# SokhengDin/DNN-MPPI-MPC

Measured on AMD Instinct MI355X. Metric: trajectory-steps/sec (KxT/iter_time), diff-drive K=4096 T=50, higher is better.
Workload: dtype f32; 1 GPU; BASELINE config 2: differential-drive analytic dynamics, K=4096 x T=50 per GPU, reference __main__ parameters, closed loop with the driver's plant on the device; K_per_gpu=4096, K_global=4096, T=50, waypoint_mode=sequential (reference-exact), noise=Philox4x32-10 in-kernel, waypoint_idx_at_end_of_timing=99, build_id=5d93f4b6a923ee1f, exchange=none (one GPU)

## Files before the change

### dnn-mppi-mpc_amd/_capi.py

```python
from __future__ import annotations

import ctypes as C
import os

PKG = os.path.dirname(os.path.abspath(__file__))
ABI_VERSION = 6
MIN_AB_ABI_VERSION = 3
LIB_PATH = os.environ.get("MPPI_LIB") or os.path.join(PKG, "lib", "libmppi_hip.so")

MODEL_DIFFDRIVE, MODEL_RACECAR, MODEL_DIFFDRIVE_MLP = 0, 1, 2
PREC_F32, PREC_F64 = 0, 1
WAYPOINT_SEQUENTIAL, WAYPOINT_FROZEN, WAYPOINT_PER_ROLLOUT = 0, 1, 2
BETA_INV_EXPLORATION, BETA_INV_LAMBDA, BETA_LAMBDA = 0, 1, 2
FILTER_DIFFDRIVE, FILTER_RACECAR, FILTER_NONE, FILTER_TORCH = 0, 1, 2, 3
OBSTACLE_NONE, OBSTACLE_CIRCLE, OBSTACLE_OUTLINE = 0, 1, 2
OK, ERR_BAD_ARG, ERR_SHAPE, ERR_NO_DEVICE, ERR_HIP, ERR_PATH_END, ERR_UNSUPPORTED, ERR_STATE = 0, -1, -2, -3, -4, -5, -6, -7
ERR_COMM = -8
LAYOUT_FUSED, LAYOUT_DUAL, LAYOUT_PAIR, LAYOUT_TRI, LAYOUT_KIND, LAYOUT_TWICE = 0, 1, 2, 3, 3, 4


class MppiConfig(C.Structure):
    _fields_ = [
        ("struct_size", C.c_int32), ("device", C.c_int32), ("model", C.c_int32), ("precision", C.c_int32),
        ("K", C.c_int32), ("T", C.c_int32), ("K_global", C.c_int32), ("k_offset", C.c_int32),
        ("delta_t", C.c_double), ("u_max", C.c_double * 2), ("wheel_base", C.c_double),
        ("param_exploration", C.c_double), ("param_lambda", C.c_double), ("param_alpha", C.c_double),
        ("sigma", C.c_double * 4), ("stage_cost_weight", C.c_double * 4), ("terminal_cost_weight", C.c_double * 4),
        ("beta_mode", C.c_int32), ("accumulate_stage_cost", C.c_int32), ("waypoint_mode", C.c_int32),
        ("search_window", C.c_int32), ("wrap_yaw_stage", C.c_int32), ("wrap_yaw_terminal", C.c_int32),
        ("clamp_rollout", C.c_int32), ("clamp_u_after_update", C.c_int32), ("filter_mode", C.c_int32),
        ("filter_window", C.c_int32), ("obstacle_model", C.c_int32), ("raise_at_path_end", C.c_int32),
        ("safety_margin", C.c_double), ("vehicle_w", C.c_double), ("vehicle_l", C.c_double),
        ("collision_penalty", C.c_double), ("seed", C.c_uint64), ("n_agents", C.c_int32), ("noise_stream", C.c_int32),
    ]


class MppiStats(C.Structure):
    _fields_ = [("rho", C.c_double), ("eta", C.c_double), ("ess", C.c_double), ("idx_start", C.c_int32),
                ("idx_after", C.c_int32), ("path_end", C.c_int32), ("rounds", C.c_int32), ("iteration", C.c_int64),
                ("n_collided", C.c_int32), ("reserved", C.c_int32), ("iter_us", C.c_double), ("kernel_us", C.c_double)]


class MppiError(RuntimeError):
    def __init__(self, code, msg):
        super().__init__(f"libmppi_hip: {msg} (status {code})")
        self.code = code


_H = C.c_void_p
_D = C.POINTER(C.c_double)

PROTOTYPES = {
    "mppi_abi_version": (C.c_int, []),
    "mppi_last_error": (C.c_char_p, [_H]),
    "mppi_device_count": (C.c_int, []),
    "mppi_create": (C.c_int, [C.POINTER(MppiConfig), C.POINTER(_H)]),
    "mppi_destroy": (C.c_int, [_H]),
    "mppi_set_ref_path": (C.c_int, [_H, _D, C.c_int32, C.c_int32]),
    "mppi_set_obstacles": (C.c_int, [_H, _D, C.c_int32]),
    "mppi_set_agent_ref_path": (C.c_int, [_H, C.c_int32, _D, C.c_int32, C.c_int32]),
    "mppi_set_agent_obstacles": (C.c_int, [_H, C.c_int32, _D, C.c_int32]),
    "mppi_get_agent_status": (C.c_int, [_H, C.POINTER(C.c_int32), C.POINTER(C.c_int32)]),
    "mppi_set_mlp": (C.c_int, [_H, C.c_int32, C.c_int32, C.POINTER(C.c_float), C.POINTER(C.c_float),
                              C.POINTER(C.POINTER(C.c_float)), C.POINTER(C.POINTER(C.c_float)),
                              C.POINTER(C.c_float), C.POINTER(C.c_float)]),
    "mppi_set_mlp_scaled": (C.c_int, [_H, C.c_int32, C.c_int32, C.POINTER(C.c_float), C.POINTER(C.c_float),
                                     C.POINTER(C.POINTER(C.c_float)), C.POINTER(C.POINTER(C.c_float)),
                                     C.POINTER(C.c_float), C.POINTER(C.c_float), C.POINTER(C.c_double),
                                     C.POINTER(C.c_double), C.POINTER(C.c_double), C.POINTER(C.c_double)]),
    "mppi_set_agent_mlp": (C.c_int, [_H, C.c_int32, C.c_int32, C.c_int32, C.POINTER(C.c_float), C.POINTER(C.c_float),
                                    C.POINTER(C.POINTER(C.c_float)), C.POINTER(C.POINTER(C.c_float)),
                                    C.POINTER(C.c_float), C.POINTER(C.c_float)]),
    "mppi_set_agent_mlp_scaled": (C.c_int, [_H, C.c_int32, C.c_int32, C.c_int32, C.POINTER(C.c_float), C.POINTER(C.c_float),
                                           C.POINTER(C.POINTER(C.c_float)), C.POINTER(C.POINTER(C.c_float)),
                                           C.POINTER(C.c_float), C.POINTER(C.c_float), C.POINTER(C.c_double),
                                           C.POINTER(C.c_double), C.POINTER(C.c_double), C.POINTER(C.c_double)]),
    "mppi_set_u_prev": (C.c_int, [_H, _D]),
    "mppi_get_u_prev": (C.c_int, [_H, _D]),
    "mppi_set_waypoint_idx": (C.c_int, [_H, C.c_int32]),
    "mppi_get_waypoint_idx": (C.c_int, [_H, C.POINTER(C.c_int32)]),
    "mppi_step": (C.c_int, [_H, _D, C.c_void_p, _D, _D, C.POINTER(MppiStats), C.c_void_p]),
    "mppi_partial_len": (C.c_int, [_H, C.POINTER(C.c_int32)]),
    "mppi_step_begin": (C.c_int, [_H, _D, C.c_void_p, C.c_void_p, C.c_void_p]),
    "mppi_step_end": (C.c_int, [_H, C.c_void_p, C.c_int32, _D, _D, C.POINTER(MppiStats), C.c_void_p]),
    "mppi_step_end_async": (C.c_int, [_H, C.c_void_p, C.c_int32, C.c_void_p]),
    "mppi_sync_result": (C.c_int, [_H, _D, _D, C.POINTER(MppiStats), C.c_void_p]),
    "mppi_comm_handle_bytes": (C.c_int, []),
    "mppi_comm_export": (C.c_int, [_H, C.c_int32, C.c_void_p]),
    "mppi_comm_buffer": (C.c_int, [_H, C.POINTER(C.c_void_p)]),
    "mppi_comm_connect": (C.c_int, [_H, C.c_int32, C.c_int32, C.c_void_p, C.POINTER(C.c_void_p)]),
    "mppi_comm_probe": (C.c_int, [_H, C.c_void_p]),
    "mppi_comm_close": (C.c_int, [_H]),
    "mppi_get_costs": (C.c_int, [_H, _D]),
    "mppi_get_weights": (C.c_int, [_H, _D]),
    "mppi_sample_epsilon": (C.c_int, [_H, C.c_int64, C.c_void_p, C.c_void_p]),
    "mppi_set_iteration": (C.c_int, [_H, C.c_int64]),
    "mppi_set_noise_ring": (C.c_int, [_H, C.c_void_p, C.c_int32]),
    "mppi_rollout_viz": (C.c_int, [_H, C.c_void_p, C.c_void_p, C.c_void_p]),
    "mppi_set_state": (C.c_int, [_H, _D]),
    "mppi_get_state": (C.c_int, [_H, _D]),
    "mppi_run_closed_loop": (C.c_int, [_H, C.c_int32, _D, C.POINTER(MppiStats), C.c_void_p]),
    "mppi_last_kernel_ms": (C.c_int, [_H, C.POINTER(C.c_float)]),
    "mppi_enable_timing": (C.c_int, [_H, C.c_int32]),
    "mppi_set_rollout_repeats": (C.c_int, [_H, C.c_int32]),
    "mppi_get_counters": (C.c_int, [_H, C.POINTER(C.c_int64)]),
    "mppi_comm_unique_id_bytes": (C.c_int, []),
    "mppi_comm_unique_id": (C.c_int, [C.c_void_p]),
    "mppi_comm_init": (C.c_int, [_H, C.c_void_p, C.c_int32, C.c_int32]),
    "mppi_get_rollout_layout": (C.c_int, [_H, C.POINTER(C.c_int32)]),
    "mppi_get_host_timing": (C.c_int, [_H, C.POINTER(C.c_double)]),
    "mppi_get_rollout_kernel": (C.c_int, [_H, C.c_char_p, C.c_int32]),
    "mppi_time_rollout_launch": (C.c_int, [_H, C.c_int32, C.c_int32, C.c_void_p, C.POINTER(C.c_double)]),
    "mppi_step_device_x0": (C.c_int, [_H, C.c_void_p, C.c_void_p, _D, _D, C.POINTER(MppiStats), C.c_void_p]),
    "mppi_eval_state_transition": (C.c_int, [_H, _D, _D, C.c_int32, _D]),
    "mppi_eval_clamp": (C.c_int, [_H, _D, C.c_int32, _D]),
    "mppi_eval_is_collided": (C.c_int, [_H, _D, C.c_int32, _D]),
    "mppi_eval_nearest_waypoint": (C.c_int, [_H, _D, C.c_int32, C.POINTER(C.c_int32), C.c_int32, C.POINTER(C.c_int32)]),
    "mppi_eval_cost": (C.c_int, [_H, C.c_int32, _D, C.c_int32, C.POINTER(C.c_int32), C.c_int32, _D, C.POINTER(C.c_int32)]),
    "mppi_eval_moving_average": (C.c_int, [_H, _D, _D]),
    "mppi_eval_weights": (C.c_int, [_H, _D, C.c_int32, _D]),
    "mppi_cb_last_error": (C.c_char_p, [_H]),
    "mppi_cb_create": (C.c_int, [C.c_void_p, C.POINTER(_H)]),
    "mppi_cb_destroy": (C.c_int, [_H]),
    "mppi_cb_set_nominal": (C.c_int, [_H, _D]),
    "mppi_cb_get_nominal": (C.c_int, [_H, _D]),
    "mppi_cb_command": (C.c_int, [_H, _D, C.c_void_p, C.c_int32, _D, C.c_void_p]),
    "mppi_cb_get_costs": (C.c_int, [_H, _D, _D]),
    "mppi_cb_eval": (C.c_int, [_H, C.c_int32, _D, _D, C.c_int32, C.c_int32, _D]),
    "mppi_cb_nominal_trajectory": (C.c_int, [_H, _D, _D]),
}

_lib = None


def load_library(path: str | None = None):
    global _lib
    if _lib is not None and path is None:
        return _lib
    p = path or LIB_PATH
    if not os.path.exists(p):
        raise MppiError(ERR_NO_DEVICE, f"{p} not found: build it with __graft_entry__.build() "
                                       "(hipcc --offload-arch=gfx950); there is no CPU fallback")
    try:
        import torch
    except ImportError:
        pass
    lib = C.CDLL(p)
    ab_build = bool(os.environ.get("MPPI_LIB")) and path is None
    for name, (res, args) in PROTOTYPES.items():
        if ab_build and not hasattr(lib, name):
            continue
        fn = getattr(lib, name)
        fn.restype, fn.argtypes = res, args
    if lib.mppi_abi_version() != ABI_VERSION and not ab_build:
        raise MppiError(ERR_BAD_ARG, "ABI version mismatch between _capi.py and libmppi_hip.so")
    if ab_build and lib.mppi_abi_version() < MIN_AB_ABI_VERSION:
        raise MppiError(ERR_BAD_ARG, f"MPPI_LIB={p} has ABI version {lib.mppi_abi_version()}: its mppi_config / mppi_stats "
                                     f"layouts differ from this binding's (needs >= {MIN_AB_ABI_VERSION})")
    if path is None:
        _lib = lib
    return lib


def check(lib, handle, rc):
    if rc != OK:
        msg = lib.mppi_last_error(handle)
        raise MppiError(rc, msg.decode() if msg else "unknown error")
```

### dnn-mppi-mpc_amd/build.py

```python
from __future__ import annotations

import os
import subprocess

PKG = os.path.dirname(os.path.abspath(__file__))
CSRC = os.path.join(PKG, "csrc")
LIB = os.path.join(PKG, "lib", "libmppi_hip.so")


def lib_is_stale() -> bool:
    if not os.path.exists(LIB):
        return True
    t = os.path.getmtime(LIB)
    srcs = [os.path.join(CSRC, f) for f in os.listdir(CSRC) if f.endswith((".hip", ".h"))]
    srcs.append(os.path.join(os.path.dirname(PKG), "include", "mppi_hip.h"))
    return any(os.path.getmtime(s) > t for s in srcs)


def source_id() -> str:
    import hashlib
    h = hashlib.sha256()
    files = sorted(os.path.join(CSRC, f) for f in os.listdir(CSRC) if f.endswith((".hip", ".h")))
    files.append(os.path.join(os.path.dirname(PKG), "include", "mppi_hip.h"))
    for f in files:
        h.update(os.path.basename(f).encode())
        with open(f, "rb") as fh:
            h.update(fh.read())
    return h.hexdigest()[:16]


PRIMS_LIB = os.path.join(PKG, "lib", "libmppi_prims.so")
PRIMS_SRC = os.path.join(os.path.dirname(PKG), "tests", "device", "prims_harness.hip")


def prims_library() -> str:
    srcs = [PRIMS_SRC] + [os.path.join(CSRC, f) for f in os.listdir(CSRC) if f.endswith(".h")]
    if not os.path.exists(PRIMS_LIB) or any(os.path.getmtime(s) > os.path.getmtime(PRIMS_LIB) for s in srcs):
        res = subprocess.run(["make", "-C", CSRC, "prims"], stdout=subprocess.PIPE, stderr=subprocess.STDOUT, text=True)
        if res.returncode != 0:
            print(res.stdout)
            raise RuntimeError("building libmppi_prims.so failed (hipcc, gfx950)")
    return PRIMS_LIB


def build(force: bool = False, verbose: bool = False) -> str:
    if force or lib_is_stale() or not os.path.exists(PRIMS_LIB):
        cmd = ["make", "-j4", "-C", CSRC] + (["-B"] if force else [])
        res = subprocess.run(cmd, stdout=subprocess.PIPE, stderr=subprocess.STDOUT, text=True)
        if verbose or res.returncode != 0:
            print(res.stdout)
        if res.returncode != 0:
            raise RuntimeError("building libmppi_hip.so failed (hipcc, gfx950)")
    return LIB
```

### dnn-mppi-mpc_amd/csrc/mppi_capi.hip

```cpp
#include <dlfcn.h>
#include <hip/hip_runtime.h>
#include <math.h>
#include <stdio.h>
#include <stdlib.h>
#include <string.h>

#include <time.h>

#include <algorithm>
#include <string>
#include <vector>

#include "../../include/mppi_hip.h"
#include "mppi_kernels.h"
#include "mppi_owner.h"

using namespace mppi;

static thread_local std::string g_create_error;

static double now_s() {
    timespec ts;
    clock_gettime(CLOCK_MONOTONIC, &ts);
    return (double)ts.tv_sec + 1e-9 * (double)ts.tv_nsec;
}

static Switches read_switches() {
    const auto set = [](const char *name) { return getenv(name) != nullptr; };
    const auto num = [](const char *name, int unset) {
        const char *e = getenv(name);
        return e ? atoi(e) : unset;
    };
    const auto on_off = [&](const char *name) { return set(name) ? (int)(num(name, 0) != 0) : -1; };
    Switches sw;
    sw.dual = on_off("MPPI_DUAL");
    sw.pair = on_off("MPPI_PAIR");
    sw.tri = on_off("MPPI_TRI");
    sw.seq = set("MPPI_SEQ") ? (num("MPPI_SEQ", 0) == 2 ? 2 : 1) : -1;
    sw.no_stream = set("MPPI_NO_STREAM");
    sw.stream_passes = num("MPPI_STREAM_PASSES", 0);
    sw.force_unfused = set("MPPI_FORCE_UNFUSED");
    sw.no_hyp = set("MPPI_NO_HYP");
    sw.no_poll = set("MPPI_NO_POLL");
    sw.no_args = set("MPPI_NO_ARGS");
    sw.traj_per_block = num("MPPI_TRAJ_PER_BLOCK", 0);
    sw.graph = on_off("MPPI_GRAPH") == 1;
    sw.graph_verbose = set("MPPI_GRAPH_VERBOSE");
    sw.graph_slots = std::max(1, num("MPPI_GRAPH_SLOTS", 64));
    sw.mlp.f32 = set("MPPI_MLP_F32");
    sw.mlp.terms = num("MPPI_MLP_TERMS", 3) == 2 ? 2 : 3;
    const char *form = getenv("MPPI_MLP_FORM");
    sw.mlp.form = form && !strcmp(form, "4x64") ? 0 : form && !strcmp(form, "8x64") ? 1 : -1;
    if (const char *e = getenv("MPPI_EXCHANGE_TIMEOUT_MS")) sw.exchange_timeout_ms = atoll(e);
    sw.lb_timeout_ticks = std::max(0, num("MPPI_LB_TIMEOUT_TICKS", (int)LB_TIMEOUT_TICKS));
    return sw;
}

struct RcclUniqueId { char internal[128]; };

struct mppi_handle {
    mppi_config cfg;
    Switches sw;
    bool f64 = false;
    int nx = 3, n_ref = 0, n_obs = 0, n_blocks = 0, traj_per_block = 0;
    bool fused = false;
    int B = 1;
    int slots = 0;
    std::vector<Event> ev;
    size_t ev_used = 0;
    Event ev_step[2];
    bool graph_on = false;
    std::vector<char> graph_key;
    Stream graph_stream;
    Event graph_ev_in, graph_ev_out;
    Event graph_done[2];
    GraphExec graph_exec[2];
    DevBuf<void> d_partials2;
    DevBuf<void> d_heads, d_heads2;
    DevBuf<float> d_mlp;
    DevBuf<unsigned short> d_mlp16;
    size_t mlp_cap = 0, mlp16_cap = 0;
    bool hyp = false;
    DevBuf<unsigned> d_hyp_slots;
    unsigned lb_seq = 0;
    std::vector<double> ref_host;
    StepResult *res_mapped = nullptr;
    long long seq = 0;
    bool idx_valid = true;
    int layout = 0;
    const char *rollout_kernel = "";
    MlpParams mlp = {}, mlp_shared = {};
    bool shared_set = false;
    struct OwnModel {
        DevBuf<float> d_mlp;
        DevBuf<unsigned short> d_mlp16;
        size_t cap = 0, cap16 = 0;
        MlpParams q = {};
        bool set = false;
    };
    std::vector<OwnModel> own_mlp;
    DevBuf<MlpParams> d_models;
    DevBuf<void> d_ref, d_obs, d_u, d_uhist, d_S;
    struct OwnScene {
        DevBuf<void> d_ref, d_obs;
        int n_ref = 0, n_obs = 0;
        bool has_obs = false;
    };
    std::vector<OwnScene> own;
    DevBuf<AgentScene> d_scenes;
    DevBuf<int> d_pout;
    DevBuf<void> d_partials;
    DevBuf<double> d_w, d_trace;
    long long trace_cap = 0;
    DevBuf<DevState> d_st;
    DevBuf<StepResult> d_res;
    PinnedBuf<StepResult> h_res;
    size_t res_bytes = 0;
    const float *last_eps = nullptr;
    const float *noise_ring = nullptr;
    int noise_slots = 0;
    bool begun = false, timing = false, dev_loop_primed = false, slot_timed = false;
    long long iter = 0;
    int idx = 0, rollout_repeats = 1;
    float last_ms[4] = {0, 0, 0, 0};
    double last_iter_us = 0.0;
    FineBuf<char> xbuf;
    size_t xbuf_bytes = 0;
    int x_rank = 0, x_nranks = 0, x_export_nranks = 0;
    std::vector<IpcMap> x_opened;
    DevBuf<char *> d_xpeers;
    DevBuf<int> d_xerr, d_xok;
    long long xseq = 0, x_timeout = 300000000LL;
    void *rccl_comm = nullptr;
    int rccl_rank = 0, rccl_nranks = 0;
    DevBuf<double> d_rccl_part, d_rccl_gath;
    long long n_rollout_launches = 0, n_finalize_launches = 0;
    double t_enqueue_s = 0.0, t_loop_s = 0.0;
    std::string err;
};

#define FAIL(h, code, ...)                                   \
    do {                                                     \
        char _b[512];                                        \
        snprintf(_b, sizeof(_b), __VA_ARGS__);               \
        if (h) (h)->err = _b; else g_create_error = _b;      \
        return (code);                                       \
    } while (0)
#define CREATE_FAIL(code, ...) FAIL((mppi_handle *)nullptr, code, __VA_ARGS__)

#define HIPCHECK(h, call)                                                                          \
    do {                                                                                           \
        hipError_t _e = (call);                                                                    \
        if (_e != hipSuccess) FAIL(h, MPPI_ERR_HIP, "%s failed: %s", #call, hipGetErrorString(_e)); \
    } while (0)

extern "C" int mppi_abi_version(void) { return MPPI_ABI_VERSION; }

extern "C" const char *mppi_last_error(const mppi_handle *h) { return h ? h->err.c_str() : g_create_error.c_str(); }

extern "C" int mppi_device_count(void) {
    int n = 0;
    if (hipGetDeviceCount(&n) != hipSuccess) return 0;
    return n;
}

template <typename Fn> static auto with_real(const mppi_handle *h, Fn &&f) { return h->f64 ? f(double{}) : f(float{}); }

static size_t rsz(const mppi_handle *h) { return with_real(h, [](auto r) { return sizeof(r); }); }

static int kernel_model(const mppi_config &c) { return c.model == MPPI_MODEL_RACECAR ? MODEL_RACE : MODEL_DIFF; }
static double softmin_beta(const mppi_config &c) {
    return c.beta_mode == MPPI_BETA_INV_EXPLORATION ? 1.0 / c.param_exploration
           : c.beta_mode == MPPI_BETA_INV_LAMBDA    ? 1.0 / c.param_lambda
                                                    : c.param_lambda;
}
static bool at_path_end(const mppi_handle *h, int idx) { return idx >= h->n_ref - 1; }
static AgentScene scene_of(const mppi_handle *h, int a) {
    AgentScene sc = {h->d_ref, h->d_obs, h->n_ref, h->n_obs, {0, 0}};
    if (a < (int)h->own.size()) {
        const mppi_handle::OwnScene &o = h->own[a];
        if (o.d_ref) sc.ref = o.d_ref, sc.n_ref = o.n_ref;
        if (o.has_obs) sc.obs = o.d_obs, sc.n_obs = o.n_obs;
    }
    if (h->cfg.obstacle_model == MPPI_OBSTACLE_NONE) sc.n_obs = 0;
    return sc;
}
static bool any_obstacles(const mppi_handle *h) {
    for (int a = 0; a < h->B; ++a)
        if (scene_of(h, a).n_obs > 0) return true;
    return false;
}
static bool lookback_serves(const mppi_handle *h, int records) {
    const mppi_config &c = h->cfg;
    const bool lb_layout = (h->layout & LAYOUT_KIND) == LAYOUT_FUSED || h->layout == LAYOUT_DUAL;
    return h->fused && lb_layout && c.T <= 64 && c.model == MPPI_MODEL_DIFFDRIVE && c.waypoint_mode == MPPI_WAYPOINT_SEQUENTIAL &&
           !c.accumulate_stage_cost && (c.search_window == HYP_WINDOW || c.search_window == HYP_WINDOW_CUDA) && c.n_agents == 1 &&
           records <= HYP_MAX_BLOCKS && !h->sw.no_hyp;
}
static bool index_can_move(const mppi_handle *h) { return h->hyp && !(h->idx_valid && h->n_ref > 0 && at_path_end(h, h->idx)); }
template <typename R> static KParams<R> make_params(const mppi_handle *h, const float *eps);
template <typename R> static RolloutPlan front_plan(const mppi_handle *h, const KParams<R> &P);

static int upload_real(mppi_handle *h, void *dst, const double *src, size_t n) {
    return with_real(h, [&](auto r) -> int {
        using R = decltype(r);
        const std::vector<R> tmp(src, src + n);
        HIPCHECK(h, hipMemcpy(dst, tmp.data(), n * sizeof(R), hipMemcpyHostToDevice));
        return MPPI_OK;
    });
}

static int download_real(mppi_handle *h, double *dst, const void *src, size_t n) {
    return with_real(h, [&](auto r) -> int {
        using R = decltype(r);
        std::vector<R> tmp(n);
        HIPCHECK(h, hipMemcpy(tmp.data(), src, n * sizeof(R), hipMemcpyDeviceToHost));
        std::copy(tmp.begin(), tmp.end(), dst);
        return MPPI_OK;
    });
}

extern "C" int mppi_create(const mppi_config *cfg, mppi_handle **out) {
    if (!cfg || !out) CREATE_FAIL(MPPI_ERR_BAD_ARG, "mppi_create: null argument");
    if (cfg->struct_size != (int32_t)sizeof(mppi_config))
        CREATE_FAIL(MPPI_ERR_BAD_ARG, "mppi_create: struct_size %d != %zu (ABI mismatch)", cfg->struct_size, sizeof(mppi_config));
    mppi_config c = *cfg;
    const Switches sw = read_switches();
    if (c.K_global == 0) c.K_global = c.K;
    if (c.K > (1 << 20) || c.T > 2048)
        CREATE_FAIL(MPPI_ERR_SHAPE, "K=%d / T=%d beyond the supported 2^20 samples / 2048 steps", c.K, c.T);
    if (c.K < 1 || c.T < 1 || c.K_global < c.K || c.k_offset < 0 || c.k_offset + c.K > c.K_global)
        CREATE_FAIL(MPPI_ERR_SHAPE, "mppi_create: bad K=%d T=%d K_global=%d k_offset=%d", c.K, c.T, c.K_global, c.k_offset);
    if (c.model != MPPI_MODEL_DIFFDRIVE && c.model != MPPI_MODEL_RACECAR && c.model != MPPI_MODEL_DIFFDRIVE_MLP)
        CREATE_FAIL(MPPI_ERR_BAD_ARG, "mppi_create: unknown model %d", c.model);
    if (c.model == MPPI_MODEL_DIFFDRIVE_MLP && c.precision != MPPI_PREC_F32)
        CREATE_FAIL(MPPI_ERR_UNSUPPORTED, "the learned-dynamics rollout runs on the f32 MFMA path only");
    if (c.precision != MPPI_PREC_F32 && c.precision != MPPI_PREC_F64)
        CREATE_FAIL(MPPI_ERR_BAD_ARG, "mppi_create: unknown precision %d", c.precision);
    if (c.waypoint_mode != MPPI_WAYPOINT_SEQUENTIAL && c.waypoint_mode != MPPI_WAYPOINT_FROZEN && c.waypoint_mode != MPPI_WAYPOINT_PER_ROLLOUT)
        CREATE_FAIL(MPPI_ERR_BAD_ARG, "mppi_create: unknown waypoint_mode %d", c.waypoint_mode);
    if (c.waypoint_mode == MPPI_WAYPOINT_PER_ROLLOUT && c.model == MPPI_MODEL_RACECAR)
        CREATE_FAIL(MPPI_ERR_UNSUPPORTED,
// ... 554 lines not shown
    P.window = c.search_window;
    P.model = kernel_model(c);
    P.accumulate = c.accumulate_stage_cost;
    P.sequential = c.waypoint_mode == MPPI_WAYPOINT_SEQUENTIAL;
    P.per_rollout = c.waypoint_mode == MPPI_WAYPOINT_PER_ROLLOUT;
    P.lb_timeout = h->sw.lb_timeout_ticks;
    P.obstacle_model = any_obstacles(h) ? c.obstacle_model : OBS_NONE;
    P.clamp_rollout = c.clamp_rollout;
    P.wrap_stage = c.wrap_yaw_stage;
    P.wrap_term = c.wrap_yaw_terminal;
    const float *noise = eps ? eps : h->noise_ring;
    P.eps_slots = eps ? 0 : (h->noise_ring ? h->noise_slots : 0);
    P.use_philox = noise == nullptr;
    P.traj_per_block = h->traj_per_block;
    P.seed_lo = (unsigned)(c.seed & 0xffffffffu);
    P.seed_hi = (unsigned)(c.seed >> 32);
    P.dt = (R)c.delta_t;
    P.umax0 = (R)c.u_max[0];
    P.umax1 = (R)c.u_max[1];
    P.wheel_base = (R)c.wheel_base;
    P.beta = (R)softmin_beta(c);
    P.gamma = (R)(c.param_lambda * (1.0 - c.param_alpha));
    P.penalty = (R)c.collision_penalty;
    P.two_pi = (R)(2.0 * M_PI);
    const double det = c.sigma[0] * c.sigma[3] - c.sigma[1] * c.sigma[2];
    const double si[4] = {c.sigma[3] / det, -c.sigma[1] / det, -c.sigma[2] / det, c.sigma[0] / det};
    for (int i = 0; i < 4; ++i) {
        P.sinv[i] = (R)si[i];
        P.ws[i] = (R)c.stage_cost_weight[i];
        P.wt[i] = (R)c.terminal_cost_weight[i];
    }
    const double vw = c.vehicle_w * c.safety_margin, vl = c.vehicle_l * c.safety_margin;
    const double sx[9] = {-0.5 * vl, -0.5 * vl, 0.0, 0.5 * vl, 0.5 * vl, 0.5 * vl, 0.0, -0.5 * vl, -0.5 * vl};
    const double sy[9] = {0.0, 0.5 * vw, 0.5 * vw, 0.5 * vw, 0.0, -0.5 * vw, -0.5 * vw, -0.5 * vw, 0.0};
    for (int i = 0; i < 9; ++i) {
        P.shape_x[i] = (R)sx[i];
        P.shape_y[i] = (R)sy[i];
    }
    const double l00 = sqrt(c.sigma[0]), l10 = c.sigma[2] / l00, l11 = sqrt(c.sigma[3] - l10 * l10);
    P.chol[0] = (float)l00;
    P.chol[1] = (float)l10;
    P.chol[2] = (float)l11;
    P.ref = (const R *)sc0.ref;
    P.obs = (const R *)sc0.obs;
    P.scenes = h->d_scenes;
    P.u = (const R *)h->d_u.get();
    P.eps = noise;
    P.S = (R *)h->d_S.get();
    P.pout = h->d_pout;
    P.st = h->d_st;
    P.noise_stream = c.noise_stream;
    P.slots = h->slots;
    P.n_agents = h->B;
    P.layout = h->layout;
    P.heads = (R *)h->d_heads.get();
    P.hyp = index_can_move(h);
    P.lb_seq = 0;
    P.hyp_slots = h->d_hyp_slots;
    return P;
}

static double record_beta(const mppi_handle *h) {
    const double beta = softmin_beta(h->cfg);
    return h->f64 ? beta : (double)(float)beta;
}

static FinalizeParams make_finalize(const mppi_handle *h, int plant, const void *abi_recs = nullptr, int n_recs = 0) {
    const mppi_config &c = h->cfg;
    FinalizeParams F;
    memset(&F, 0, sizeof(F));
    F.T = c.T;
    F.K = c.K;
    F.n_part = n_recs;
    F.filter_mode = c.filter_mode;
    F.filter_window = c.filter_window;
    F.clamp_u = c.clamp_u_after_update;
    F.raise_at_path_end = c.raise_at_path_end;
    F.model = kernel_model(c);
    F.sequential = c.waypoint_mode == MPPI_WAYPOINT_SEQUENTIAL;
    F.plant = plant;
    const AgentScene sc0 = scene_of(h, 0);
    F.n_ref = sc0.n_ref;
    F.window = c.search_window;
    F.is_f64 = h->f64;
    F.count_hits = any_obstacles(h);
    F.beta = record_beta(h);
    F.dt = c.delta_t;
    F.wheel_base = c.wheel_base;
    F.umax0 = c.u_max[0];
    F.umax1 = c.u_max[1];
    F.partials = abi_recs;
    F.heads = h->d_heads;
    F.u = h->d_u;
    F.u_out = h->d_u;
    F.u_before = h->d_uhist;
    F.ref = sc0.ref;
    F.scenes = h->d_scenes;
    F.pout = h->d_pout;
    F.st = h->d_st;
    F.st_out = h->d_st;
    F.res = h->d_res;
    F.slots = h->slots;
    F.n_agents = h->B;
    F.res_stride = h->res_bytes;
    F.u0_trace = nullptr;
    F.hyp_slots = h->d_hyp_slots;
    F.lb_seq = 0;
    F.pad_lb = 0;
    return F;
}

constexpr int EV_PER_SLOT = 8;
constexpr size_t EV_MAX = 8u * 200000u;

static hipEvent_t next_event(mppi_handle *h) {
    if (h->ev_used == h->ev.size()) hipEventCreate(h->ev.emplace_back().put());
    return h->ev[h->ev_used++];
}

static bool timing_on(const mppi_handle *h) { return h->timing && h->ev_used + EV_PER_SLOT <= EV_MAX; }

static void wire_exchange(const mppi_handle *h, FinalizeParams &F) {
    if (h->x_nranks <= 1) return;
    F.x_nranks = h->x_nranks;
    F.x_rank = h->x_rank;
    F.x_timeout = h->x_timeout;
    F.x_peers = h->d_xpeers;
    F.x_err = h->d_xerr;
}

template <typename R> static RolloutPlan front_plan(const mppi_handle *h, const KParams<R> &P) {
    if constexpr (sizeof(R) == 4)
        if (h->cfg.model == MPPI_MODEL_DIFFDRIVE_MLP) return plan_mlp(P, h->mlp, h->sw);
    return plan_rollout<R>(P, h->fused, h->sw);
}

struct SlotPlan {
    RolloutPlan front;
    bool reduce = false;
    int n_merges = 0;
    MergeStep merge[2];
    double beta = 0.0;
    KernelLaunch fin;
};
template <typename R>
static SlotPlan plan_slot(const mppi_handle *h, const KParams<R> &P, FinalizeParams *F, double *rank_record = nullptr) {
    SlotPlan sp;
    sp.front = front_plan<R>(h, P);
    sp.reduce = h->cfg.model != MPPI_MODEL_DIFFDRIVE_MLP && !h->fused;
    sp.beta = record_beta(h);
    const void *recs = h->d_partials, *heads = h->d_heads;
    const MergeTree tree = merge_tree(sp.front.records, rank_record == nullptr);
    if (tree.group) {
        sp.merge[sp.n_merges++] = plan_merge<R>(recs, heads, sp.front.records, tree.group, h->cfg.T, h->d_partials2, h->d_heads2);
        recs = h->d_partials2;
        heads = h->d_heads2;
    }
    if (rank_record) {
        sp.merge[sp.n_merges++] = plan_merge<R>(recs, heads, tree.n_out, tree.n_out, h->cfg.T, rank_record, nullptr);
        return sp;
    }
    F->partials = recs;
    F->heads = heads;
    F->n_part = tree.n_out;
    F->hyp = sp.front.lookback;
    F->hyp_blocks = sp.front.records;
    wire_exchange(h, *F);
    sp.fin = plan_finalize<R>(*F, false, sp.front.lookback);
    return sp;
}

template <typename R> static void launch_records(mppi_handle *h, const SlotPlan &sp, const KParams<R> &P, hipStream_t s, bool tm) {
    if (tm) hipEventRecord(next_event(h), s);
    h->n_rollout_launches += h->rollout_repeats;
    for (int rep = 0; rep < h->rollout_repeats; ++rep) {
        if constexpr (sizeof(R) == 4)
            if (h->cfg.model == MPPI_MODEL_DIFFDRIVE_MLP) {
                launch_mlp(sp.front, P, h->mlp, h->d_models, h->d_partials, nullptr, s);
                continue;
            }
        launch_rollout<R>(sp.front, P, h->d_partials, s);
    }
    h->rollout_kernel = sp.front.k.name;
    if (tm) hipEventRecord(next_event(h), s);
    if (tm) hipEventRecord(next_event(h), s);
    if (sp.reduce) launch_reduce<R>(P, h->d_partials, sp.front.records, s);
    for (int i = 0; i < sp.n_merges; ++i) launch_merge<R>(sp.merge[i], h->cfg.T, sp.beta, s);
    if (tm) hipEventRecord(next_event(h), s);
}

static void launch_back(mppi_handle *h, const KernelLaunch &fin, const FinalizeParams &F, hipStream_t s, bool tm) {
    if (tm) hipEventRecord(next_event(h), s);
    ++h->n_finalize_launches;
    launch_finalize(fin, F, s);
    if (tm) hipEventRecord(next_event(h), s);
    if (tm) hipEventRecord(next_event(h), s);
    if (tm) hipEventRecord(next_event(h), s);
}

template <typename R>
static void launch_slot(mppi_handle *h, const SlotPlan &sp, const KParams<R> &P, FinalizeParams F, hipStream_t s) {
    const bool tm = timing_on(h);
    if (F.x_nranks > 1) F.x_seq = ++h->xseq;
    if (sp.front.lookback) {
        if ((++h->lb_seq & 0xffffffu) == 0u) ++h->lb_seq;
        KParams<R> Pl = P;
        Pl.lb_seq = F.lb_seq = h->lb_seq;
        launch_records<R>(h, sp, Pl, s, tm);
    } else {
        launch_records<R>(h, sp, P, s, tm);
    }
    launch_back(h, sp.fin, F, s, tm);
}

static void collect_timing(mppi_handle *h) {
    double acc[4] = {0, 0, 0, 0};
    const size_t slots = h->ev_used / EV_PER_SLOT;
    for (size_t i = 0; i < slots; ++i)
        for (int j = 0; j < 4; ++j) {
            float ms = 0;
            hipEventElapsedTime(&ms, h->ev[EV_PER_SLOT * i + 2 * j], h->ev[EV_PER_SLOT * i + 2 * j + 1]);
            acc[j] += ms;
        }
    const double cal = slots ? acc[3] / slots : 0.0;
    for (int j = 0; j < 3; ++j) {
        const double v = slots ? acc[j] / slots - cal : 0.0;
        h->last_ms[j] = (float)(v > 0 ? v : 0);
    }
    h->last_ms[3] = (float)cal;
}

static int check_ready(mppi_handle *h, const char *who) {
    if (!h) return MPPI_ERR_BAD_ARG;
    for (int a = 0; a < h->B; ++a) {
        const AgentScene sc = scene_of(h, a);
        if (!sc.ref || sc.n_ref < 1) {
            if (h->B > 1) FAIL(h, MPPI_ERR_STATE, "%s: ref_path of agent %d has not been set", who, a);
            FAIL(h, MPPI_ERR_STATE, "%s: ref_path has not been set", who);
        }
        if (sc.n_obs > 0 && !sc.obs) FAIL(h, MPPI_ERR_STATE, "%s: obstacles not uploaded", who);
    }
    if (h->cfg.model == MPPI_MODEL_DIFFDRIVE_MLP)
        for (int a = 0; a < h->B; ++a)
            if (!has_model(h, a)) {
                if (h->B > 1) FAIL(h, MPPI_ERR_STATE, "%s: agent %d has no model (mppi_set_mlp / mppi_set_agent_mlp)", who, a);
                FAIL(h, MPPI_ERR_STATE, "%s: mppi_set_mlp has not been called", who);
            }
    return MPPI_OK;
}

#define SINGLE_AGENT_ONLY(h, who)                                                                                     \
    do {                                                                                                              \
        if ((h)->B > 1) FAIL(h, MPPI_ERR_UNSUPPORTED, "%s serves single-agent handles (n_agents = %d)", who, (h)->B); \
    } while (0)

static void fill_stats(mppi_handle *h, mppi_stats *stats) {
    if (!stats) return;
    if (h->timing && h->ev_used >= EV_PER_SLOT) {
        if (hipEventSynchronize(h->ev[h->ev_used - 1]) == hipSuccess) collect_timing(h);
        else (void)hipGetLastError();
    }
    const StepResult *r = h->h_res;
    stats->rho = r->rho;
    stats->eta = r->eta;
    stats->ess = r->ess;
    stats->idx_start = r->idx_start;
    stats->idx_after = r->idx_after;
    stats->path_end = r->path_end;
    stats->rounds = r->rounds;
    stats->iteration = r->iter;
    stats->n_collided = r->n_collided;
    stats->reserved = 0;
    stats->iter_us = h->last_iter_us;
    stats->kernel_us = h->timing ? 1e3 * ((double)h->last_ms[0] + h->last_ms[1] + h->last_ms[2]) : 0.0;
}

static int host_x0_call(const mppi_handle *h, const double *x0) {
    const int p = h->idx, n = h->n_ref, w = h->cfg.search_window;
    int best_j = 0;
    double best = INFINITY;
    for (int j = 0; j < w && p + j < n; ++j) {
        const double dx = x0[0] - h->ref_host[4 * (size_t)(p + j)], dy = x0[1] - h->ref_host[4 * (size_t)(p + j) + 1];
        const double d = dx * dx + dy * dy;
        if (d < best) { best = d; best_j = j; }
    }
    return p + best_j;
}

static int fetch_result(mppi_handle *h, size_t bytes, hipStream_t s, bool check_launches = true) {
    HIPCHECK(h, hipMemcpyAsync(h->h_res, h->d_res, bytes, hipMemcpyDeviceToHost, s));
    HIPCHECK(h, hipStreamSynchronize(s));
    if (check_launches) HIPCHECK(h, hipGetLastError());
    return MPPI_OK;
}

static int wait_result(mppi_handle *h, long long seq, hipStream_t s) {
    if (seq) {
        volatile long long *flag = &h->h_res->seq;
        const double t0 = now_s();
        for (long long spins = 0; *flag != seq; ++spins) {
            __builtin_ia32_pause();
            if ((spins & 1023) == 1023 && now_s() - t0 > 0.020) {
                HIPCHECK(h, hipStreamSynchronize(s));
                HIPCHECK(h, hipGetLastError());
                if (*flag != seq) FAIL(h, MPPI_ERR_HIP, "the finalize kernel never published its result");
                break;
            }
        }
        __atomic_thread_fence(__ATOMIC_ACQUIRE);
        return MPPI_OK;
    }
    return fetch_result(h, h->res_bytes, s);
}

static void note_noise(mppi_handle *h, const float *eps, bool observed_state) {
    h->last_eps = eps;
    if (observed_state) h->dev_loop_primed = false;
}

enum : unsigned {
    KEEP_IDX_VALID = 1u,
    KEEP_GOING = 2u,
};
static int adopt_result(mppi_handle *h, unsigned keep, double *u_out, double *u0_out, mppi_stats *stats) {
    const StepResult *res = h->h_res;
    h->idx = res->idx_after;
    if (!(keep & KEEP_IDX_VALID)) h->idx_valid = true;
    fill_stats(h, stats);
    if (!(keep & KEEP_GOING)) {
        if (res->status == STATUS_EXCHANGE_FAILED)
            FAIL(h, MPPI_ERR_COMM, "peer-to-peer exchange: a rank did not arrive within the timeout");
        if (res->status == STATUS_PATH_END) FAIL(h, MPPI_ERR_PATH_END, "[ERROR] Reached the end of the reference path.");
    }
    h->iter = res->iter;
    if (u_out) memcpy(u_out, reinterpret_cast<const double *>(h->h_res + 1), sizeof(double) * 2 * h->cfg.T);
    if (u0_out) { u0_out[0] = res->u0[0]; u0_out[1] = res->u0[1]; }
    return MPPI_OK;
}

template <typename R>
static int step_rccl(mppi_handle *h, const double *x0, const double *x0_dev, const float *eps, double *u_out, double *u0_out,
                     mppi_stats *stats, hipStream_t s);
template <typename R>
static int closed_loop_rccl(mppi_handle *h, int n_iters, double *u0_trace, mppi_stats *stats, hipStream_t s);

template <typename R>
static int step_impl(mppi_handle *h, const double *x0, const double *x0_dev, const float *eps, double *u_out, double *u0_out,
                     mppi_stats *stats, hipStream_t s) {
    if (h->rccl_comm && h->x_nranks <= 1) return step_rccl<R>(h, x0, x0_dev, eps, u_out, u0_out, stats, s);
    const double t_call = now_s();
    KParams<R> P = make_params<R>(h, eps);
    FinalizeParams F = make_finalize(h, 0);
    const bool by_args = x0 && h->idx_valid && !h->sw.no_args;
    if (!x0) {
        if (!h->idx_valid) FAIL(h, MPPI_ERR_STATE, "mppi_step_device_x0 after an asynchronous split step: call mppi_sync_result first");
        launch_set_state_dev<R>(P, x0_dev, h->nx, s);
    } else if (by_args) {
        P.use_args = F.use_args = 1;
        P.c_arg = F.c_arg = host_x0_call(h, x0);
        P.hyp = h->hyp && !at_path_end(h, P.c_arg);
        for (int i = 0; i < 4; ++i) P.x0_arg[i] = F.x0_arg[i] = x0[i];
    } else {
        launch_set_state<R>(P, x0, s);
    }
    if (!h->sw.no_poll) F.res = h->res_mapped;
    const SlotPlan sp = plan_slot<R>(h, P, &F);
    for (int round = 0;; ++round) {
        F.seq = !h->sw.no_poll ? ++h->seq : 0;
        launch_slot<R>(h, sp, P, F, s);
        HIPCHECK(h, hipGetLastError());
        int rc = wait_result(h, F.seq, s);
        if (rc) return rc;
        if (h->h_res->status != STATUS_NEED_ROUND) break;
        if (round > h->cfg.K + 1) FAIL(h, MPPI_ERR_STATE, "waypoint speculation did not converge");
        P.use_args = 0;
    }
    note_noise(h, eps, true);
    h->last_iter_us = 1e6 * (now_s() - t_call);
    return adopt_result(h, 0, u_out, u0_out, stats);
}

extern "C" int mppi_step(mppi_handle *h, const double *x0, const float *eps, double *u_out, double *u0_out,
                         mppi_stats *stats, void *stream) {
    int rc = check_ready(h, "mppi_step");
    if (rc) return rc;
    SINGLE_AGENT_ONLY(h, "mppi_step");
    if (!x0) FAIL(h, MPPI_ERR_BAD_ARG, "mppi_step: x0 is null");
    HIPCHECK(h, hipSetDevice(h->cfg.device));
    double x[4] = {0, 0, 0, 0};
    for (int i = 0; i < h->nx; ++i) x[i] = x0[i];
    return with_real(h, [&](auto r) { return step_impl<decltype(r)>(h, x, nullptr, eps, u_out, u0_out, stats, (hipStream_t)stream); });
}

extern "C" int mppi_step_device_x0(mppi_handle *h, const double *x0_device, const float *eps, double *u_out, double *u0_out,
                                   mppi_stats *stats, void *stream) {
    int rc = check_ready(h, "mppi_step_device_x0");
    if (rc) return rc;
    SINGLE_AGENT_ONLY(h, "mppi_step_device_x0");
    if (!x0_device) FAIL(h, MPPI_ERR_BAD_ARG, "mppi_step_device_x0: x0 is null");
    HIPCHECK(h, hipSetDevice(h->cfg.device));
    return with_real(h, [&](auto r) { return step_impl<decltype(r)>(h, nullptr, x0_device, eps, u_out, u0_out, stats, (hipStream_t)stream); });
}

extern "C" int mppi_partial_len(const mppi_handle *h, int32_t *n) {
    if (!h || !n) return MPPI_ERR_BAD_ARG;
    *n = partial_len(h->cfg.T);
    return MPPI_OK;
}

template <typename R>
static int begin_impl(mppi_handle *h, const double *x0, const float *eps, double *partial, hipStream_t s) {
    KParams<R> P = make_params<R>(h, eps);
    if (x0 || !h->dev_loop_primed) launch_set_state<R>(P, x0, s);
    h->dev_loop_primed = x0 == nullptr;
    h->slot_timed = timing_on(h);
    launch_records<R>(h, plan_slot<R>(h, P, nullptr, partial), P, s, h->slot_timed);
    HIPCHECK(h, hipGetLastError());
    note_noise(h, eps, false);
    h->begun = true;
    return MPPI_OK;
}

extern "C" int mppi_step_begin(mppi_handle *h, const double *x0, const float *eps, double *partial, void *stream) {
    int rc = check_ready(h, "mppi_step_begin");
    if (rc) return rc;
    SINGLE_AGENT_ONLY(h, "mppi_step_begin");
    if (!partial) FAIL(h, MPPI_ERR_BAD_ARG, "mppi_step_begin: null argument");
    if (h->cfg.waypoint_mode == MPPI_WAYPOINT_SEQUENTIAL)
        FAIL(h, MPPI_ERR_UNSUPPORTED, "the split step needs MPPI_WAYPOINT_FROZEN (no cross-sample waypoint state)");
    HIPCHECK(h, hipSetDevice(h->cfg.device));
    double x[4] = {0, 0, 0, 0};
    if (x0)
        for (int i = 0; i < h->nx; ++i) x[i] = x0[i];
    return with_real(h, [&](auto r) { return begin_impl<decltype(r)>(h, x0 ? x : nullptr, eps, partial, (hipStream_t)stream); });
}

extern "C" int mppi_step_end(mppi_handle *h, const double *partials, int32_t nranks, double *u_out, double *u0_out,
                             mppi_stats *stats, void *stream) {
    int rc = check_ready(h, "mppi_step_end");
    if (rc) return rc;
    SINGLE_AGENT_ONLY(h, "mppi_step_end");
    if (!partials || nranks < 1 || nranks > MERGE_MAX_RECORDS)
        FAIL(h, MPPI_ERR_BAD_ARG, "mppi_step_end: bad partials/nranks (1..%d)", MERGE_MAX_RECORDS);
    if (!h->begun) FAIL(h, MPPI_ERR_STATE, "mppi_step_end without mppi_step_begin");
    HIPCHECK(h, hipSetDevice(h->cfg.device));
    hipStream_t s = (hipStream_t)stream;
    const FinalizeParams F = make_finalize(h, 0, partials, nranks);
    with_real(h, [&](auto r) { launch_back(h, plan_finalize<decltype(r)>(F, true, false), F, s, h->slot_timed); });
    if ((rc = fetch_result(h, h->res_bytes, s))) return rc;
    h->begun = false;
    h->dev_loop_primed = false;
    return adopt_result(h, KEEP_IDX_VALID, u_out, u0_out, stats);
}

extern "C" int mppi_step_end_async(mppi_handle *h, const double *partials, int32_t nranks, void *stream) {
    int rc = check_ready(h, "mppi_step_end_async");
    if (rc) return rc;
    SINGLE_AGENT_ONLY(h, "mppi_step_end_async");
    if (!partials || nranks < 1 || nranks > MERGE_MAX_RECORDS)
        FAIL(h, MPPI_ERR_BAD_ARG, "mppi_step_end_async: bad partials/nranks (1..%d)", MERGE_MAX_RECORDS);
    if (!h->begun) FAIL(h, MPPI_ERR_STATE, "mppi_step_end_async without mppi_step_begin");
    HIPCHECK(h, hipSetDevice(h->cfg.device));
    const FinalizeParams F = make_finalize(h, 1, partials, nranks);
    with_real(h, [&](auto r) { launch_back(h, plan_finalize<decltype(r)>(F, true, false), F, (hipStream_t)stream, h->slot_timed); });
    HIPCHECK(h, hipGetLastError());
    h->begun = false;
    h->idx_valid = false;
    return MPPI_OK;
}

extern "C" int mppi_sync_result(mppi_handle *h, double *u_out, double *u0_out, mppi_stats *stats, void *stream) {
    if (!h) return MPPI_ERR_BAD_ARG;
    HIPCHECK(h, hipSetDevice(h->cfg.device));
    if (int rc = fetch_result(h, h->res_bytes, (hipStream_t)stream, false)) return rc;
    return adopt_result(h, 0, u_out, u0_out, stats);
}

extern "C" int mppi_get_costs(mppi_handle *h, double *S) {
    if (!h || !S) return MPPI_ERR_BAD_ARG;
    HIPCHECK(h, hipSetDevice(h->cfg.device));
    HIPCHECK(h, hipDeviceSynchronize());
    return download_real(h, S, h->d_S, (size_t)h->B * h->cfg.K);
}

extern "C" int mppi_get_weights(mppi_handle *h, double *w) {
    if (!h || !w) return MPPI_ERR_BAD_ARG;
    SINGLE_AGENT_ONLY(h, "mppi_get_weights");
    HIPCHECK(h, hipSetDevice(h->cfg.device));
    HIPCHECK(h, hipDeviceSynchronize());
    if (!h->d_w) HIPCHECK(h, h->d_w.alloc(sizeof(double) * h->cfg.K));
    with_real(h, [&](auto r) {
        using R = decltype(r);
        launch_weights<R>(make_params<R>(h, nullptr), h->h_res->rho, h->h_res->eta, h->d_w, nullptr);
    });
    HIPCHECK(h, hipDeviceSynchronize());
    HIPCHECK(h, hipMemcpy(w, h->d_w, sizeof(double) * h->cfg.K, hipMemcpyDeviceToHost));
    return MPPI_OK;
}

extern "C" int mppi_sample_epsilon(mppi_handle *h, int64_t iteration, float *eps_out, void *stream) {
    if (!h || !eps_out || iteration < 0) return MPPI_ERR_BAD_ARG;
    HIPCHECK(h, hipSetDevice(h->cfg.device));
    KParams<float> P = make_params<float>(h, nullptr);
    for (int a = 0; a < h->B; ++a)
        launch_sample(P.seed_lo, P.seed_hi, (unsigned)iteration, h->cfg.K, h->cfg.T, h->cfg.k_offset, P.chol,
                      eps_out + (size_t)a * h->cfg.K * h->cfg.T * 2, (hipStream_t)stream, (unsigned)(h->cfg.noise_stream + a));
    HIPCHECK(h, hipGetLastError());
    return MPPI_OK;
}

extern "C" int mppi_set_noise_ring(mppi_handle *h, const float *eps_ring, int32_t n_slots) {
    if (!h) return MPPI_ERR_BAD_ARG;
    if (!eps_ring || n_slots == 0) {
        h->noise_ring = nullptr;
        h->noise_slots = 0;
        return MPPI_OK;
    }
    if (n_slots < 1 || (n_slots & (n_slots - 1)) != 0)
        FAIL(h, MPPI_ERR_BAD_ARG, "mppi_set_noise_ring: n_slots must be a power of two (got %d)", n_slots);
    hipPointerAttribute_t at;
    memset(&at, 0, sizeof(at));
    if (hipPointerGetAttributes(&at, eps_ring) != hipSuccess || at.type == hipMemoryTypeHost || at.type == hipMemoryTypeUnregistered ||
        at.device != h->cfg.device) {
        (void)hipGetLastError();
        FAIL(h, MPPI_ERR_BAD_ARG, "mppi_set_noise_ring: the ring must be device memory on the handle's GPU (device %d)", h->cfg.device);
    }
    h->noise_ring = eps_ring;
    h->noise_slots = n_slots;
    return MPPI_OK;
}

extern "C" int mppi_rollout_viz(mppi_handle *h, float *optimal_traj, float *sampled_traj, void *stream) {
    int rc = check_ready(h, "mppi_rollout_viz");
    if (rc) return rc;
    SINGLE_AGENT_ONLY(h, "mppi_rollout_viz");
    if (h->iter < 1) FAIL(h, MPPI_ERR_STATE, "mppi_rollout_viz before the first mppi_step");
    HIPCHECK(h, hipSetDevice(h->cfg.device));
    with_real(h, [&](auto r) {
        using R = decltype(r);
        const KParams<R> P = make_params<R>(h, h->last_eps);
        const R *hist = (const R *)h->d_uhist.get(), *hist_after = hist + 2 * h->cfg.T;
        if constexpr (sizeof(R) == 4)
            if (h->cfg.model == MPPI_MODEL_DIFFDRIVE_MLP)
                return launch_viz_mlp(P, h->mlp, h->sw, hist, hist_after, h->iter - 1, optimal_traj, sampled_traj, (hipStream_t)stream);
        launch_viz<R>(P, hist, hist_after, h->iter - 1, optimal_traj, sampled_traj, (hipStream_t)stream);
    });
    HIPCHECK(h, hipGetLastError());
    return MPPI_OK;
}


namespace {
struct RcclApi {
    void *lib = nullptr;
    int (*GetUniqueId)(void *) = nullptr;
    int (*CommInitRank)(void **, int, RcclUniqueId, int) = nullptr;
    int (*AllGather)(const void *, void *, size_t, int, void *, hipStream_t) = nullptr;
    int (*CommDestroy)(void *) = nullptr;
    const char *(*GetErrorString)(int) = nullptr;
    std::string why;
};
RcclApi rccl_load() {
    RcclApi a;
    for (const char *name : {"librccl.so.1", "librccl.so"}) {
        a.lib = dlopen(name, RTLD_NOW | RTLD_GLOBAL);
        if (a.lib) break;
    }
    if (!a.lib) {
        a.why = std::string("librccl.so.1 could not be loaded: ") + dlerror();
        return a;
    }
    a.GetUniqueId = reinterpret_cast<decltype(a.GetUniqueId)>(dlsym(a.lib, "ncclGetUniqueId"));
    a.CommInitRank = reinterpret_cast<decltype(a.CommInitRank)>(dlsym(a.lib, "ncclCommInitRank"));
    a.AllGather = reinterpret_cast<decltype(a.AllGather)>(dlsym(a.lib, "ncclAllGather"));
    a.CommDestroy = reinterpret_cast<decltype(a.CommDestroy)>(dlsym(a.lib, "ncclCommDestroy"));
    a.GetErrorString = reinterpret_cast<decltype(a.GetErrorString)>(dlsym(a.lib, "ncclGetErrorString"));
    if (!a.GetUniqueId || !a.CommInitRank || !a.AllGather || !a.CommDestroy || !a.GetErrorString) {
        a.why = "librccl.so.1 lacks an expected symbol";
        a.lib = nullptr;
    }
    return a;
}
RcclApi &rccl_api() {
    static RcclApi a = rccl_load();
    return a;
}
}

static void rccl_release(mppi_handle *h) {
    if (h->rccl_comm) rccl_api().CommDestroy(h->rccl_comm);
    (void)h->d_rccl_part.reset();
    (void)h->d_rccl_gath.reset();
    h->rccl_comm = nullptr;
    h->rccl_nranks = 0;
}

#define RCCLCHECK(h, call)                                                                                   \
    do {                                                                                                     \
        const int _r = (call);                                                                               \
        if (_r != 0) FAIL(h, MPPI_ERR_COMM, "%s failed: %s", #call, rccl_api().GetErrorString(_r));          \
    } while (0)

extern "C" int mppi_comm_unique_id_bytes(void) { return (int)sizeof(RcclUniqueId); }

extern "C" int mppi_comm_unique_id(void *id_out) {
    if (!id_out) return MPPI_ERR_BAD_ARG;
    RcclApi &a = rccl_api();
    if (!a.lib) {
        g_create_error = a.why;
        return MPPI_ERR_COMM;
    }
    if (a.GetUniqueId(id_out) != 0) {
        g_create_error = "ncclGetUniqueId failed";
        return MPPI_ERR_COMM;
    }
    return MPPI_OK;
}

extern "C" int mppi_comm_init(mppi_handle *h, const void *unique_id, int32_t rank, int32_t nranks) {
    if (!h || !unique_id) return MPPI_ERR_BAD_ARG;
    SINGLE_AGENT_ONLY(h, "mppi_comm_init");
    if (nranks < 1 || nranks > MERGE_MAX_RECORDS || rank < 0 || rank >= nranks)
        FAIL(h, MPPI_ERR_BAD_ARG, "mppi_comm_init: rank %d of %d (1..%d ranks)", rank, nranks, MERGE_MAX_RECORDS);
    if (h->cfg.waypoint_mode == MPPI_WAYPOINT_SEQUENTIAL)
        FAIL(h, MPPI_ERR_UNSUPPORTED, "the exchange needs MPPI_WAYPOINT_FROZEN (no cross-sample waypoint state)");
    RcclApi &a = rccl_api();
    if (!a.lib) FAIL(h, MPPI_ERR_COMM, "mppi_comm_init: %s", a.why.c_str());
    HIPCHECK(h, hipSetDevice(h->cfg.device));
    rccl_release(h);
    RcclUniqueId id;
    memcpy(&id, unique_id, sizeof(id));
    RCCLCHECK(h, a.CommInitRank(&h->rccl_comm, nranks, id, rank));
    const size_t len = (size_t)partial_len(h->cfg.T);
    HIPCHECK(h, h->d_rccl_part.alloc(sizeof(double) * len));
    HIPCHECK(h, h->d_rccl_gath.alloc(sizeof(double) * len * nranks));
    h->rccl_rank = rank;
    h->rccl_nranks = nranks;
    return MPPI_OK;
}

static int trace_rows(mppi_handle *h, int n_iters, double **rows) {
    if (h->trace_cap < n_iters) {
        h->trace_cap = 0;
        HIPCHECK(h, h->d_trace.reset());
        HIPCHECK(h, h->d_trace.alloc(sizeof(double) * 2 * n_iters));
        h->trace_cap = n_iters;
    }
    *rows = h->d_trace.get() - 2 * h->iter;
    return MPPI_OK;
}

template <typename R>
static int rccl_iteration(mppi_handle *h, const KParams<R> &P, int plant, double *u0_trace_dev, hipStream_t s) {
    const bool tm = timing_on(h);
    launch_records<R>(h, plan_slot<R>(h, P, nullptr, h->d_rccl_part), P, s, tm);
    RCCLCHECK(h, rccl_api().AllGather(h->d_rccl_part, h->d_rccl_gath, (size_t)partial_len(h->cfg.T), 8 ,
                                      h->rccl_comm, s));
    FinalizeParams F = make_finalize(h, plant, h->d_rccl_gath, h->rccl_nranks);
    F.u0_trace = u0_trace_dev;
    launch_back(h, plan_finalize<R>(F, true, false), F, s, tm);
    return MPPI_OK;
}

static int rccl_fetch(mppi_handle *h, double *u_out, double *u0_out, mppi_stats *stats, hipStream_t s) {
    HIPCHECK(h, hipGetLastError());
    if (int rc = fetch_result(h, h->res_bytes, s)) return rc;
    return adopt_result(h, 0, u_out, u0_out, stats);
}

template <typename R>
static int step_rccl(mppi_handle *h, const double *x0, const double *x0_dev, const float *eps, double *u_out, double *u0_out,
                     mppi_stats *stats, hipStream_t s) {
    const KParams<R> P = make_params<R>(h, eps);
    if (x0) launch_set_state<R>(P, x0, s);
    else launch_set_state_dev<R>(P, x0_dev, h->nx, s);
    if (int rc = rccl_iteration<R>(h, P, 0, nullptr, s)) return rc;
    note_noise(h, eps, true);
    return rccl_fetch(h, u_out, u0_out, stats, s);
}

template <typename R>
static int closed_loop_rccl(mppi_handle *h, int n_iters, double *u0_trace, mppi_stats *stats, hipStream_t s) {
    const KParams<R> P = make_params<R>(h, nullptr);
    double *trace = nullptr;
    if (u0_trace)
        if (int rc = trace_rows(h, n_iters, &trace)) return rc;
    if (!h->dev_loop_primed) launch_set_state<R>(P, nullptr, s);
    h->dev_loop_primed = false;
    for (int i = 0; i < n_iters; ++i)
        if (int rc = rccl_iteration<R>(h, P, 1, trace, s)) return rc;
    note_noise(h, nullptr, false);
    if (int rc = rccl_fetch(h, nullptr, nullptr, stats, s)) return rc;
    if (u0_trace) HIPCHECK(h, hipMemcpy(u0_trace, h->d_trace, sizeof(double) * 2 * n_iters, hipMemcpyDeviceToHost));
    h->dev_loop_primed = true;
    return MPPI_OK;
}

extern "C" int mppi_comm_handle_bytes(void) { return (int)sizeof(hipIpcMemHandle_t); }

extern "C" int mppi_comm_close(mppi_handle *h) {
    if (!h) return MPPI_ERR_BAD_ARG;
    hipSetDevice(h->cfg.device);
    hipDeviceSynchronize();
    h->x_opened.clear();
    (void)h->d_xpeers.reset();
    (void)h->d_xerr.reset();
    (void)h->d_xok.reset();
    (void)h->xbuf.reset();
    h->x_nranks = h->x_export_nranks = 0;
    rccl_release(h);
    return MPPI_OK;
}

extern "C" int mppi_comm_export(mppi_handle *h, int32_t nranks, void *handle_out) {
    if (!h || !handle_out) return MPPI_ERR_BAD_ARG;
    SINGLE_AGENT_ONLY(h, "mppi_comm_export");
    if (nranks < 2 || nranks > XCHG_MAX_RANKS)
        FAIL(h, MPPI_ERR_BAD_ARG, "mppi_comm_export: nranks must be 2..%d (got %d)", XCHG_MAX_RANKS, nranks);
    if (h->cfg.waypoint_mode == MPPI_WAYPOINT_SEQUENTIAL)
        FAIL(h, MPPI_ERR_UNSUPPORTED, "the exchange needs MPPI_WAYPOINT_FROZEN (no cross-sample waypoint state)");
    if (merge_lds_elems(h->cfg.T, h->cfg.filter_window, rsz(h)) * rsz(h) + sizeof(double) * XCHG_LDS_RANKS * xchg_rec_len(h->cfg.T) > 64 * 1024)
        FAIL(h, MPPI_ERR_UNSUPPORTED, "the peer-to-peer exchange stages the rank records in LDS: horizon T=%d is too long for it "
                                      "(use the split step with a collective)", h->cfg.T);
    if (h->xbuf) mppi_comm_close(h);
    HIPCHECK(h, hipSetDevice(h->cfg.device));
    h->xbuf_bytes = 2 * xchg_slot_bytes(h->cfg.T, nranks);
    HIPCHECK(h, h->xbuf.alloc(h->xbuf_bytes));
    HIPCHECK(h, hipMemset(h->xbuf, 0, h->xbuf_bytes));
    HIPCHECK(h, hipDeviceSynchronize());
    hipIpcMemHandle_t ipc;
    HIPCHECK(h, hipIpcGetMemHandle(&ipc, h->xbuf));
    memcpy(handle_out, &ipc, sizeof(ipc));
    h->x_export_nranks = nranks;
    return MPPI_OK;
}

extern "C" int mppi_comm_buffer(mppi_handle *h, void **device_ptr) {
    if (!h || !device_ptr) return MPPI_ERR_BAD_ARG;
    if (!h->xbuf) FAIL(h, MPPI_ERR_STATE, "mppi_comm_buffer before mppi_comm_export");
    *device_ptr = h->xbuf;
    return MPPI_OK;
}

extern "C" int mppi_comm_connect(mppi_handle *h, int32_t rank, int32_t nranks, const void *handles,
                                 void *const *local_ptrs) {
    if (!h || (!handles && !local_ptrs)) return MPPI_ERR_BAD_ARG;
    if (!h->xbuf || nranks != h->x_export_nranks)
        FAIL(h, MPPI_ERR_STATE, "mppi_comm_connect: call mppi_comm_export with the same nranks first");
    if (rank < 0 || rank >= nranks) FAIL(h, MPPI_ERR_BAD_ARG, "mppi_comm_connect: rank %d of %d", rank, nranks);
    HIPCHECK(h, hipSetDevice(h->cfg.device));
    std::vector<char *> peers(nranks, nullptr);
    std::vector<IpcMap> opened;
    for (int r = 0; r < nranks; ++r) {
        if (r == rank) {
            peers[r] = h->xbuf;
        } else if (local_ptrs && local_ptrs[r]) {
            hipPointerAttribute_t at;
            memset(&at, 0, sizeof(at));
            if (hipPointerGetAttributes(&at, local_ptrs[r]) != hipSuccess || at.type == hipMemoryTypeHost ||
                at.type == hipMemoryTypeUnregistered) {
                (void)hipGetLastError();
                FAIL(h, MPPI_ERR_UNSUPPORTED, "mppi_comm_connect: local_ptrs[%d] is not device memory (pass the peer's mppi_comm_buffer)", r);
            }
            if (at.device != h->cfg.device) {
                int can = 0;
                if (hipDeviceCanAccessPeer(&can, h->cfg.device, at.device) != hipSuccess || !can)
                    FAIL(h, MPPI_ERR_UNSUPPORTED, "mppi_comm_connect: device %d cannot access rank %d's buffer on device %d "
                                                  "(no peer access: use the collective carrier)", h->cfg.device, r, at.device);
                const hipError_t pe = hipDeviceEnablePeerAccess(at.device, 0);
                if (pe != hipSuccess && pe != hipErrorPeerAccessAlreadyEnabled)
                    FAIL(h, MPPI_ERR_UNSUPPORTED, "mppi_comm_connect: hipDeviceEnablePeerAccess(%d) failed: %s", at.device,
                         hipGetErrorString(pe));
                (void)hipGetLastError();
            }
            peers[r] = (char *)local_ptrs[r];
        } else {
            if (!handles) FAIL(h, MPPI_ERR_BAD_ARG, "mppi_comm_connect: no handle for rank %d", r);
            hipIpcMemHandle_t ipc;
            memcpy(&ipc, (const char *)handles + sizeof(ipc) * (size_t)r, sizeof(ipc));
            HIPCHECK(h, hipIpcOpenMemHandle(opened.emplace_back().put(), ipc, hipIpcMemLazyEnablePeerAccess));
            peers[r] = (char *)opened.back().get();
        }
    }
    DevBuf<char *> d_xpeers;
    DevBuf<int> d_xerr, d_xok;
    HIPCHECK(h, d_xpeers.alloc(sizeof(char *) * nranks));
    HIPCHECK(h, hipMemcpy(d_xpeers, peers.data(), sizeof(char *) * nranks, hipMemcpyHostToDevice));
    HIPCHECK(h, d_xerr.alloc(sizeof(int)));
    HIPCHECK(h, d_xok.alloc(sizeof(int)));
    HIPCHECK(h, hipMemset(d_xerr, 0, sizeof(int)));
    h->d_xpeers = std::move(d_xpeers);
    h->d_xerr = std::move(d_xerr);
    h->d_xok = std::move(d_xok);
    for (IpcMap &m : opened) h->x_opened.push_back(std::move(m));
    if (const long long ms = read_switches().exchange_timeout_ms; ms > 0) h->x_timeout = ms * 100000LL;
    h->x_rank = rank;
    h->x_nranks = nranks;
    h->xseq = 0;
    return MPPI_OK;
}

extern "C" int mppi_comm_probe(mppi_handle *h, void *stream) {
    if (!h) return MPPI_ERR_BAD_ARG;
    if (h->x_nranks <= 1) FAIL(h, MPPI_ERR_STATE, "mppi_comm_probe before mppi_comm_connect");
    HIPCHECK(h, hipSetDevice(h->cfg.device));
    FinalizeParams F = make_finalize(h, 0);
    wire_exchange(h, F);
    F.x_seq = ++h->xseq;
    launch_exchange_probe(F, h->d_xok, (hipStream_t)stream);
    int ok = 0;
    HIPCHECK(h, hipMemcpyAsync(&ok, h->d_xok, sizeof(int), hipMemcpyDeviceToHost, (hipStream_t)stream));
    HIPCHECK(h, hipStreamSynchronize((hipStream_t)stream));
    if (!ok) {
// ... 206 lines not shown
    return MPPI_OK;
}

extern "C" int mppi_time_rollout_launch(mppi_handle *h, int32_t n_slots, int32_t extra, void *stream, double *us_out2) {
    int rc = check_ready(h, "mppi_time_rollout_launch");
    if (rc) return rc;
    if (!us_out2 || n_slots < 1 || n_slots > 4096 || extra < 1 || extra > 16)
        FAIL(h, MPPI_ERR_BAD_ARG, "mppi_time_rollout_launch: n_slots 1..4096, extra 1..16");
    if (h->x_nranks > 1 || h->rccl_comm)
        FAIL(h, MPPI_ERR_UNSUPPORTED, "mppi_time_rollout_launch: not with an exchange between ranks (its sequence numbers cannot be replayed)");
    HIPCHECK(h, hipSetDevice(h->cfg.device));
    return with_real(h, [&](auto r) { return time_rollout_impl<decltype(r)>(h, n_slots, extra, (hipStream_t)stream, us_out2); });
}

static void eval_transition_mlp(mppi_handle *h, const KParams<float> &P, const void *x, const void *v, int n, void *out) {
    launch_eval_mlp(P, h->mlp, h->sw, (const float *)x, (const float *)v, n, (float *)out, nullptr);
}
static void eval_transition_mlp(mppi_handle *, const KParams<double> &, const void *, const void *, int, void *) {}

template <typename R>
static int eval_impl(mppi_handle *h, int what, const double *x, const double *v, int n, int32_t *prev_idx, int update,
                     double *out, int32_t *idx_out) {
    const KParams<R> P = make_params<R>(h, nullptr);
    const int nx = h->nx;
    const bool need_x = what != EVAL_CLAMP, need_v = what == EVAL_TRANSITION || what == EVAL_CLAMP;
    const bool need_idx = what == EVAL_COST_STAGE || what == EVAL_COST_TERMINAL || what < 0;
    const int n_out = what == EVAL_TRANSITION ? nx : what == EVAL_CLAMP ? 2 : 1;
    DevBuf<R> dx, dv, dout;
    DevBuf<int> di, dp;
    if (need_x) {
        HIPCHECK(h, dx.alloc(sizeof(R) * (size_t)n * nx));
        if (int rc = upload_real(h, dx, x, (size_t)n * nx)) return rc;
    }
    if (need_v) {
        HIPCHECK(h, dv.alloc(sizeof(R) * (size_t)n * 2));
        if (int rc = upload_real(h, dv, v, (size_t)n * 2)) return rc;
    }
    if (need_idx) {
        if (!prev_idx) FAIL(h, MPPI_ERR_BAD_ARG, "mppi_eval: prev_idx is null");
        if (*prev_idx < 0 || *prev_idx >= P.n_ref) FAIL(h, MPPI_ERR_BAD_ARG, "mppi_eval: waypoint index %d out of range", *prev_idx);
        HIPCHECK(h, di.alloc(sizeof(int) * (size_t)n));
        HIPCHECK(h, dp.alloc(sizeof(int)));
        launch_eval_index<R>(P, dx, nx, n, *prev_idx, update ? 1 : 0, di, dp, nullptr);
    }
    if (what >= 0) {
        HIPCHECK(h, dout.alloc(sizeof(R) * (size_t)n * n_out));
        if (what == EVAL_TRANSITION && h->cfg.model == MPPI_MODEL_DIFFDRIVE_MLP)
            eval_transition_mlp(h, P, dx, dv, n, dout);
        else
            launch_eval<R>(P, what, dx, dv, di, n, dout, nullptr);
    }
    HIPCHECK(h, hipGetLastError());
    HIPCHECK(h, hipDeviceSynchronize());
    if (what >= 0)
        if (int rc = download_real(h, out, dout, (size_t)n * n_out)) return rc;
    if (need_idx) {
        if (idx_out) HIPCHECK(h, hipMemcpy(idx_out, di, sizeof(int) * (size_t)n, hipMemcpyDeviceToHost));
        int pn = *prev_idx;
        HIPCHECK(h, hipMemcpy(&pn, dp, sizeof(int), hipMemcpyDeviceToHost));
        if (update) *prev_idx = pn;
    }
    return MPPI_OK;
}

static int eval_entry(mppi_handle *h, const char *who, int what, const double *x, const double *v, int n, int32_t *prev_idx,
                      int update, double *out, int32_t *idx_out) {
    int rc = check_ready(h, who);
    if (rc) return rc;
    if (n < 1 || (what >= 0 && !out)) FAIL(h, MPPI_ERR_BAD_ARG, "%s: bad argument", who);
    if ((what != EVAL_CLAMP && !x) || ((what == EVAL_TRANSITION || what == EVAL_CLAMP) && !v))
        FAIL(h, MPPI_ERR_BAD_ARG, "%s: null input", who);
    HIPCHECK(h, hipSetDevice(h->cfg.device));
    return with_real(h, [&](auto r) { return eval_impl<decltype(r)>(h, what, x, v, n, prev_idx, update, out, idx_out); });
}

extern "C" int mppi_eval_state_transition(mppi_handle *h, const double *x, const double *v, int32_t n, double *x_next) {
    return eval_entry(h, "mppi_eval_state_transition", EVAL_TRANSITION, x, v, n, nullptr, 0, x_next, nullptr);
}
extern "C" int mppi_eval_clamp(mppi_handle *h, const double *v, int32_t n, double *out) {
    return eval_entry(h, "mppi_eval_clamp", EVAL_CLAMP, nullptr, v, n, nullptr, 0, out, nullptr);
}
extern "C" int mppi_eval_is_collided(mppi_handle *h, const double *x, int32_t n, double *out) {
    return eval_entry(h, "mppi_eval_is_collided", EVAL_COLLIDED, x, nullptr, n, nullptr, 0, out, nullptr);
}
extern "C" int mppi_eval_nearest_waypoint(mppi_handle *h, const double *x, int32_t n, int32_t *prev_idx, int32_t update_prev_idx,
                                          int32_t *idx_out) {
    if (h && !idx_out) FAIL(h, MPPI_ERR_BAD_ARG, "mppi_eval_nearest_waypoint: idx_out is null");
    return eval_entry(h, "mppi_eval_nearest_waypoint", -1, x, nullptr, n, prev_idx, update_prev_idx, nullptr, idx_out);
}
extern "C" int mppi_eval_cost(mppi_handle *h, int32_t terminal, const double *x, int32_t n, int32_t *prev_idx,
                              int32_t update_prev_idx, double *cost, int32_t *idx_out) {
    return eval_entry(h, "mppi_eval_cost", terminal ? EVAL_COST_TERMINAL : EVAL_COST_STAGE, x, nullptr, n, prev_idx,
                      update_prev_idx, cost, idx_out);
}

extern "C" int mppi_eval_moving_average(mppi_handle *h, const double *xx, double *out) {
    if (!h || !xx || !out) return MPPI_ERR_BAD_ARG;
    HIPCHECK(h, hipSetDevice(h->cfg.device));
    const int T = h->cfg.T;
    DevBuf<void> in, o;
    HIPCHECK(h, in.alloc(rsz(h) * 2 * T));
    HIPCHECK(h, o.alloc(rsz(h) * 2 * T));
    if (int rc = upload_real(h, in, xx, (size_t)2 * T)) return rc;
    with_real(h, [&](auto r) {
        using R = decltype(r);
        launch_eval_filter<R>((const R *)in.get(), (R *)o.get(), T, h->cfg.filter_window, h->cfg.filter_mode, nullptr);
    });
    HIPCHECK(h, hipGetLastError());
    HIPCHECK(h, hipDeviceSynchronize());
    return download_real(h, out, o, (size_t)2 * T);
}

extern "C" int mppi_eval_weights(mppi_handle *h, const double *S, int32_t n, double *w) {
    if (!h || !S || !w || n < 1) return MPPI_ERR_BAD_ARG;
    HIPCHECK(h, hipSetDevice(h->cfg.device));
    DevBuf<double> in, o;
    HIPCHECK(h, in.alloc(sizeof(double) * (size_t)n));
    HIPCHECK(h, o.alloc(sizeof(double) * (size_t)n));
    HIPCHECK(h, hipMemcpy(in, S, sizeof(double) * (size_t)n, hipMemcpyHostToDevice));
    launch_eval_weights(in, n, softmin_beta(h->cfg), o, nullptr);
    HIPCHECK(h, hipGetLastError());
    HIPCHECK(h, hipDeviceSynchronize());
    HIPCHECK(h, hipMemcpy(w, o, sizeof(double) * (size_t)n, hipMemcpyDeviceToHost));
    return MPPI_OK;
}

extern "C" int mppi_get_counters(mppi_handle *h, int64_t *out3) {
    if (!h || !out3) return MPPI_ERR_BAD_ARG;
    out3[0] = h->iter;
    out3[1] = h->n_rollout_launches;
    out3[2] = h->n_finalize_launches;
    return MPPI_OK;
}

extern "C" int mppi_get_host_timing(const mppi_handle *h, double *out2) {
    if (!h || !out2) return MPPI_ERR_BAD_ARG;
    out2[0] = h->t_enqueue_s;
    out2[1] = h->t_loop_s;
    return MPPI_OK;
}

extern "C" int mppi_get_rollout_layout(const mppi_handle *h, int32_t *layout) {
    if (!h || !layout) return MPPI_ERR_BAD_ARG;
    *layout = (h->fused && h->cfg.model != MPPI_MODEL_DIFFDRIVE_MLP) ? h->layout : -1;
    return MPPI_OK;
}

extern "C" int mppi_get_rollout_kernel(const mppi_handle *h, char *buf, int32_t n) {
    if (!h || !buf || n < 1) return MPPI_ERR_BAD_ARG;
    snprintf(buf, (size_t)n, "%s", h->rollout_kernel);
    return MPPI_OK;
}

extern "C" int mppi_enable_timing(mppi_handle *h, int32_t on) {
    if (!h) return MPPI_ERR_BAD_ARG;
    if (on && !h->timing) h->ev_used = 0;
    h->timing = on != 0;
    return MPPI_OK;
}

extern "C" int mppi_set_rollout_repeats(mppi_handle *h, int32_t n) {
    if (!h || n < 1 || n > 64) return MPPI_ERR_BAD_ARG;
    h->rollout_repeats = n;
    return MPPI_OK;
}

extern "C" int mppi_last_kernel_ms(mppi_handle *h, float *out4) {
    if (!h || !out4) return MPPI_ERR_BAD_ARG;
    HIPCHECK(h, hipSetDevice(h->cfg.device));
    HIPCHECK(h, hipDeviceSynchronize());
    collect_timing(h);
    memcpy(out4, h->last_ms, sizeof(h->last_ms));
    return MPPI_OK;
}
```

### dnn-mppi-mpc_amd/csrc/mppi_kernels.h

```cpp
#pragma once
#include <hip/hip_runtime.h>
#include <stdarg.h>
#include <stddef.h>
#include <stdint.h>
#include <stdio.h>

namespace mppi {

constexpr int MODEL_DIFF = 0, MODEL_RACE = 1;
constexpr int OBS_NONE = 0, OBS_CIRCLE = 1, OBS_OUTLINE = 2;
constexpr int FILTER_DIFF = 0, FILTER_RACE = 1, FILTER_NONE = 2, FILTER_TORCH = 3;
constexpr int NO_TRIGGER = 0x7fffffff;
constexpr int STATUS_DONE = 0, STATUS_NEED_ROUND = 1, STATUS_PATH_END = 2, STATUS_EXCHANGE_FAILED = 3;

constexpr int XCHG_MAX_RANKS = 64;
constexpr int XCHG_LDS_RANKS = 16;
__host__ __device__ inline int xchg_rec_len(int T) { return (3 + 2 * T + 1) & ~1; }
__host__ __device__ inline size_t xchg_slot_bytes(int T, int nranks) {
    return sizeof(long long) * XCHG_MAX_RANKS + sizeof(double) * (size_t)nranks * xchg_rec_len(T);
}

constexpr int HYP_WINDOW = 20, HYP_WINDOW_CUDA = 10;
constexpr int LB_CAND = 32, LB_BAD = 0x80;
constexpr unsigned LB_TAG_MASK = 0xffffff00u;
constexpr unsigned long long LB_TIMEOUT_TICKS = 20000ull;
constexpr int HYP_MAX_BLOCKS = 512;
constexpr int LB_COPIES = 8, LB_COPY_STRIDE = 2048;
__host__ __device__ inline unsigned lb_tag(unsigned seq) { return (seq & 0xffffffu) << 8; }

struct DevState {
    double x0[4];
    int p;
    int c;
    int k_start;
    int first_k;
    int round;
    int path_end;
    int idx_start;
    int pad;
    long long iter;
};

struct StepResult {
    int status, k_next, c_next, idx_start;
    int idx_after, path_end, rounds;
    int costs_hyp;
    int n_collided, pad_res;
    long long iter;
    double rho, eta, ess;
    double u0[2];
    double x_next[4];
    long long seq;
};

__host__ __device__ inline int partial_len(int T) { return 3 + 2 * T; }
__host__ __device__ inline int record_len(int T, int elem_bytes) {
    const int vw = 16 / elem_bytes;
    return 4 + ((2 * T + vw - 1) / vw) * vw;
}

constexpr int MERGE_THREADS = 256;
constexpr int MERGE_MAX_RECORDS = 256;
constexpr int MERGE_MAX_WINDOWS = 2;
__host__ __device__ inline size_t merge_lds_elems(int T, int W, size_t elem, int nt = MERGE_THREADS) {
    const size_t r4 = 3, nw = (2 * (size_t)(T + W + 1) + r4) & ~r4, nu = (2 * (size_t)T + r4) & ~r4;
    return nw + nu + (size_t)MERGE_MAX_WINDOWS * nt + 64 + (size_t)(nt / 32) * 32 * (16 / elem);
}
struct MergeTree { int group, n_out, windows; };
inline MergeTree merge_tree(int n, bool finalize_reads) {
    MergeTree t = {0, n, 1};
    if (n > (finalize_reads ? MERGE_MAX_WINDOWS : 1) * MERGE_MAX_RECORDS) {
        t.group = n > 64 * MERGE_MAX_RECORDS ? MERGE_MAX_RECORDS : 64;
        t.n_out = (n + t.group - 1) / t.group;
    }
    t.windows = (t.n_out + MERGE_MAX_RECORDS - 1) / MERGE_MAX_RECORDS;
    return t;
}

struct alignas(32) AgentScene {
    const void *ref, *obs;
    int n_ref, n_obs;
    int pad[2];
};
static_assert(sizeof(AgentScene) == 32, "AgentScene layout");

template <typename R> struct KParams {
    int K, T, k_offset, noise_stream;
    int n_exploit, n_ref, n_obs, window;
    int model, accumulate, sequential, obstacle_model;
    int clamp_rollout, wrap_stage, wrap_term, use_philox;
    int traj_per_block, slots;
    unsigned seed_lo, seed_hi;
    R dt, umax0, umax1, wheel_base;
    R beta, gamma, penalty, two_pi;
    R sinv[4], ws[4], wt[4];
    R shape_x[9], shape_y[9];
    float chol[3];
    const R *ref;
    const R *obs;
    const R *u;
    const float *eps;
    int eps_slots;
    int pad_eps;
    R *S;
    int *pout;
    DevState *st;
    R *heads;
    int use_args, c_arg;
    double x0_arg[4];
    int n_agents, layout;
    int per_rollout;
    int lb_timeout;
    int hyp;
    unsigned lb_seq;
    unsigned *hyp_slots;
    const AgentScene *scenes;
    long long pad_scenes[3];
};
static_assert(sizeof(KParams<float>) == 424 && sizeof(KParams<double>) == 576, "KParams layout");
static_assert(offsetof(KParams<float>, hyp) == 376 && offsetof(KParams<double>, hyp) == 528, "KParams layout");
static_assert(offsetof(KParams<float>, scenes) == 392 && offsetof(KParams<double>, scenes) == 544, "KParams layout");

struct FinalizeParams {
    int T, K, n_part, pad2;
    int filter_mode, filter_window, clamp_u, raise_at_path_end;
    int model, sequential, plant, n_ref;
    int window, is_f64, count_hits, pad1;
    double beta, dt, wheel_base, umax0, umax1;
    const void *partials;
    const void *heads;
    void *u;
    void *u_out;
    DevState *st_out;
    void *u_before;
    const void *ref;
    const int *pout;
    DevState *st;
    StepResult *res;
    double *u0_trace;
    long long seq;
    int use_args, c_arg;
    double x0_arg[4];
    int x_nranks, x_rank;
    long long x_seq;
    long long x_timeout;
    char *const *x_peers;
    int *x_err;
    int slots, n_agents;
    size_t res_stride;
    int hyp, hyp_blocks;
    const unsigned *hyp_slots;
    unsigned lb_seq, pad_lb;
    const AgentScene *scenes;
    long long pad_scenes[3];
};

constexpr int MLP_MAX_HIDDEN = 4;
struct MlpParams {
    const float *w_in, *b_in;
    const float *w_h[MLP_MAX_HIDDEN], *b_h[MLP_MAX_HIDDEN];
    const float *w_out;
    float b_out[3];
    int use_h3;
    const unsigned short *h3_w_in;
    const unsigned short *h3_w_h[MLP_MAX_HIDDEN];
    float in_gain, in_bias;
    int n_hidden;
    int hidden;
};

inline bool mlp_shape_is_h3(int hidden, int n_hidden) { return hidden == 512 && (n_hidden == 2 || n_hidden == 3); }
inline bool mlp_shape_supported(int hidden, int n_hidden) {
    return (hidden == 64 || hidden == 128 || hidden == 256 || hidden == 512) && n_hidden >= 1 && n_hidden <= MLP_MAX_HIDDEN;
}

struct VizParams {
    int K, T, model, clamp_rollout;
    int k_offset, n_exploit, use_philox, pad;
    unsigned seed_lo, seed_hi;
    long long iter;
};

template <typename R> void launch_set_state(const KParams<R> &P, const double *x0_or_null, hipStream_t s);
template <typename R> void launch_reduce(const KParams<R> &P, void *partials, int n_blocks, hipStream_t s);
bool fused_supported(int T);

struct Switches {
    int dual = -1, pair = -1, tri = -1;
    int seq = -1;
    bool no_stream = false;
    int stream_passes = 0;
    bool force_unfused = false, no_hyp = false, no_poll = false, no_args = false;
    int traj_per_block = 0;
    bool graph = false, graph_verbose = false;
    int graph_slots = 64;
    struct Mlp { bool f32 = false; int terms = 3, form = -1; } mlp;
    long long exchange_timeout_ms = 0;
    int lb_timeout_ticks = (int)LB_TIMEOUT_TICKS;
};

struct KernelLaunch {
    const void *fn = nullptr;
    const char *name = "";
    dim3 grid, block;
    size_t lds = 0;
    bool *lds_raised = nullptr;
};
struct RolloutPlan {
    KernelLaunch k;
    int records = 0;
    int passes = 0;
    bool lookback = false;
};
struct MergeStep {
    KernelLaunch k;
    const void *recs = nullptr, *heads = nullptr;
    int n = 0, group = 0;
    void *out = nullptr, *out_heads = nullptr;
};
constexpr int PLAN_MAX_DEVICES = 64;
struct KernelEntry {
    char name[96];
    bool lds_raised[PLAN_MAX_DEVICES] = {};
    __attribute__((format(printf, 2, 3))) explicit KernelEntry(const char *fmt, ...) {
        va_list ap;
        va_start(ap, fmt);
        vsnprintf(name, sizeof(name), fmt, ap);
        va_end(ap);
    }
    static const char *of(bool b) { return b ? "true" : "false"; }
};
inline KernelLaunch plan_entry(const void *fn, KernelEntry &e, int threads, size_t lds = 0) {
    KernelLaunch p;
    p.fn = fn;
    p.name = e.name;
    p.block = dim3(threads);
    p.lds = lds;
    p.lds_raised = lds ? e.lds_raised : nullptr;
    return p;
}
inline void launch_plan(const KernelLaunch &p, void **args, hipStream_t s) {
    if (p.lds_raised) {
        int dev = 0;
        (void)hipGetDevice(&dev);
        const bool known = dev >= 0 && dev < PLAN_MAX_DEVICES;
        if (!known || !p.lds_raised[dev]) {
            (void)hipFuncSetAttribute(p.fn, hipFuncAttributeMaxDynamicSharedMemorySize, (int)p.lds);
            if (known) p.lds_raised[dev] = true;
        }
    }
    (void)hipLaunchKernel(p.fn, p.grid, p.block, args, p.lds, s);
}

enum { LAYOUT_FUSED = 0, LAYOUT_DUAL = 1, LAYOUT_PAIR = 2, LAYOUT_TRI = 3, LAYOUT_KIND = 3, LAYOUT_TWICE = 4 };
int rollout_layout(const Switches &sw, int K, int T, int n_agents, int model, bool f64, bool per_rollout = false, bool tri_ok = false);
int fused_blocks(int K, int T, int layout);
int fused_max_records(int K, int T, int layout);
template <typename R> RolloutPlan plan_rollout(const KParams<R> &P, bool fused, const Switches &sw);
template <typename R> void launch_rollout(const RolloutPlan &plan, const KParams<R> &P, void *partials, hipStream_t s);
template <typename R> MergeStep plan_merge(const void *recs, const void *heads, int n, int group, int T, void *out, void *out_heads);
template <typename R> void launch_merge(const MergeStep &m, int T, double beta, hipStream_t s);
template <typename R> KernelLaunch plan_finalize(const FinalizeParams &F, bool abi_recs, bool lookback);
void launch_finalize(const KernelLaunch &k, const FinalizeParams &F, hipStream_t s);
void launch_exchange_probe(const FinalizeParams &F, int *ok_out, hipStream_t s);
enum { EVAL_TRANSITION = 0, EVAL_COST_STAGE = 1, EVAL_COST_TERMINAL = 2, EVAL_COLLIDED = 3, EVAL_CLAMP = 4 };
template <typename R>
void launch_eval_index(const KParams<R> &P, const R *xy, int stride, int n, int p0, int sequential, int *idx_out, int *p_out,
                       hipStream_t s);
template <typename R>
void launch_eval(const KParams<R> &P, int what, const R *x, const R *v, const int *idx, int n, R *out, hipStream_t s);
template <typename R> void launch_eval_filter(const R *xx, R *out, int T, int W, int mode, hipStream_t s);
void launch_eval_weights(const double *S, int n, double beta, double *w, hipStream_t s);
template <typename R> void launch_set_state_dev(const KParams<R> &P, const double *x_dev, int nx, hipStream_t s);
template <typename R> void launch_weights(const KParams<R> &P, double rho, double eta, double *w_out, hipStream_t s);
void launch_sample(unsigned seed_lo, unsigned seed_hi, unsigned iter, int K, int T, int k_offset, const float *chol,
                   float *eps_out, hipStream_t s, unsigned stream_word = 0);
template <typename R>
void launch_viz(const KParams<R> &P, const R *u_before, const R *u_after_pre_shift, long long iter, float *opt,
                float *smp, hipStream_t s);
int reduce_blocks(int K, int traj_per_block);
struct MlpViz;
RolloutPlan plan_mlp(const KParams<float> &P, const MlpParams &Q, const Switches &sw, const MlpViz *viz = nullptr);
void launch_mlp(const RolloutPlan &plan, const KParams<float> &P, const MlpParams &Q, const MlpParams *models, void *partials,
                const MlpViz *viz, hipStream_t s);
void launch_viz_mlp(const KParams<float> &P, const MlpParams &Q, const Switches &sw, const float *u_before, const float *u_upd,
                    long long iter, float *opt, float *smp, hipStream_t s);
void launch_eval_mlp(const KParams<float> &P, const MlpParams &Q, const Switches &sw, const float *x, const float *v, int n,
                     float *out, hipStream_t s);
int mlp_blocks(int K, int tile);
void pack_linear(const float *w, int n_in, float *packed, int n_out = 512);
void pack_linear_h3(const float *w, int n_in, unsigned short *packed, int n_out = 512);
constexpr int MODEL_DIFF_MLP = 2;

}
```

### dnn-mppi-mpc_amd/csrc/mppi_kernels.hip

```cpp
#include <hip/hip_runtime.h>
#include <limits.h>
#include <math.h>

#include "mppi_device.h"

#ifdef MPPI_STAMPS
namespace mppi {
__device__ unsigned long long g_stamps[128];
}
#define STAMP(n)                                                                 \
    do {                                                                         \
        if (blockIdx.x == gridDim.x - 1 && threadIdx.x == 0) g_stamps[64 + (n)] = wall_clock64(); \
        if (blockIdx.x == 0 && threadIdx.x == 0) {                               \
            g_stamps[n] = wall_clock64();                                        \
            if ((n) < 8) g_stamps[40 + (n)] = clock64();  \
            if ((n) == 16 || (n) == 21) g_stamps[32 + (n)] = clock64();           \
        }                                                                        \
    } while (0)
#else
#define STAMP(n) \
    do {         \
    } while (0)
#endif

#include "mppi_merge.h"

namespace mppi {

template <typename R>
__device__ __forceinline__ void x0_call(DevState *st, const R *ref, int n_ref, int window, int sequential, int lane,
                                        double x, double y, int p) {
    const int c = nearest_x0(ref, p, window_len<R>(window, n_ref, p), x, y, lane);
    if (lane == 0) {
        st->c = c;
        st->idx_start = c;
        st->path_end = c >= n_ref - 1;
        if (!sequential) st->p = c;
        st->k_start = 0;
        st->first_k = NO_TRIGGER;
        st->round = 0;
    }
}

template <typename R>
__global__ __launch_bounds__(64) void k_set_state(const R *ref, int n_ref, int window, int sequential, DevState *st,
                                                  double x0, double x1, double x2, double x3, int have_x,
                                                  const AgentScene *scenes) {
    const int lane = threadIdx.x;
    st += blockIdx.x;
    if (scenes) {
        ref = reinterpret_cast<const R *>(scenes[blockIdx.x].ref);
        n_ref = scenes[blockIdx.x].n_ref;
    }
    if (have_x) {
        if (lane == 0) { st->x0[0] = x0; st->x0[1] = x1; st->x0[2] = x2; st->x0[3] = x3; }
    } else {
        x0 = st->x0[0];
        x1 = st->x0[1];
    }
    x0_call<R>(st, ref, n_ref, window, sequential, lane, x0, x1, st->p);
}

template <typename R, int MODEL, bool OBS = true, bool PLAIN = false> struct Rollout {
    __device__ __forceinline__ bool use_philox() const { return PLAIN || P.use_philox; }
    __device__ __forceinline__ bool clamp_rollout() const { return PLAIN || P.clamp_rollout; }
    __device__ __forceinline__ bool wrap_stage() const { return !PLAIN && P.wrap_stage; }
    __device__ __forceinline__ bool wrap_term() const { return !PLAIN && P.wrap_term; }
    const KParams<R> &P;
    const int k, lane, c;
    const unsigned iter;
    const bool exploit;
    R cx, cy, cyaw, cvel;
    int p;
    bool slow;
    bool hit_seen = false;
    bool doomed = false;
    int *sh_first = nullptr;
    R s_acc, s_last;
    const int n_chunk, lane_last;
    const RefPair<R> *win;
    const ObsLanes<R> obs;
    const int agent;

    __device__ __forceinline__ Rollout(const KParams<R> &P_, const DevState &sv, int k_, int lane_,
                                       const RefPair<R> *win_, const ObsLanes<R> &obs_, int agent_ = 0)
        : P(P_), k(k_), lane(lane_), c(sv.c), iter((unsigned)sv.iter),
          exploit((k_ + P_.k_offset) < P_.n_exploit), cx((R)sv.x0[0]), cy((R)sv.x0[1]), cyaw((R)sv.x0[2]),
          cvel(MODEL == MODEL_RACE ? (R)sv.x0[3] : R(0)), p(sv.c), slow(false), s_acc(0), s_last(0),
          n_chunk((P_.T + 63) >> 6), lane_last((P_.T - 1) & 63), win(win_), obs(obs_), agent(agent_) {}

    __device__ __forceinline__ void load_eps(int ch, float &e0, float &e1) const {
        const int t = ch * 64 + lane;
        e0 = 0.f;
        e1 = 0.f;
        if (t < P.T) noise_at(P, use_philox(), iter, agent, k, t, e0, e1);
    }

    struct Step { R x, y, yaw, vel, u0, u1, v0, v1; bool act; };
    __device__ __forceinline__ Step dynamics(int ch, float &e0, float &e1) {
        const int t = ch * 64 + lane;
        const bool act = t < P.T;
        STAMP(8);
        load_eps(ch, e0, e1);
        STAMP(9);
        R u0 = 0, u1 = 0;
        if (act) {
            const R *u = P.u + (size_t)agent * 2 * P.T;
            u0 = u[2 * t];
            u1 = u[2 * t + 1];
        }
        R v0 = exploit ? u0 + (R)e0 : (R)e0, v1 = exploit ? u1 + (R)e1 : (R)e1;
        if (clamp_rollout()) {
            v0 = mf::clamp(v0, P.umax0);
            v1 = mf::clamp(v1, P.umax1);
        }
        if (!act) { v0 = 0; v1 = 0; }

        R x, y, yaw, vel = 0;
        if (MODEL == MODEL_DIFF) {
            const R dyaw = v1 * P.dt;
            yaw = cyaw + wv::scan_incl<wv::OpAdd>(dyaw);
            const R yaw_b = wv::shift_up1(yaw, cyaw);
            R sn, cs;
            mf::sincos_(yaw_b, sn, cs);
            x = cx + wv::scan_incl<wv::OpAdd>(v0 * cs * P.dt);
            y = cy + wv::scan_incl<wv::OpAdd>(v0 * sn * P.dt);
        } else {
            const R dvel = act ? v1 * P.dt : R(0);
            vel = cvel + wv::scan_incl<wv::OpAdd>(dvel);
            const R vel_b = wv::shift_up1(vel, cvel);
            const R dyaw = act ? vel_b / P.wheel_base * mf::tan_(v0) * P.dt : R(0);
            yaw = cyaw + wv::scan_incl<wv::OpAdd>(dyaw);
            const R yaw_b = wv::shift_up1(yaw, cyaw);
            R sn, cs;
            mf::sincos_(yaw_b, sn, cs);
            x = cx + wv::scan_incl<wv::OpAdd>(act ? vel_b * cs * P.dt : R(0));
            y = cy + wv::scan_incl<wv::OpAdd>(act ? vel_b * sn * P.dt : R(0));
        }
        cx = wv::read_lane(x, 63);
        cy = wv::read_lane(y, 63);
        cyaw = wv::read_lane(yaw, 63);
        if (MODEL == MODEL_RACE) cvel = wv::read_lane(vel, 63);
        STAMP(10);
        return Step{x, y, yaw, vel, u0, u1, v0, v1, act};
    }

    __device__ __forceinline__ void chunk(int ch, float &e0, float &e1) {
        const R *__restrict__ ref = P.ref;
        const Step sp = dynamics(ch, e0, e1);
        const R x = sp.x, y = sp.y, yaw = sp.yaw, vel = sp.vel, u0 = sp.u0, u1 = sp.u1, v0 = sp.v0, v1 = sp.v1;
        const bool act = sp.act;
        int my_idx;
        if (P.per_rollout) {
            slow = window_len<R>(P.window, P.n_ref, p) > 1;
            doomed = false;
// ... 1001 lines not shown
        }
        if (P.clamp_rollout) {
            v00 = mf::clamp(v00, P.umax0); v01 = mf::clamp(v01, P.umax1);
            v10 = mf::clamp(v10, P.umax0); v11 = mf::clamp(v11, P.umax1);
        }
        if (!a0) { v00 = 0; v01 = 0; }
        if (!a1) { v10 = 0; v11 = 0; }
        const R d0 = v01 * P.dt, d1 = v11 * P.dt;
        const R yb0 = yaw_0 + wv::shift_up1_half(wv::scan_incl_half<wv::OpAdd>(d0 + d1), R(0));
        const R yw0 = yb0 + d0, yw1 = yw0 + d1;
        R s0, c0, s1, c1;
        mf::sincos_(yb0, s0, c0);
        mf::sincos_(yw0, s1, c1);
        const R dx0 = v00 * c0 * P.dt, dx1 = v10 * c1 * P.dt, dy0 = v00 * s0 * P.dt, dy1 = v10 * s1 * P.dt;
        const R px0 = x_0 + wv::shift_up1_half(wv::scan_incl_half<wv::OpAdd>(dx0 + dx1), R(0)) + dx0, px1 = px0 + dx1;
        const R py0 = y_0 + wv::shift_up1_half(wv::scan_incl_half<wv::OpAdd>(dy0 + dy1), R(0)) + dy0, py1 = py0 + dy1;
        const R lx_l = sub_last ? px1 : px0, ly_l = sub_last ? py1 : py0, lyaw_l = sub_last ? yw1 : yw0;
        const R lx = h ? wv::read_lane(lx_l, 32 + lane_last) : wv::read_lane(lx_l, lane_last);
        const R ly = h ? wv::read_lane(ly_l, 32 + lane_last) : wv::read_lane(ly_l, lane_last);
        const R lyaw = h ? wv::read_lane(lyaw_l, 32 + lane_last) : wv::read_lane(lyaw_l, lane_last);
        R wx, wy, wyaw;
        {
            const R ddx = lx - cand_x, ddy = ly - cand_y;
            const R d = l32 < wlen ? ddx * ddx + ddy * ddy : R(INFINITY);
            const R ms = wv::scan_incl_half<wv::OpMin>(d);
            const R m = h ? wv::read_lane(ms, 63) : wv::read_lane(ms, 31);
            const int js = wv::scan_incl_half<wv::OpMinInt>(d == m ? l32 : 0x7fffffff);
            const int ja = wv::read_lane(js, 31), jb = wv::read_lane(js, 63);
            wx = h ? wv::read_lane(cand_x, jb) : wv::read_lane(cand_x, ja);
            wy = h ? wv::read_lane(cand_y, jb) : wv::read_lane(cand_y, ja);
            wyaw = h ? wv::read_lane(cand_yaw, jb) : wv::read_lane(cand_yaw, ja);
        }
        auto track = [&](const R (&w)[4], bool wrap) {
            const R yw = wrap ? mf::pymod(lyaw + P.two_pi, P.two_pi) : lyaw;
            const R ex = lx - wx, ey = ly - wy, eyaw = yw - wyaw;
            return w[0] * (ex * ex) + w[1] * (ey * ey) + w[2] * (eyaw * eyaw);
        };
        const bool hit = OBS ? collided<false>(P, lx, ly, lyaw, obs) : false;
        R st_c = track(P.ws, P.wrap_stage);
        if (hit) st_c += P.penalty;
        const R va = sub_last ? v10 : v00, vb = sub_last ? v11 : v01;
        const R ctrl_l = ca * va + cb * vb;
        const R ctrl = h ? wv::read_lane(ctrl_l, 32 + lane_last) : wv::read_lane(ctrl_l, lane_last);
        R term = track(P.wt, P.wrap_term);
        if (hit) term += P.penalty;
        const R S_k = (st_c + P.gamma * ctrl) + term;
        if (l32 == 0 && valid) S_[k] = S_k;
        if (OBS && valid && hit) hit_h += R(1);
        if (valid) {
            const R rho_new = fmin(rho_h, S_k);
            const R scale = rho_h < R(INFINITY) ? mf::exp_(-P.beta * (rho_h - rho_new)) : R(0);
            const R e_w = mf::exp_(-P.beta * (S_k - rho_new));
            const float4 e = *reinterpret_cast<const float4 *>(&sh_raw[sidx][4 * l32]);
            w0 = w0 * scale + e_w * (R)e.x; w1 = w1 * scale + e_w * (R)e.y;
            w2 = w2 * scale + e_w * (R)e.z; w3 = w3 * scale + e_w * (R)e.w;
            eta_h = eta_h * scale + e_w;
            eta2_h = eta2_h * scale * scale + e_w * e_w;
            rho_h = rho_new;
        }
    }
    if (l32 == 0) sh_rho[sidx] = rho_h;
    __syncthreads();
    const R rho = wv::read_lane(wv::scan_incl_half<wv::OpMin>(sh_rho[l32]), 31);
    const R sc = rho_h < R(INFINITY) ? mf::exp_(-P.beta * (rho_h - rho)) : R(0);
    if (l32 == 0) { sh_eta[sidx][0] = sc * eta_h; sh_eta[sidx][1] = sc * sc * eta2_h; sh_eta[sidx][2] = hit_h; }
    *reinterpret_cast<VecT4<R> *>(&sh_acc[sidx][4 * l32]) = VecT4<R>{sc * w0, sc * w1, sc * w2, sc * w3};
    __syncthreads();
    const size_t slot = (size_t)agent * P.slots + blockIdx.x;
    R *out = partials + slot * record_len(T, (int)sizeof(R));
    if (tid < 2 * T) {
        R acc = 0;
#pragma unroll
        for (int q = 0; q < ROWS; ++q) acc += sh_acc[q][tid];
        out[4 + tid] = acc;
    }
    if (tid == 64 * (DUAL_WAVES - 1)) record_head(P, out, slot, rho, sh_eta);
}

template <typename R>
__global__ __launch_bounds__(256) void k_reduce(const KParams<R> P, R *__restrict__ partials) {
    extern __shared__ __attribute__((aligned(16))) char smem[];
    const DevState *st = P.st;
    if (round_unresolved(st, P.K)) return;
    const int tid = threadIdx.x, lane = tid & 63, wid = tid >> 6, nw = blockDim.x >> 6;
    const int k0 = blockIdx.x * P.traj_per_block, k1 = min(P.K, k0 + P.traj_per_block), nk = k1 - k0;
    R *sh_e = reinterpret_cast<R *>(smem);
    R *sh_red = sh_e + P.traj_per_block;
    R *sh_acc = sh_red + 16;
    const unsigned iter = (unsigned)st->iter;

    R m = R(INFINITY);
    for (int i = tid; i < nk; i += blockDim.x) m = fmin(m, P.S[k0 + i]);
    m = wv::reduce<wv::OpMin>(m);
    if (lane == 0) sh_red[wid] = m;
    __syncthreads();
    R rho = sh_red[0];
    for (int w = 1; w < nw; ++w) rho = fmin(rho, sh_red[w]);
    __syncthreads();

    R eta = 0, eta2 = 0, n_hit = 0;
    for (int i = tid; i < nk; i += blockDim.x) {
        const R e = mf::exp_(-P.beta * (P.S[k0 + i] - rho));
        sh_e[i] = e;
        eta += e;
        eta2 += e * e;
        if (P.obstacle_model != OBS_NONE && P.S[k0 + i] >= P.penalty) n_hit += R(1);
    }
    eta = wv::reduce<wv::OpAdd>(eta);
    eta2 = wv::reduce<wv::OpAdd>(eta2);
    n_hit = wv::reduce<wv::OpAdd>(n_hit);
    if (lane == 0) { sh_red[4 + wid] = eta; sh_red[8 + wid] = eta2; sh_red[12 + wid] = n_hit; }
    __syncthreads();
    R *out = partials + (size_t)blockIdx.x * record_len(P.T, (int)sizeof(R));
    if (tid == 0) {
        R a = 0, b = 0, nh = 0;
        for (int w = 0; w < nw; ++w) { a += sh_red[4 + w]; b += sh_red[8 + w]; nh += sh_red[12 + w]; }
        out[0] = rho;
        out[1] = a;
        out[2] = b;
        *reinterpret_cast<VecT4<R> *>(P.heads + 4 * (size_t)blockIdx.x) = VecT4<R>{rho, a, b, nh};
    }

    const int n_chunk = (P.T + 63) >> 6;
    for (int ch = 0; ch < n_chunk; ++ch) {
        const int t = ch * 64 + lane;
        R a0 = 0, a1 = 0;
        if (t < P.T) {
            for (int i = wid; i < nk; i += nw) {
                float e0, e1;
                noise_at(P, (bool)P.use_philox, iter, 0, k0 + i, t, e0, e1);
                const R w = sh_e[i];
                a0 += w * (R)e0;
                a1 += w * (R)e1;
            }
        }
        sh_acc[wid * 128 + 2 * lane] = a0;
        sh_acc[wid * 128 + 2 * lane + 1] = a1;
        __syncthreads();
        if (tid < 128 && ch * 64 + (tid >> 1) < P.T) {
            R s = 0;
            for (int w = 0; w < nw; ++w) s += sh_acc[w * 128 + tid];
            out[4 + ch * 128 + tid] = s;
        }
        __syncthreads();
    }
}

template <typename R>
__global__ void k_weights(const R *__restrict__ S, int K, double beta, double rho, double eta, double *w) {
    const int k = blockIdx.x * blockDim.x + threadIdx.x;
    if (k < K) w[k] = exp(-beta * ((double)S[k] - rho)) / eta;
}

template <typename A, bool ABI_OUT>
__global__ __launch_bounds__(MERGE_THREADS) void k_merge(const A *__restrict__ recs, const A *__restrict__ heads, int n,
                                                         int group, int T, A beta, void *__restrict__ out,
                                                         A *__restrict__ out_heads) {
    extern __shared__ __attribute__((aligned(16))) char smem[];
    const MergeLds<A> L(smem, T, 0);
    A *sh_w = L.w;
    const int b0 = blockIdx.x * group, nb = min(group, n - b0);
    const A *mine = recs + (size_t)b0 * record_len(T, (int)sizeof(A));
    MergeRegs<A, MERGE_THREADS, 1> mr;
    merge_load_heads<A, MERGE_THREADS, 1>(heads + 4 * (size_t)b0, mr);
    merge_load_tile<A, MERGE_THREADS, 1>(mine, T, 0, mr);
    A rho, eta, eta2, n_hit = 0;
    merge_combine<A, MERGE_THREADS, 1>(mine, nb, T, beta, mr, L.s, L.part, rho, eta, eta2, [&](int i, A v) { sh_w[i] = v; }, &n_hit);
    if (ABI_OUT) {
        double *o = reinterpret_cast<double *>(out) + (size_t)blockIdx.x * partial_len(T);
        for (int i = threadIdx.x; i < 2 * T; i += MERGE_THREADS) o[3 + i] = (double)(sh_w[i] * eta);
        if (threadIdx.x == 0) { o[0] = (double)rho; o[1] = (double)eta; o[2] = (double)eta2; }
    } else {
        A *o = reinterpret_cast<A *>(out) + (size_t)blockIdx.x * record_len(T, (int)sizeof(A));
        for (int i = threadIdx.x; i < 2 * T; i += MERGE_THREADS) o[4 + i] = sh_w[i] * eta;
        if (threadIdx.x == 0) {
            o[0] = rho; o[1] = eta; o[2] = eta2;
            *reinterpret_cast<VecT4<A> *>(out_heads + 4 * (size_t)blockIdx.x) = VecT4<A>{rho, eta, eta2, n_hit};
        }
    }
}

__device__ __forceinline__ char *peer_base(unsigned long long peer_ptr, int p) {
    const unsigned lo = (unsigned)__builtin_amdgcn_readlane((int)(unsigned)peer_ptr, p);
    const unsigned hi = (unsigned)__builtin_amdgcn_readlane((int)(unsigned)(peer_ptr >> 32), p);
    return reinterpret_cast<char *>(((unsigned long long)hi << 32) | lo);
}
__device__ __forceinline__ unsigned long long load_peer_ptrs(const FinalizeParams &F) {
    const int lane = threadIdx.x & 63;
    return lane < F.x_nranks ? reinterpret_cast<unsigned long long>(F.x_peers[lane]) : 0ull;
}

__device__ __forceinline__ bool exchange_flags(const FinalizeParams &F, unsigned long long peer_ptr, size_t slot_off) {
    const int tid = threadIdx.x;
    char *own = peer_base(peer_ptr, F.x_rank);
    __syncthreads();
    if (tid < F.x_nranks) {
        long long *theirs = reinterpret_cast<long long *>(reinterpret_cast<char *>(peer_ptr) + slot_off) + F.x_rank;
        __hip_atomic_store(theirs, F.x_seq, __ATOMIC_RELEASE, __HIP_MEMORY_SCOPE_SYSTEM);
        const long long *mine = reinterpret_cast<const long long *>(own + slot_off) + tid;
        const unsigned long long t0 = wall_clock64();
        while (__hip_atomic_load(mine, __ATOMIC_RELAXED, __HIP_MEMORY_SCOPE_SYSTEM) != F.x_seq) {
            if (wall_clock64() - t0 > (unsigned long long)F.x_timeout) {
                __hip_atomic_store(F.x_err, 1, __ATOMIC_RELAXED, __HIP_MEMORY_SCOPE_AGENT);
                break;
            }
            __builtin_amdgcn_s_sleep(2);
        }
        __builtin_amdgcn_fence(__ATOMIC_ACQUIRE, "");
    }
    __syncthreads();
    return __hip_atomic_load(F.x_err, __ATOMIC_RELAXED, __HIP_MEMORY_SCOPE_AGENT) == 0;
}

__global__ __launch_bounds__(64) void k_exchange_probe(const FinalizeParams F, int *ok_out) {
    const int tid = threadIdx.x, n_chk = 8;
    const size_t slot_off = (size_t)(F.x_seq & 1) * xchg_slot_bytes(F.T, F.x_nranks);
    const size_t recs_off = slot_off + sizeof(long long) * XCHG_MAX_RANKS;
    auto pattern = [&](int rank, int i) { return (double)(F.x_seq * 4096 + rank * 64 + i); };
    const unsigned long long peer_ptr = load_peer_ptrs(F);
    for (int p = 0; p < F.x_nranks; ++p) {
        double *rec = reinterpret_cast<double *>(peer_base(peer_ptr, p) + recs_off) + (size_t)F.x_rank * xchg_rec_len(F.T);
        if (tid < n_chk) rec[tid] = pattern(F.x_rank, tid);
    }
    bool ok = exchange_flags(F, peer_ptr, slot_off);
    const double *recs = reinterpret_cast<const double *>(peer_base(peer_ptr, F.x_rank) + recs_off);
    bool match = true;
    for (int r = 0; r < F.x_nranks; ++r)
        if (tid < n_chk) match &= recs[(size_t)r * xchg_rec_len(F.T) + tid] == pattern(r, tid);
    ok = ok && __ballot(!match) == 0ull;
    if (tid == 0) *ok_out = ok ? 1 : 0;
}

template <typename A, int MODE, int NT, int NWIN, bool PLAIN = false, bool HYPK = false>
__device__ __forceinline__ void finalize_body(const void *partials_pre, const void *heads_pre, const DevState *st_pre,
                                              const void *u_pre, int T_pre, const FinalizeParams &F, char *smem,
                                              int agent) {
    constexpr bool ABI_RECS = MODE == 1, XCHG = MODE == 2;
    const bool f_use_args = !PLAIN && F.use_args, f_sequential = PLAIN || F.sequential, f_plant = PLAIN || F.plant;
    const bool f_raise = !PLAIN && F.raise_at_path_end, f_clamp_u = !PLAIN && F.clamp_u, f_trace = !PLAIN && F.u0_trace != nullptr;
    const int f_model = PLAIN ? (int)MODEL_DIFF : F.model, f_filter = PLAIN ? (int)FILTER_DIFF : F.filter_mode;
    static_assert(MODE == 0 || NT == MERGE_THREADS, "the ABI / exchange variants are 256-thread kernels");
    const int tid = threadIdx.x, lane = tid & 63, wid = tid >> 6;
    const int T = F.T, W = F.filter_window;
    const MergeLds<A, NT> L(smem, T, W);
    A *sh_w = L.w;
    A *sh_u = L.u;
    DevState *st_out = F.st_out + agent;
    StepResult *res = reinterpret_cast<StepResult *>(reinterpret_cast<char *>(F.res) + (size_t)agent * F.res_stride);
    double *res_u = reinterpret_cast<double *>(res + 1);
    const A *u_in = reinterpret_cast<const A *>(u_pre);
    A *u_out = reinterpret_cast<A *>(F.u_out) + (size_t)agent * 2 * T;
    A *u_hist = reinterpret_cast<A *>(F.u_before) + (size_t)agent * 4 * T;
    const int *pout = F.pout + (size_t)agent * F.K;
    const void *partials = partials_pre;
    const A *ref = reinterpret_cast<const A *>(F.ref);

    STAMP(16);
    static_assert(sizeof(DevState) == 72, "DevState layout");
    const int st_word = reinterpret_cast<const int *>(st_pre)[lane < 18 ? lane : 0];
    const A u_old = tid < 2 * T_pre ? u_in[tid] : A(0);
    unsigned long long peer_ptr = 0;
    if (XCHG) peer_ptr = load_peer_ptrs(F);
    MergeRegs<A, NT, NWIN> mr;
    constexpr int HW = HYP_MAX_BLOCKS / 256;
    uint4 hwords[HW];
#pragma unroll
    for (int i = 0; i < HW; ++i) {
        hwords[i] = uint4{0, 0, 0, 0};
        if (HYPK && 4 * (lane + 64 * i) < F.hyp_blocks) hwords[i] = reinterpret_cast<const uint4 *>(F.hyp_slots)[lane + 64 * i];
    }
    if (!ABI_RECS) {
        merge_load_heads<A, NT, NWIN>(reinterpret_cast<const A *>(heads_pre), mr);
        merge_load_tile<A, NT, NWIN>(reinterpret_cast<const A *>(partials_pre), T_pre, 0, mr);
    }
    STAMP(24);
    DevState sv;
    {
        auto word = [&](int i) { return __builtin_amdgcn_readlane(st_word, i); };
        auto dbl = [&](int i) {
            return __builtin_bit_cast(double, ((long long)word(i + 1) << 32) | (unsigned int)word(i));
        };
        sv.x0[0] = dbl(0); sv.x0[1] = dbl(2); sv.x0[2] = dbl(4); sv.x0[3] = dbl(6);
        sv.p = word(8); sv.c = word(9); sv.k_start = word(10); sv.first_k = word(11);
        sv.round = word(12); sv.path_end = word(13); sv.idx_start = word(14); sv.pad = 0;
        sv.iter = ((long long)word(17) << 32) | (unsigned int)word(16);
    }
    const int fk = sv.first_k, round = sv.round;
    const bool args = f_use_args && round == 0;
    const int c_state = args ? F.c_arg : sv.c;
    const int p_state = (args && !f_sequential) ? F.c_arg : sv.p;
    const int idx_start = args ? F.c_arg : sv.idx_start, path_end = args ? (F.c_arg >= F.n_ref - 1) : sv.path_end;
    const long long iter = sv.iter;
    const double x0v[4] = {args ? F.x0_arg[0] : sv.x0[0], args ? F.x0_arg[1] : sv.x0[1],
                           args ? F.x0_arg[2] : sv.x0[2], args ? F.x0_arg[3] : sv.x0[3]};
    DevState nx = sv;
    nx.x0[0] = x0v[0]; nx.x0[1] = x0v[1]; nx.x0[2] = x0v[2]; nx.x0[3] = x0v[3];
    nx.c = c_state; nx.p = p_state; nx.idx_start = idx_start; nx.path_end = path_end;
    nx.first_k = NO_TRIGGER;
    auto publish = [&]() {
        __syncthreads();
        if (tid == 0 && F.seq) {
            __threadfence_system();
            *reinterpret_cast<volatile long long *>(&res->seq) = F.seq;
        }
    };
    auto leave = [&]() {
        if (tid == 0) *st_out = nx;
        if (u_out != u_in)
            for (int i = tid; i < 2 * T; i += NT) u_out[i] = i == tid ? u_old : u_in[i];
        publish();
    };

    if (XCHG && *reinterpret_cast<volatile int *>(F.x_err)) {
        if (tid == 0) { res->status = STATUS_EXCHANGE_FAILED; res->iter = iter; }
        return leave();
    }
    int c_final = c_state;
    bool hyp_done = false;
    if (HYPK) {
        static_assert(!HYPK || (MODE == 0 && NWIN <= 2 && NT == MERGE_THREADS), "the resolution is part of the plain 256-thread finalize");
        const bool hyp_round = round == 0 && min(F.window, F.n_ref - c_state) > 1;
        if (hyp_round) {
            const unsigned tag = lb_tag(F.lb_seq);
            int mx = 0;
            bool bd = false;
#pragma unroll
            for (int i = 0; i < HW; ++i) {
                const unsigned hw[4] = {hwords[i].x, hwords[i].y, hwords[i].z, hwords[i].w};
#pragma unroll
                for (int j = 0; j < 4; ++j) {
                    if (4 * (lane + 64 * i) + j < F.hyp_blocks) {
                        bd |= (hw[j] & LB_TAG_MASK) != tag || (hw[j] & LB_BAD) != 0u;
                        mx = max(mx, (int)(hw[j] & (LB_BAD - 1)));
                    }
                }
            }
            const int lb_max = wv::reduce<wv::OpMaxInt>(mx);
            const bool lb_bad = __ballot(bd) != 0ull;
            if (lb_bad) {
                nx.k_start = 0;
                nx.c = c_state;
                nx.round = round + 1;
                if (tid == 0) {
                    res->status = STATUS_NEED_ROUND;
                    res->k_next = 0;
                    res->c_next = c_state;
                    res->rounds = round + 1;
                    res->iter = iter;
                }
                return leave();
            }
            c_final = c_state + lb_max;
            hyp_done = true;
        }
    }
    if (!hyp_done && f_sequential && fk != NO_TRIGGER) {
        const int c_new = pout[fk];
        if (fk + 1 < F.K) {
            nx.k_start = fk + 1;
            nx.c = c_new;
            nx.round = round + 1;
            if (tid == 0) {
                res->status = STATUS_NEED_ROUND;
                res->k_next = fk + 1;
                res->c_next = c_new;
                res->rounds = round + 1;
                res->iter = iter;
            }
            return leave();
        }
        c_final = c_new;
    }
    const int p_now = f_sequential ? c_final : p_state;

    A cand_x = 0, cand_y = 0;
    const int wlen_next = min(F.window, F.n_ref - p_now);
    if (wid == 0 && f_plant && lane < wlen_next) {
        cand_x = ref[4 * (p_now + lane)];
        cand_y = ref[4 * (p_now + lane) + 1];
    }
    A sn_yaw = 0, cs_yaw = 1;
    if (f_plant) mf::sincos_((A)x0v[2], sn_yaw, cs_yaw);
    STAMP(17);

    const bool pad_copy = f_filter == FILTER_RACE || f_filter == FILTER_TORCH;
    auto store_w = [&](int i, A v) { filter_store<A>(sh_w, i, v, T, W, pad_copy); };
    A rho, eta, eta2;
    A n_hit = A(-1);
    const bool count_hits = F.count_hits != 0;
    if (ABI_RECS) {
        merge_abi<A>(reinterpret_cast<const double *>(F.partials), F.n_part, T, (A)F.beta, L.s, L.red, rho, eta, eta2,
                     store_w);
    } else if (!XCHG) {
        if (count_hits) n_hit = A(0);
        merge_combine<A, NT, NWIN>(reinterpret_cast<const A *>(partials), F.n_part, T, (A)F.beta, mr, L.s, L.part, rho,
                                   eta, eta2, store_w, &n_hit);
        if (!count_hits) n_hit = A(0);
    } else {
        merge_combine<A, NT, NWIN>(reinterpret_cast<const A *>(partials), F.n_part, T, (A)F.beta, mr, L.s, L.part, rho,
                                   eta, eta2, [&](int i, A v) { sh_u[i] = v; });
        const size_t slot_off = (size_t)(F.x_seq & 1) * xchg_slot_bytes(T, F.x_nranks);
        const size_t rec_off = slot_off + sizeof(long long) * XCHG_MAX_RANKS + sizeof(double) * (size_t)F.x_rank * xchg_rec_len(T);
        for (int p = 0; p < F.x_nranks; ++p) {
            double *rec = reinterpret_cast<double *>(peer_base(peer_ptr, p) + rec_off);
            for (int i = tid; i < 2 * T; i += NT) rec[3 + i] = (double)(sh_u[i] * eta);
            if (tid == 0) { rec[0] = (double)rho; rec[1] = (double)eta; rec[2] = (double)eta2; }
        }
        __builtin_amdgcn_fence(__ATOMIC_RELEASE, "");
        if (!exchange_flags(F, peer_ptr, slot_off)) {
            if (tid == 0) {
                res->status = STATUS_EXCHANGE_FAILED;
                res->rounds = round + 1; res->iter = iter;
            }
            return leave();
        }
        const double *recs = reinterpret_cast<const double *>(peer_base(peer_ptr, F.x_rank) + slot_off + sizeof(long long) * XCHG_MAX_RANKS);
        if (F.x_nranks <= XCHG_LDS_RANKS) {
            double *sh_x = reinterpret_cast<double *>(smem + sizeof(A) * merge_lds_elems(T, W, sizeof(A), NT));
            const int tot = F.x_nranks * xchg_rec_len(T);
            for (int i = tid; i < tot; i += NT) sh_x[i] = recs[i];
            __syncthreads();
            recs = sh_x;
        }
        merge_abi<A>(recs, F.x_nranks, T, (A)F.beta, L.s, L.red, rho, eta, eta2, store_w, xchg_rec_len(T));
    }
    STAMP(18);

    if (f_raise && path_end) {
        nx.k_start = 0;
        nx.round = 0;
        if (tid == 0) {
            res->status = STATUS_PATH_END;
            res->idx_start = idx_start; res->idx_after = p_state; res->path_end = 1;
            res->rounds = round + 1; res->iter = iter;
        }
        return leave();
    }

    for (int i = tid; i < 2 * T; i += NT) {
        const int t = i >> 1, d = i & 1;
        const A f = filter_at<A>(sh_w, t, d, T, W, f_filter);
        const A uo = i == tid ? u_old : u_in[i];
        A un = uo + f;
        if (f_clamp_u) un = mf::clamp(un, d == 0 ? (A)F.umax0 : (A)F.umax1);
        sh_u[i] = un;
    }
    __syncthreads();
    STAMP(19);
    for (int i = tid; i < 2 * T; i += NT) {
        const int t = i >> 1, d = i & 1;
        const A uo = i == tid ? u_old : u_in[i];
        const A shifted = sh_u[2 * (t < T - 1 ? t + 1 : T - 1) + d];
        u_hist[i] = uo;
        u_hist[2 * T + i] = sh_u[i];
        res_u[i] = (double)shifted;
        u_out[i] = shifted;
    }

    STAMP(20);
    if (wid == 0) {
        const A u0a = sh_u[2 * (T > 1 ? 1 : 0)], u0b = sh_u[2 * (T > 1 ? 1 : 0) + 1];
        double xn[4] = {x0v[0], x0v[1], x0v[2], x0v[3]};
        if (f_plant) {
            if (f_model == MODEL_DIFF) {
                xn[0] += (double)(u0a * cs_yaw) * F.dt;
                xn[1] += (double)(u0a * sn_yaw) * F.dt;
                xn[2] += (double)u0b * F.dt;
            } else {
                const A steer = mf::clamp(u0a, (A)F.umax0), accel = mf::clamp(u0b, (A)F.umax1);
                const double v = xn[3];
                xn[0] += v * (double)cs_yaw * F.dt;
                xn[1] += v * (double)sn_yaw * F.dt;
                xn[2] += v / F.wheel_base * (double)mf::tan_(steer) * F.dt;
                xn[3] += (double)accel * F.dt;
            }
        }
        nx.iter = iter + 1;
        nx.k_start = 0;
        nx.round = 0;
        nx.p = p_now;
        if (lane == 0) {
            res->status = STATUS_DONE;
            res->k_next = 0; res->c_next = c_final;
            res->idx_start = idx_start;
            res->idx_after = p_now;
            res->path_end = path_end;
            res->rounds = round + 1;
            res->costs_hyp = hyp_done ? 1 : 0;
            res->n_collided = (int)n_hit;
            res->rho = (double)rho; res->eta = (double)eta; res->ess = (double)(eta * eta / eta2);
            res->u0[0] = (double)u0a; res->u0[1] = (double)u0b;
            for (int q = 0; q < 4; ++q) res->x_next[q] = xn[q];
            if (f_trace && agent == 0) { F.u0_trace[2 * iter] = (double)u0a; F.u0_trace[2 * iter + 1] = (double)u0b; }
            res->iter = iter + 1;
        }
        if (f_plant) {
            double best = INFINITY;
            int bj = INT_MAX;
            if (lane < wlen_next) {
                const double dx = xn[0] - (double)cand_x, dy = xn[1] - (double)cand_y;
                best = dx * dx + dy * dy;
                bj = lane;
            }
            for (int j = lane + 64; j < wlen_next; j += 64) {
                const double dx = xn[0] - (double)ref[4 * (p_now + j)], dy = xn[1] - (double)ref[4 * (p_now + j) + 1];
                const double dd = dx * dx + dy * dy;
                if (dd < best) { best = dd; bj = j; }
            }
            wv::argmin_first(best, bj);
            const int c = p_now + bj;
            nx.x0[0] = xn[0]; nx.x0[1] = xn[1]; nx.x0[2] = xn[2]; nx.x0[3] = xn[3];
            nx.c = c;
            nx.idx_start = c;
            nx.path_end = c >= F.n_ref - 1;
            if (!f_sequential) nx.p = c;
        }
        if (lane == 0) *st_out = nx;
    }
    publish();
    STAMP(21);
}

template <typename A, int MODE, int NWIN, bool MULTI, bool PLAIN = false, bool HYPK = false>
__global__ __launch_bounds__(MERGE_THREADS) void k_finalize(const void *partials_pre, const void *heads_pre,
                                                            const DevState *st_pre, const void *u_pre, int T_pre,
                                                            const FinalizeParams F) {
    extern __shared__ __attribute__((aligned(16))) char smem[];
    if (MULTI) {
        const int a = blockIdx.y;
        const AgentScene sc = F.scenes[a];
        FinalizeParams Fa = F;
        Fa.ref = sc.ref;
        Fa.n_ref = sc.n_ref;
        Fa.count_hits = F.count_hits && sc.n_obs > 0;
        const size_t rec = (size_t)a * F.slots * record_len(T_pre, (int)sizeof(A));
        finalize_body<A, MODE, MERGE_THREADS, NWIN>(reinterpret_cast<const A *>(partials_pre) + rec,
                                                    reinterpret_cast<const A *>(heads_pre) + (size_t)a * F.slots * 4,
                                                    st_pre + a, reinterpret_cast<const A *>(u_pre) + (size_t)a * 2 * T_pre,
                                                    T_pre, Fa, smem, a);
    } else {
        finalize_body<A, MODE, MERGE_THREADS, NWIN, PLAIN, HYPK>(partials_pre, heads_pre, st_pre, u_pre, T_pre, F, smem, 0);
    }
}

__global__ void k_sample(unsigned seed_lo, unsigned seed_hi, unsigned iter, int K, int T, int k_offset, float l00,
                         float l10, float l11, float *__restrict__ eps, unsigned stream_word) {
    const size_t i = (size_t)blockIdx.x * blockDim.x + threadIdx.x;
    if (i >= (size_t)K * T) return;
    const int k = (int)(i / T), t = (int)(i % T);
    const float chol[3] = {l00, l10, l11};
    float e0, e1;
    px::sample(seed_lo, seed_hi, iter, (unsigned)(k + k_offset), t, chol, e0, e1, stream_word);
    reinterpret_cast<float2 *>(eps)[i] = make_float2(e0, e1);
}

template <typename R, int MODEL>
__global__ __launch_bounds__(256) void k_viz(const KParams<R> P, const R *__restrict__ u_before,
                                             const R *__restrict__ u_upd, unsigned iter, float *__restrict__ opt,
                                             float *__restrict__ smp) {
    const int lane = threadIdx.x & 63;
    const int row = blockIdx.x * (blockDim.x >> 6) + (threadIdx.x >> 6) - 1;
    if (row >= P.K) return;
    if (row < 0 && !opt) return;
    if (row >= 0 && !smp) return;
    const DevState *st = P.st;
    constexpr int NX = MODEL == MODEL_RACE ? 4 : 3;
    R cx = (R)st->x0[0], cy = (R)st->x0[1], cyaw = (R)st->x0[2], cvel = MODEL == MODEL_RACE ? (R)st->x0[3] : R(0);
    const bool exploit = (row + P.k_offset) < P.n_exploit;
    float *dst = row < 0 ? opt : smp + (size_t)row * P.T * NX;
    const int n_chunk = (P.T + 63) >> 6;
    for (int ch = 0; ch < n_chunk; ++ch) {
        const int t = ch * 64 + lane;
        const bool act = t < P.T;
        const int tc = (t + P.T - 1) % P.T;
        R v0 = 0, v1 = 0;
        if (act) {
            if (row < 0) {
                v0 = mf::clamp(u_upd[2 * tc], P.umax0);
                v1 = mf::clamp(u_upd[2 * tc + 1], P.umax1);
            } else {
                float e0, e1;
                noise_at(P, (bool)P.use_philox, iter, 0, row, tc, e0, e1);
                perturb_clamp(P, exploit, true, u_before[2 * tc], u_before[2 * tc + 1], e0, e1, v0, v1);
            }
        }
        R x, y, yaw, vel = 0;
        if (MODEL == MODEL_DIFF) {
            yaw = cyaw + wv::scan_incl<wv::OpAdd>(v1 * P.dt);
            const R yaw_b = wv::shift_up1(yaw, cyaw);
            R sn, cs;
            mf::sincos_(yaw_b, sn, cs);
            x = cx + wv::scan_incl<wv::OpAdd>(v0 * cs * P.dt);
            y = cy + wv::scan_incl<wv::OpAdd>(v0 * sn * P.dt);
        } else {
            vel = cvel + wv::scan_incl<wv::OpAdd>(act ? v1 * P.dt : R(0));
            const R vel_b = wv::shift_up1(vel, cvel);
            yaw = cyaw + wv::scan_incl<wv::OpAdd>(act ? vel_b / P.wheel_base * mf::tan_(v0) * P.dt : R(0));
            const R yaw_b = wv::shift_up1(yaw, cyaw);
            R sn, cs;
            mf::sincos_(yaw_b, sn, cs);
            x = cx + wv::scan_incl<wv::OpAdd>(act ? vel_b * cs * P.dt : R(0));
            y = cy + wv::scan_incl<wv::OpAdd>(act ? vel_b * sn * P.dt : R(0));
        }
        cx = wv::read_lane(x, 63); cy = wv::read_lane(y, 63); cyaw = wv::read_lane(yaw, 63);
        if (MODEL == MODEL_RACE) cvel = wv::read_lane(vel, 63);
        if (act) {
            dst[(size_t)t * NX] = (float)x;
            dst[(size_t)t * NX + 1] = (float)y;
            dst[(size_t)t * NX + 2] = (float)yaw;
            if (MODEL == MODEL_RACE) dst[(size_t)t * NX + 3] = (float)vel;
        }
    }
}

template <typename R>
__global__ __launch_bounds__(64) void k_eval_index(const R *__restrict__ ref, int n_ref, int window, const R *__restrict__ xy,
                                                   int stride, int n, int p0, int sequential, int *__restrict__ idx_out,
                                                   int *__restrict__ p_out) {
    const int lane = threadIdx.x;
    if (sequential) {
        int p = p0;
        for (int i = 0; i < n; ++i) {
            p = nearest_uniform(ref, p, window_len<R>(window, n_ref, p), xy[(size_t)i * stride], xy[(size_t)i * stride + 1], lane);
            if (lane == 0) idx_out[i] = p;
        }
        if (lane == 0) *p_out = p;
    } else {
        const int i = blockIdx.x * 64 + lane;
        if (i < n) idx_out[i] = nearest_in_window(ref, p0, window_len<R>(window, n_ref, p0), xy[(size_t)i * stride], xy[(size_t)i * stride + 1]);
        if (i == 0) *p_out = p0;
    }
}

template <typename R, int MODEL>
__global__ __launch_bounds__(256) void k_eval(const KParams<R> P, int what, const R *__restrict__ x, const R *__restrict__ v,
                                              const int *__restrict__ idx, int n, R *__restrict__ out) {
    constexpr int NX = MODEL == MODEL_RACE ? 4 : 3;
    const int lane = threadIdx.x & 63, i = blockIdx.x * blockDim.x + threadIdx.x;
    const ObsLanes<R> obs = load_obstacles(P, lane);
    const bool act = i < n;
    R s[4] = {R(0), R(0), R(0), R(0)}, v0 = 0, v1 = 0;
    if (act && x)
        for (int q = 0; q < NX; ++q) s[q] = x[(size_t)i * NX + q];
    if (act && v) { v0 = v[2 * (size_t)i]; v1 = v[2 * (size_t)i + 1]; }
    if (what == EVAL_TRANSITION) {
        R sn, cs;
        mf::sincos_(s[2], sn, cs);
        if (MODEL == MODEL_DIFF) {
            s[0] += v0 * cs * P.dt;
            s[1] += v0 * sn * P.dt;
            s[2] += v1 * P.dt;
        } else {
            const R vel = s[3];
            s[0] += vel * cs * P.dt;
            s[1] += vel * sn * P.dt;
            s[2] += vel / P.wheel_base * mf::tan_(v0) * P.dt;
            s[3] += v1 * P.dt;
        }
        if (act)
            for (int q = 0; q < NX; ++q) out[(size_t)i * NX + q] = s[q];
    } else if (what == EVAL_CLAMP) {
        if (act) {
            out[2 * (size_t)i] = mf::clamp(v0, P.umax0);
            out[2 * (size_t)i + 1] = mf::clamp(v1, P.umax1);
        }
    } else {
        const bool hit = collided<MODEL == MODEL_RACE>(P, s[0], s[1], s[2], obs);
        if (what == EVAL_COLLIDED) {
            if (act) out[i] = hit ? R(1) : R(0);
        } else {
            const bool term = what == EVAL_COST_TERMINAL;
            const R c = state_cost_row<R, MODEL>(P, term ? P.wt : P.ws, term ? P.wrap_term : P.wrap_stage,
                                                 P.ref + 4 * (act ? idx[i] : 0), s[0], s[1], s[2], s[3], hit);
            if (act) out[i] = c;
        }
    }
}

template <typename A>
__global__ __launch_bounds__(256) void k_eval_filter(const A *__restrict__ xx, A *__restrict__ out, int T, int W, int f_filter) {
    extern __shared__ __attribute__((aligned(16))) char smem[];
    A *sh_w = reinterpret_cast<A *>(smem);
    const bool pad_copy = f_filter == FILTER_RACE || f_filter == FILTER_TORCH;
    for (int i = threadIdx.x; i < 2 * T; i += blockDim.x) filter_store<A>(sh_w, i, xx[i], T, W, pad_copy);
    __syncthreads();
    for (int i = threadIdx.x; i < 2 * T; i += blockDim.x) out[i] = filter_at<A>(sh_w, i >> 1, i & 1, T, W, f_filter);
}

__global__ __launch_bounds__(256) void k_eval_weights(const double *__restrict__ S, int n, double beta, double *__restrict__ w) {
    __shared__ double sh[8];
    const int tid = threadIdx.x, lane = tid & 63, wid = tid >> 6;
    double m = INFINITY;
    for (int i = tid; i < n; i += 256) m = fmin(m, S[i]);
    m = wv::reduce<wv::OpMin>(m);
// ... 35 lines not shown
}
template <bool PLAIN, bool SHARE> static KernelLaunch tri_entry() {
    static KernelEntry e("k_rollout_tri<%s, %s>", KernelEntry::of(PLAIN), KernelEntry::of(SHARE));
    return plan_entry(reinterpret_cast<const void *>(k_rollout_tri<PLAIN, SHARE>), e, 64 * DUAL_WAVES);
}
template <typename R, bool MULTI, bool OBS, bool PHILOX> static KernelLaunch stream_entry() {
    static KernelEntry e("k_rollout_stream<%s, %s, %s, %s>", type_name<R>(), KernelEntry::of(MULTI), KernelEntry::of(OBS),
                                 KernelEntry::of(PHILOX));
    return plan_entry(reinterpret_cast<const void *>(k_rollout_stream<R, MULTI, OBS, PHILOX>), e, 64 * DUAL_WAVES);
}

int reduce_blocks(int K, int traj_per_block) { return (K + traj_per_block - 1) / traj_per_block; }

template <typename R> void launch_set_state(const KParams<R> &P, const double *x, hipStream_t s) {
    const int agents = x ? 1 : (P.n_agents > 1 ? P.n_agents : 1);
    const double z[4] = {0, 0, 0, 0};
    const double *v = x ? x : z;
    hipLaunchKernelGGL(k_set_state<R>, dim3(agents), dim3(64), 0, s, P.ref, P.n_ref, P.window, P.sequential, P.st, v[0],
                       v[1], v[2], v[3], x ? 1 : 0, agents > 1 ? P.scenes : (const AgentScene *)nullptr);
}

bool fused_supported(int T) { return T <= 128; }
static bool dual_layout(const Switches &sw, int K, int T, int n_agents) {
    if (T > 64) return false;
    if (sw.dual >= 0) return sw.dual != 0;
    return (long long)K * n_agents >= 8192;
}
static bool pair_layout(const Switches &sw, int T) {
    if (T <= 64 || T > 128) return false;
    if (sw.pair >= 0) return sw.pair != 0;
    return true;
}
static bool tri_layout(const Switches &sw, int T, bool tri_ok) {
    if (!tri_ok || T <= 64 || T > 32 * TRI_STEPS) return false;
    if (sw.tri >= 0) return sw.tri != 0;
    return true;
}
int rollout_layout(const Switches &sw, int K, int T, int n_agents, int model, bool f64, bool per_rollout, bool tri_ok) {
    if (!per_rollout && model == MODEL_RACE && !f64 && n_agents <= 1 && tri_layout(sw, T, tri_ok)) return LAYOUT_TRI;
    const int kind = per_rollout ? LAYOUT_FUSED : dual_layout(sw, K, T, n_agents) ? LAYOUT_DUAL : pair_layout(sw, T) ? LAYOUT_PAIR : LAYOUT_FUSED;
    if (kind == LAYOUT_FUSED) return kind;
    const int blocks = fused_blocks(K, T, kind);
    const bool shares_cu = kind == LAYOUT_DUAL && model == MODEL_DIFF && !f64;
    bool twice = blocks > (shares_cu ? 512 : 256) && blocks <= 1024;
    if (sw.seq >= 0) twice = sw.seq == 2;
    return kind | (twice ? LAYOUT_TWICE : 0);
}
int fused_blocks(int K, int T, int layout) {
    const int kind = layout & LAYOUT_KIND;
    const int per_block = ((kind == LAYOUT_DUAL || kind == LAYOUT_TRI) ? DUAL_SAMPLES : FUSED_WAVES) * (layout & LAYOUT_TWICE ? 2 : 1);
    return (K + per_block - 1) / per_block;
}

static int stream_batches(int K) { return (K + DUAL_SAMPLES - 1) / DUAL_SAMPLES; }
template <typename R> static int stream_passes(const KParams<R> &P, const Switches &sw) {
    if (P.model != MODEL_DIFF || P.sequential || P.accumulate || P.T > 64 || P.window > 32 ||
        (P.layout & LAYOUT_KIND) != LAYOUT_DUAL)
        return 0;
    if (sw.no_stream) return 0;
    const long long batches = (long long)stream_batches(P.K) * (P.n_agents > 1 ? P.n_agents : 1);
    if (sw.stream_passes > 0) return sw.stream_passes;
    int np = (int)(batches / 1024);
    return np < 1 ? 1 : np > 16 ? 16 : np;
}
int fused_max_records(int K, int T, int layout) {
    const int blocks = fused_blocks(K, T, layout), batches = (layout & LAYOUT_KIND) == LAYOUT_DUAL ? stream_batches(K) : 0;
    return blocks > batches ? blocks : batches;
}

template <typename R, int MODEL, bool MULTI, int SPW> static KernelLaunch dual_plan(bool twice, bool plain, bool lb) {
    if constexpr (!MULTI && MODEL == MODEL_DIFF && SPW == 2)
        if (lb) return plain ? dual_entry<R, MODEL_DIFF, 2, false, 1, true, true>() : dual_entry<R, MODEL_DIFF, 2, false, 1, false, true>();
    if constexpr (!MULTI)
        if (plain) return twice ? dual_entry<R, MODEL, SPW, false, 2, true>() : dual_entry<R, MODEL, SPW, false, 1, true>();
    if constexpr (MULTI && SPW == 2)
        if (plain && !twice) return dual_entry<R, MODEL, 2, true, 1, true>();
    return twice ? dual_entry<R, MODEL, SPW, MULTI, 2, false>() : dual_entry<R, MODEL, SPW, MULTI, 1, false>();
}
template <typename R, int MODEL, int NCH, bool MULTI, bool HYPK> static KernelLaunch fused_plan(int spec) {
    return spec == 2   ? fused_entry<R, MODEL, NCH, MULTI, 2, HYPK>()
           : spec == 1 ? fused_entry<R, MODEL, NCH, MULTI, 1, HYPK>()
                       : fused_entry<R, MODEL, NCH, MULTI, 0, HYPK>();
}
template <typename R, int MODEL, bool MULTI> static RolloutPlan plan_fused(const KParams<R> &P, const Switches &sw) {
    RolloutPlan p;
    if (const int np = stream_passes(P, sw)) {
        const bool obs = P.obstacle_model != OBS_NONE;
        p.k = P.use_philox ? (obs ? stream_entry<R, MULTI, true, true>() : stream_entry<R, MULTI, false, true>())
                           : (obs ? stream_entry<R, MULTI, true, false>() : stream_entry<R, MULTI, false, false>());
        p.passes = np;
        p.records = (stream_batches(P.K) + np - 1) / np;
        p.k.grid = dim3(p.records, MULTI ? P.n_agents : 1);
        return p;
    }
    const int blocks = fused_blocks(P.K, P.T, P.layout);
    const bool twice = (P.layout & LAYOUT_TWICE) != 0;
    const bool race = MODEL == MODEL_RACE;
    const bool plain_ok = P.use_philox && P.clamp_rollout && (bool)P.wrap_stage == race && (bool)P.wrap_term == race;
    switch (P.layout & LAYOUT_KIND) {
    case LAYOUT_DUAL:
        p.lookback = !MULTI && MODEL == MODEL_DIFF && P.hyp && !twice;
        p.k = dual_plan<R, MODEL, MULTI, 2>(twice, plain_ok, p.lookback);
        break;
    case LAYOUT_PAIR: p.k = dual_plan<R, MODEL, MULTI, 1>(twice, plain_ok, false); break;
    case LAYOUT_TRI:
        if constexpr (sizeof(R) == 4 && MODEL == MODEL_RACE && !MULTI) {
            const bool share = blocks > 256;
            p.k = plain_ok ? (share ? tri_entry<true, true>() : tri_entry<true, false>())
                           : (share ? tri_entry<false, true>() : tri_entry<false, false>());
        }
        break;
    default:
        {
            const bool plain = P.obstacle_model == OBS_NONE && P.use_philox && P.clamp_rollout && !P.wrap_stage && !P.wrap_term &&
                               !P.per_rollout;
            const int spec = plain ? 2 : P.obstacle_model == OBS_NONE ? 1 : 0;
            p.lookback = !MULTI && MODEL == MODEL_DIFF && P.hyp && P.T <= 64;
            p.k = p.lookback  ? fused_plan<R, MODEL_DIFF, 1, false, true>(spec)
                  : P.T <= 64 ? fused_plan<R, MODEL, 1, MULTI, false>(spec)
                              : fused_plan<R, MODEL, 2, MULTI, false>(spec);
        }
    }
    p.records = blocks;
    p.k.grid = dim3(blocks, MULTI ? P.n_agents : 1);
    return p;
}

template <typename R> RolloutPlan plan_rollout(const KParams<R> &P, bool fused, const Switches &sw) {
    const bool diff = P.model == MODEL_DIFF;
    if (fused) {
        if (P.n_agents > 1) return diff ? plan_fused<R, MODEL_DIFF, true>(P, sw) : plan_fused<R, MODEL_RACE, true>(P, sw);
        return diff ? plan_fused<R, MODEL_DIFF, false>(P, sw) : plan_fused<R, MODEL_RACE, false>(P, sw);
    }
    RolloutPlan p;
    p.k = diff ? rollout_entry<R, MODEL_DIFF>() : rollout_entry<R, MODEL_RACE>();
    p.k.grid = dim3((P.K + 3) / 4);
    p.records = reduce_blocks(P.K, P.traj_per_block);
    return p;
}
template <typename R> void launch_rollout(const RolloutPlan &plan, const KParams<R> &P, void *partials, hipStream_t s) {
    const DevState *st = P.st;
    int n_pass = plan.passes;
    void *args[] = {&st, const_cast<KParams<R> *>(&P), &partials, &n_pass};
    launch_plan(plan.k, args, s);
}

template <typename R> void launch_reduce(const KParams<R> &P, void *partials, int n_blocks, hipStream_t s) {
    const size_t shmem = sizeof(R) * ((size_t)P.traj_per_block + 16 + 4 * 128);
    hipLaunchKernelGGL(k_reduce<R>, dim3(n_blocks), dim3(256), shmem, s, P, (R *)partials);
}

static size_t merge_lds(int T, int W, size_t elem) { return elem * merge_lds_elems(T, W, elem); }

template <typename R, bool ABI_OUT> static KernelLaunch merge_entry() {
    static KernelEntry e("k_merge<%s, %s>", type_name<R>(), KernelEntry::of(ABI_OUT));
    return plan_entry(reinterpret_cast<const void *>(k_merge<R, ABI_OUT>), e, MERGE_THREADS);
}
template <typename R> MergeStep plan_merge(const void *recs, const void *heads, int n, int group, int T, void *out, void *out_heads) {
    MergeStep m;
    m.k = out_heads ? merge_entry<R, false>() : merge_entry<R, true>();
    m.k.grid = dim3((n + group - 1) / group);
    m.k.lds = merge_lds(T, 0, sizeof(R));
    m.recs = recs, m.heads = heads, m.n = n, m.group = group, m.out = out, m.out_heads = out_heads;
    return m;
}
template <typename R> void launch_merge(const MergeStep &m, int T, double beta, hipStream_t s) {
    R b = (R)beta;
    void *args[] = {const_cast<const void **>(&m.recs), const_cast<const void **>(&m.heads), const_cast<int *>(&m.n),
                    const_cast<int *>(&m.group), &T, &b, const_cast<void **>(&m.out), const_cast<void **>(&m.out_heads)};
    launch_plan(m.k, args, s);
}

template <typename R, int MODE, int NWIN, bool MULTI, bool PLAIN = false, bool HYPK = false> static KernelLaunch finalize_entry() {
    static KernelEntry e("k_finalize<%s, %d, %d, %s, %s, %s>", type_name<R>(), MODE, NWIN, KernelEntry::of(MULTI), KernelEntry::of(PLAIN),
                         KernelEntry::of(HYPK));
    return plan_entry(reinterpret_cast<const void *>(k_finalize<R, MODE, NWIN, MULTI, PLAIN, HYPK>), e, MERGE_THREADS);
}
template <typename R> KernelLaunch plan_finalize(const FinalizeParams &F, bool abi_recs, bool lookback) {
    const bool two = merge_tree(F.n_part, true).windows > 1;
    const bool multi = !abi_recs && F.x_nranks <= 1 && F.n_agents > 1;
    const bool plain = F.sequential && F.plant && !F.use_args && !F.raise_at_path_end && !F.clamp_u && F.model == MODEL_DIFF &&
                       !F.u0_trace && F.filter_mode == FILTER_DIFF;
    KernelLaunch k = abi_recs         ? finalize_entry<R, 1, 1, false>()
                     : F.x_nranks > 1 ? (two ? finalize_entry<R, 2, 2, false>() : finalize_entry<R, 2, 1, false>())
                     : multi          ? (two ? finalize_entry<R, 0, 2, true>() : finalize_entry<R, 0, 1, true>())
                     : two            ? (lookback ? finalize_entry<R, 0, 2, false, false, true>() : finalize_entry<R, 0, 2, false>())
                     : lookback       ? (plain ? finalize_entry<R, 0, 1, false, true, true>() : finalize_entry<R, 0, 1, false, false, true>())
                                      : (plain ? finalize_entry<R, 0, 1, false, true, false>() : finalize_entry<R, 0, 1, false>());
    k.grid = dim3(1, multi ? F.n_agents : 1);
    k.lds = merge_lds(F.T, F.filter_window, sizeof(R)) + (F.x_nranks > 1 ? sizeof(double) * XCHG_LDS_RANKS * xchg_rec_len(F.T) : 0) +
            (lookback ? (size_t)HYP_MAX_BLOCKS + 16 : 0);
    return k;
}
void launch_finalize(const KernelLaunch &k, const FinalizeParams &F, hipStream_t s) {
    const DevState *st = F.st;
    void *args[] = {const_cast<const void **>(&F.partials), const_cast<const void **>(&F.heads), &st, const_cast<void **>(&F.u),
                    const_cast<int *>(&F.T), const_cast<FinalizeParams *>(&F)};
    launch_plan(k, args, s);
}

void launch_exchange_probe(const FinalizeParams &F, int *ok_out, hipStream_t s) {
    hipLaunchKernelGGL(k_exchange_probe, dim3(1), dim3(64), 0, s, F, ok_out);
}

template <typename R>
void launch_eval_index(const KParams<R> &P, const R *xy, int stride, int n, int p0, int sequential, int *idx_out, int *p_out,
                       hipStream_t s) {
    hipLaunchKernelGGL(k_eval_index<R>, dim3(sequential ? 1 : (n + 63) / 64), dim3(64), 0, s, P.ref, P.n_ref, P.window, xy,
                       stride, n, p0, sequential, idx_out, p_out);
}
template <typename R>
void launch_eval(const KParams<R> &P, int what, const R *x, const R *v, const int *idx, int n, R *out, hipStream_t s) {
    const dim3 grid((n + 255) / 256), block(256);
    if (P.model == MODEL_DIFF) hipLaunchKernelGGL((k_eval<R, MODEL_DIFF>), grid, block, 0, s, P, what, x, v, idx, n, out);
    else hipLaunchKernelGGL((k_eval<R, MODEL_RACE>), grid, block, 0, s, P, what, x, v, idx, n, out);
}
template <typename R> void launch_eval_filter(const R *xx, R *out, int T, int W, int mode, hipStream_t s) {
    hipLaunchKernelGGL(k_eval_filter<R>, dim3(1), dim3(256), sizeof(R) * 2 * (size_t)(T + W + 2), s, xx, out, T, W, mode);
}
void launch_eval_weights(const double *S, int n, double beta, double *w, hipStream_t s) {
    hipLaunchKernelGGL(k_eval_weights, dim3(1), dim3(256), 0, s, S, n, beta, w);
}
template <typename R> void launch_set_state_dev(const KParams<R> &P, const double *x_dev, int nx, hipStream_t s) {
    hipLaunchKernelGGL(k_set_state_dev<R>, dim3(1), dim3(64), 0, s, P.ref, P.n_ref, P.window, P.sequential, P.st, x_dev, nx);
}

template <typename R> void launch_weights(const KParams<R> &P, double rho, double eta, double *w, hipStream_t s) {
    hipLaunchKernelGGL(k_weights<R>, dim3((P.K + 255) / 256), dim3(256), 0, s, P.S, P.K, (double)P.beta, rho, eta, w);
}

void launch_sample(unsigned seed_lo, unsigned seed_hi, unsigned iter, int K, int T, int k_offset, const float *chol,
                   float *eps_out, hipStream_t s, unsigned stream_word) {
    const size_t n = (size_t)K * T;
    hipLaunchKernelGGL(k_sample, dim3((unsigned)((n + 255) / 256)), dim3(256), 0, s, seed_lo, seed_hi, iter, K, T,
                       k_offset, chol[0], chol[1], chol[2], eps_out, stream_word);
}

template <typename R>
void launch_viz(const KParams<R> &P, const R *u_before, const R *u_upd, long long iter, float *opt, float *smp,
                hipStream_t s) {
    const int rows = P.K + 1, blocks = (rows + 3) / 4;
    if (P.model == MODEL_DIFF)
        hipLaunchKernelGGL((k_viz<R, MODEL_DIFF>), dim3(blocks), dim3(256), 0, s, P, u_before, u_upd, (unsigned)iter,
                           opt, smp);
    else
        hipLaunchKernelGGL((k_viz<R, MODEL_RACE>), dim3(blocks), dim3(256), 0, s, P, u_before, u_upd, (unsigned)iter,
                           opt, smp);
}

#ifdef MPPI_STAMPS
extern "C" int mppi_debug_stamps(unsigned long long *out, int n) {
    return (int)hipMemcpyFromSymbol(out, HIP_SYMBOL(g_stamps), sizeof(unsigned long long) * (n < 128 ? n : 128));
}
#endif

#define INSTANTIATE(R)                                                                                    \
    template void launch_set_state<R>(const KParams<R> &, const double *, hipStream_t);                   \
    template RolloutPlan plan_rollout<R>(const KParams<R> &, bool, const Switches &);                     \
    template void launch_rollout<R>(const RolloutPlan &, const KParams<R> &, void *, hipStream_t);        \
    template void launch_reduce<R>(const KParams<R> &, void *, int, hipStream_t);                         \
    template MergeStep plan_merge<R>(const void *, const void *, int, int, int, void *, void *);             \
    template void launch_merge<R>(const MergeStep &, int, double, hipStream_t);                           \
    template KernelLaunch plan_finalize<R>(const FinalizeParams &, bool, bool);                           \
    template void launch_weights<R>(const KParams<R> &, double, double, double *, hipStream_t);           \
    template void launch_eval_index<R>(const KParams<R> &, const R *, int, int, int, int, int *, int *, hipStream_t); \
    template void launch_eval<R>(const KParams<R> &, int, const R *, const R *, const int *, int, R *, hipStream_t);   \
    template void launch_eval_filter<R>(const R *, R *, int, int, int, hipStream_t);                                 \
    template void launch_set_state_dev<R>(const KParams<R> &, const double *, int, hipStream_t);                     \
    template void launch_viz<R>(const KParams<R> &, const R *, const R *, long long, float *, float *, hipStream_t);
INSTANTIATE(float)
INSTANTIATE(double)

}
```

### dnn-mppi-mpc_amd/csrc/mppi_merge.h

```cpp
#pragma once
#include <hip/hip_runtime.h>
#include <math.h>

#include "mppi_device.h"

#ifndef STAMP
#define STAMP(n) \
    do {         \
    } while (0)
#endif

namespace mppi {

template <int NT> struct MergeShape {
    static constexpr int GROUPS = NT / 32, MAXJ = MERGE_MAX_RECORDS / GROUPS, WAVES = NT / 64;
};

template <typename A> struct alignas(16) VecT { A v[16 / sizeof(A)]; };

template <typename A, int NT = MERGE_THREADS> struct MergeLds {
    A *w, *u, *s, *red, *part;
    __device__ __forceinline__ MergeLds(char *smem, int T, int W) {
        w = reinterpret_cast<A *>(smem);
        u = w + ((2 * (T + W + 1) + 3) & ~3);
        s = u + ((2 * T + 3) & ~3);
        red = s + MERGE_MAX_WINDOWS * NT;
        part = red + 64;
    }
};

__device__ __forceinline__ float fast_exp(float x) { return __expf(x); }
__device__ __forceinline__ double fast_exp(double x) { return exp(x); }
__device__ __forceinline__ float fast_div(float a, float b) { return a * __builtin_amdgcn_rcpf(b); }
__device__ __forceinline__ double fast_div(double a, double b) { return a / b; }

template <typename A> __device__ __forceinline__ void filter_store(A *sh_w, int i, A v, int T, int W, bool pad_copy) {
    const int t = i >> 1, d = i & 1, H = W / 2;
    const A pv = pad_copy ? v : A(0);
    sh_w[2 * (t + H) + d] = v;
    if (t < H) sh_w[2 * t + d] = pv;
    if (t >= T - (W - H)) sh_w[2 * (t + W) + d] = pv;
}
template <typename A> __device__ __forceinline__ A filter_at(const A *sh_w, int t, int d, int T, int W, int f_filter) {
    const int H = W / 2;
    const A inv_w = fast_div(A(1), (A)W);
    if (f_filter == FILTER_NONE) return sh_w[2 * (t + H) + d];
    if (f_filter == FILTER_TORCH) {
        A sacc = 0;
        for (int q = 0; q < W; ++q) {
            const int m = t - H + q;
            if (m >= 0) sacc += sh_w[2 * m + d] * inv_w;
        }
        return sacc;
    }
    const A *tap = sh_w + 2 * t + d;
    A sacc = 0;
    if (W == 10) {
#pragma unroll
        for (int q = 0; q < 10; ++q) sacc += tap[2 * (9 - q)] * inv_w;
    } else {
        for (int q = 0; q < W; ++q) sacc += tap[2 * (W - 1 - q)] * inv_w;
    }
    if (f_filter == FILTER_DIFF) {
        const int n_conv = (W + 1) / 2;
        if (t == 0) sacc *= fast_div((A)W, (A)n_conv);
        else if (t < n_conv) sacc *= fast_div((A)W, (A)(t + n_conv));
        if (t == T - 1)
            for (int q = 1; q < n_conv; ++q) sacc *= fast_div((A)W, (A)(q + n_conv - (W % 2)));
    }
    return sacc;
}

template <typename A> struct BlockRed {
    static __device__ __forceinline__ A min1(A v, A *sh, int tid) {
        v = wv::reduce<wv::OpMin>(v);
        __syncthreads();
        if ((tid & 63) == 0) sh[tid >> 6] = v;
        __syncthreads();
        A r = sh[0];
#pragma unroll
        for (int w = 1; w < MERGE_THREADS / 64; ++w) r = fmin(r, sh[w]);
        return r;
    }
    static __device__ __forceinline__ void add2(A &a, A &b, A *sh, int tid) {
        a = wv::reduce<wv::OpAdd>(a);
        b = wv::reduce<wv::OpAdd>(b);
        __syncthreads();
        if ((tid & 63) == 0) { sh[tid >> 6] = a; sh[32 + (tid >> 6)] = b; }
        __syncthreads();
        a = 0;
        b = 0;
#pragma unroll
        for (int w = 0; w < MERGE_THREADS / 64; ++w) { a += sh[w]; b += sh[32 + w]; }
    }
};

template <typename A, int NT = MERGE_THREADS, int NWIN = 1> struct MergeRegs {
    VecT<A> w[NWIN][MergeShape<NT>::MAXJ];
    A hr[4 * NWIN], he[4 * NWIN], he2[4 * NWIN];
    A hc[4 * NWIN];
};

template <typename A, int NT, int NWIN>
__device__ __forceinline__ void merge_load_heads(const A *__restrict__ heads, MergeRegs<A, NT, NWIN> &m) {
    const int lane = threadIdx.x & 63;
#pragma unroll
    for (int i = 0; i < 4 * NWIN; ++i) {
        const int b = lane + 64 * i;
        const size_t r = (size_t)b;
        const VecT4<A> hd = *reinterpret_cast<const VecT4<A> *>(heads + 4 * r);
        m.hr[i] = hd.x;
        m.he[i] = hd.y;
        m.he2[i] = hd.z;
        m.hc[i] = hd.w;
    }
}

template <typename A, int NT, int NWIN>
__device__ __forceinline__ void merge_load_tile(const A *__restrict__ recs, int T, int vt, MergeRegs<A, NT, NWIN> &m) {
    constexpr int VW = 16 / sizeof(A), MAXJ = MergeShape<NT>::MAXJ;
    const int tid = threadIdx.x, vc = tid & 31, grp = tid >> 5;
    const unsigned rbytes = (unsigned)record_len(T, (int)sizeof(A)) * (unsigned)sizeof(A);
    const int nvc = (2 * T + VW - 1) / VW;
    const char *base = reinterpret_cast<const char *>(recs);
    const unsigned col = (unsigned)(4 + min(vt * 32 + vc, nvc - 1) * VW) * (unsigned)sizeof(A);
    const unsigned off0 = (unsigned)(grp * MAXJ) * rbytes + col;
#pragma unroll
    for (int win = 0; win < NWIN; ++win)
#pragma unroll
        for (int j = 0; j < MAXJ; ++j)
            m.w[win][j] = *reinterpret_cast<const VecT<A> *>(base + (off0 + (unsigned)(win * MERGE_MAX_RECORDS + j) * rbytes));
}

template <typename A, int NT, int NWIN, typename Store>
__device__ __forceinline__ void merge_combine(const A *__restrict__ recs, int n, int T, A beta,
                                              MergeRegs<A, NT, NWIN> &m, A *sh_s, A *sh_part, A &rho, A &eta, A &eta2,
                                              Store store, A *n_hit = nullptr) {
    constexpr int VW = 16 / sizeof(A), MAXJ = MergeShape<NT>::MAXJ, GROUPS = MergeShape<NT>::GROUPS;
    using V = VecT<A>;
    const int tid = threadIdx.x, lane = tid & 63, wid = tid >> 6;
    const int vc = tid & 31, grp = tid >> 5;
    const int nvc = (2 * T + VW - 1) / VW;
    A lr = A(INFINITY);
#pragma unroll
    for (int i = 0; i < 4 * NWIN; ++i) {
        if (lane + 64 * i >= n) m.hr[i] = A(INFINITY);
        lr = fmin(lr, m.hr[i]);
    }
    rho = wv::reduce<wv::OpMin>(lr);
    STAMP(25);
    A sc[4 * NWIN];
    eta = 0;
    eta2 = 0;
#pragma unroll
    for (int i = 0; i < 4 * NWIN; ++i) {
        sc[i] = lane + 64 * i < n ? fast_exp(-beta * (m.hr[i] - rho)) : A(0);
        eta += sc[i] * m.he[i];
        eta2 += sc[i] * sc[i] * m.he2[i];
    }
    eta = wv::reduce<wv::OpAdd>(eta);
    eta2 = wv::reduce<wv::OpAdd>(eta2);
    if (n_hit && *n_hit >= A(0)) {
        A cnt = 0;
#pragma unroll
        for (int i = 0; i < 4 * NWIN; ++i) cnt += lane + 64 * i < n ? m.hc[i] : A(0);
        *n_hit = wv::reduce<wv::OpAdd>(cnt);
    }
    const int r0 = wid * 2 * MAXJ, slot = r0 >> 6;
    A *my_s = sh_s + wid * 64;
#pragma unroll
    for (int win = 0; win < NWIN; ++win)
        my_s[win * NT + lane] = slot == 0 ? sc[4 * win] : slot == 1 ? sc[4 * win + 1] : slot == 2 ? sc[4 * win + 2] : sc[4 * win + 3];
    __builtin_amdgcn_fence(__ATOMIC_RELEASE, "wavefront");
    __builtin_amdgcn_wave_barrier();
    __builtin_amdgcn_fence(__ATOMIC_ACQUIRE, "wavefront");
    STAMP(26);
    const A *sj_base = my_s + (r0 & 63) + (grp & 1) * MAXJ;
    const A inv_eta = fast_div(A(1), eta);
    const int n_tiles = (nvc + 31) / 32;
    for (int vt = 0; vt < n_tiles; ++vt) {
        V acc;
#pragma unroll
        for (int q = 0; q < VW; ++q) acc.v[q] = 0;
#pragma unroll
        for (int win = 0; win < NWIN; ++win)
#pragma unroll
            for (int j = 0; j < MAXJ; ++j) {
                const A sj = sj_base[win * NT + j];
#pragma unroll
                for (int q = 0; q < VW; ++q) acc.v[q] += sj * m.w[win][j].v[q];
            }
        if (vt > 0) __syncthreads();
        *reinterpret_cast<V *>(sh_part + (grp * 32 + vc) * VW) = acc;
        __syncthreads();
        if (__builtin_expect(vt + 1 < n_tiles, 0)) merge_load_tile<A, NT, NWIN>(recs, T, vt + 1, m);
        for (int e = tid; e < 32 * VW; e += NT) {
            const int i = vt * 32 * VW + e;
            if (i < 2 * T) {
                A t = 0;
#pragma unroll
                for (int g = 0; g < GROUPS; ++g) t += sh_part[g * 32 * VW + e];
                store(i, t * inv_eta);
            }
        }
    }
    __syncthreads();
}

template <typename A, typename Store>
__device__ __forceinline__ void merge_abi(const double *recs, int n, int T, A beta, A *sh_s, A *sh_red, A &rho, A &eta,
                                          A &eta2, Store store, int stride = 0) {
    const int tid = threadIdx.x, plen = stride ? stride : partial_len(T);
    A hr = A(INFINITY), he = 0, he2 = 0;
    if (tid < n) {
        const double *pb = recs + tid * plen;
        hr = (A)pb[0];
        he = (A)pb[1];
        he2 = (A)pb[2];
    }
    rho = BlockRed<A>::min1(hr, sh_red, tid);
    const A sc = tid < n ? fast_exp(-beta * (hr - rho)) : A(0);
    if (tid < n) sh_s[tid] = sc;
    eta = sc * he;
    eta2 = sc * sc * he2;
    BlockRed<A>::add2(eta, eta2, sh_red, tid);
    const A inv_eta = fast_div(A(1), eta);
    for (int i = tid; i < 2 * T; i += MERGE_THREADS) {
        A t = 0;
        for (int b = 0; b < n; ++b) t += sh_s[b] * (A)recs[b * plen + 3 + i];
        store(i, t * inv_eta);
    }
    __syncthreads();
}

}
```

### dnn-mppi-mpc_amd/engine.py

```python
from __future__ import annotations

import ctypes as C

import numpy as np

from . import _capi as capi


def _dp(a: np.ndarray):
    return a.ctypes.data_as(C.POINTER(C.c_double))


def _dev_ptr(t):
    if t is None:
        return None
    if not t.is_cuda or not t.is_contiguous():
        raise ValueError("expected a contiguous CUDA tensor")
    return C.c_void_p(t.data_ptr())


def _stream_ptr(stream):
    if stream is None:
        return None
    return C.c_void_p(getattr(stream, "cuda_stream", stream))
# ... 194 lines not shown
    def comm_connect(self, rank, handles, local_ptrs=None):
        n = len(handles)
        blob = C.create_string_buffer(b"".join(bytes(hd) for hd in handles))
        lp = None
        if local_ptrs is not None:
            lp = (C.c_void_p * n)(*[C.c_void_p(p) if p else C.c_void_p(None) for p in local_ptrs])
        self._ck(self.lib.mppi_comm_connect(self._h, int(rank), n, blob, lp))

    def comm_probe(self, stream=None):
        self._ck(self.lib.mppi_comm_probe(self._h, _stream_ptr(stream)))

    def comm_close(self):
        self._ck(self.lib.mppi_comm_close(self._h))

    def comm_unique_id(self):
        buf = C.create_string_buffer(self.lib.mppi_comm_unique_id_bytes())
        rc = self.lib.mppi_comm_unique_id(buf)
        if rc != capi.OK:
            raise capi.MppiError(rc, (self.lib.mppi_last_error(None) or b"").decode() or "mppi_comm_unique_id failed")
        return buf.raw

    def comm_init(self, unique_id, rank, nranks):
        buf = C.create_string_buffer(bytes(unique_id), len(unique_id))
        self._ck(self.lib.mppi_comm_init(self._h, buf, int(rank), int(nranks)))

    def step_end(self, partials, nranks, stream=None):
        u, u0 = np.empty((self.T, 2)), np.empty(2)
        self._ck(self.lib.mppi_step_end(self._h, _dev_ptr(partials), int(nranks), _dp(u), _dp(u0),
                                        C.byref(self.stats), _stream_ptr(stream)))
        return u, u0, self.stats

    def costs(self):
        S = np.empty(self._lead + (self.K,))
        self._ck(self.lib.mppi_get_costs(self._h, _dp(S)))
        return S

    def weights(self):
        w = np.empty(self.K)
        self._ck(self.lib.mppi_get_weights(self._h, _dp(w)))
        return w

    def sample_epsilon(self, iteration, out=None, stream=None):
        import torch
        shape = self._lead + (self.K, self.T, 2)
        if out is None:
            out = torch.empty(shape, dtype=torch.float32, device=f"cuda:{self.cfg.device}")
        elif out.dtype != torch.float32 or tuple(out.shape) != shape:
            raise ValueError(f"out must be float32 {list(shape)}")
        self._ck(self.lib.mppi_sample_epsilon(self._h, int(iteration), _dev_ptr(out), _stream_ptr(stream)))
        return out

    def set_noise_ring(self, ring):
        if ring is None:
            self._ck(self.lib.mppi_set_noise_ring(self._h, None, 0))
            self._noise_ring = None
            return
        import torch
        want = self._lead + (self.K, self.T, 2)
        if ring.dtype != torch.float32 or tuple(ring.shape[1:]) != want:
            raise ValueError(f"the noise ring must be float32 [n_slots, {', '.join(map(str, want))}]")
        self._ck(self.lib.mppi_set_noise_ring(self._h, _dev_ptr(ring), int(ring.shape[0])))
        self._noise_ring = ring

    def rollout_viz(self, want_optimal=True, want_sampled=True, stream=None):
        import torch
        dev = f"cuda:{self.cfg.device}"
        opt = torch.empty((self.T, self.nx), dtype=torch.float32, device=dev) if want_optimal else None
        smp = torch.empty((self.K, self.T, self.nx), dtype=torch.float32, device=dev) if want_sampled else None
        self._ck(self.lib.mppi_rollout_viz(self._h, _dev_ptr(opt), _dev_ptr(smp), _stream_ptr(stream)))
        return opt, smp

    @staticmethod
    def _rows(a, ncol):
        a = np.ascontiguousarray(a, dtype=np.float64)
        if a.ndim != 2 or a.shape[1] != ncol:
            raise ValueError(f"expected an [n, {ncol}] array")
        return a

    def eval_state_transition(self, x, v):
        x, v = self._rows(x, self.nx), self._rows(v, 2)
        if v.shape[0] != x.shape[0]:
            raise ValueError("x and v must have the same number of rows")
        out = np.empty_like(x)
        self._ck(self.lib.mppi_eval_state_transition(self._h, _dp(x), _dp(v), x.shape[0], _dp(out)))
        return out

    def eval_clamp(self, v):
        v = self._rows(v, 2)
        out = np.empty_like(v)
        self._ck(self.lib.mppi_eval_clamp(self._h, _dp(v), v.shape[0], _dp(out)))
        return out

    def eval_is_collided(self, x):
        x = self._rows(x, self.nx)
        out = np.empty(x.shape[0])
        self._ck(self.lib.mppi_eval_is_collided(self._h, _dp(x), x.shape[0], _dp(out)))
        return out

    def eval_nearest_waypoint(self, x, prev_idx, update_prev_idx=False):
        x = self._rows(x, self.nx)
        p, idx = C.c_int32(int(prev_idx)), np.empty(x.shape[0], dtype=np.int32)
        self._ck(self.lib.mppi_eval_nearest_waypoint(self._h, _dp(x), x.shape[0], C.byref(p), int(bool(update_prev_idx)),
                                                     idx.ctypes.data_as(C.POINTER(C.c_int32))))
        return idx, p.value

    def eval_cost(self, x, prev_idx, terminal=False, update_prev_idx=False):
        x = self._rows(x, self.nx)
        p, idx, cost = C.c_int32(int(prev_idx)), np.empty(x.shape[0], dtype=np.int32), np.empty(x.shape[0])
        self._ck(self.lib.mppi_eval_cost(self._h, int(bool(terminal)), _dp(x), x.shape[0], C.byref(p),
                                         int(bool(update_prev_idx)), _dp(cost), idx.ctypes.data_as(C.POINTER(C.c_int32))))
        return cost, idx, p.value

    def eval_moving_average(self, xx):
        xx = np.ascontiguousarray(xx, dtype=np.float64)
        if xx.shape != (self.T, 2):
            raise ValueError(f"the filter input must be [{self.T}, 2]")
        out = np.empty_like(xx)
        self._ck(self.lib.mppi_eval_moving_average(self._h, _dp(xx), _dp(out)))
        return out

    def eval_weights(self, S):
        S = np.ascontiguousarray(S, dtype=np.float64).reshape(-1)
        w = np.empty_like(S)
        self._ck(self.lib.mppi_eval_weights(self._h, _dp(S), S.size, _dp(w)))
        return w

    def run_closed_loop(self, n_iters, trace=False, stream=None):
        tr = np.empty((n_iters, 2)) if trace else None
        self._ck(self.lib.mppi_run_closed_loop(self._h, int(n_iters), _dp(tr) if trace else None,
                                               C.byref(self.stats), _stream_ptr(stream)))
        return tr, self.stats

    def enable_timing(self, on=True):
        self._ck(self.lib.mppi_enable_timing(self._h, int(bool(on))))

    def set_rollout_repeats(self, n):
        self._ck(self.lib.mppi_set_rollout_repeats(self._h, int(n)))

    def counters(self):
        out = (C.c_int64 * 3)()
        self._ck(self.lib.mppi_get_counters(self._h, out))
        layout = C.c_int32(-1)
        if hasattr(self.lib, "mppi_get_rollout_layout"):
            self._ck(self.lib.mppi_get_rollout_layout(self._h, C.byref(layout)))
        return {"iterations": out[0], "rollout_launches": out[1], "finalize_launches": out[2], "rollout_layout": layout.value}

    def rollout_kernel(self):
        if not hasattr(self.lib, "mppi_get_rollout_kernel"):
            return ""
        buf = C.create_string_buffer(192)
        self._ck(self.lib.mppi_get_rollout_kernel(self._h, buf, 192))
        return buf.value.decode()

    def host_timing(self):
        out = (C.c_double * 2)()
        self._ck(self.lib.mppi_get_host_timing(self._h, out))
        return {"enqueue_s": out[0], "loop_s": out[1]}

    def time_rollout_launch(self, n_slots=500, extra=2, stream=None):
        out = (C.c_double * 2)()
        self._ck(self.lib.mppi_time_rollout_launch(self._h, int(n_slots), int(extra), _stream_ptr(stream), out))
        return {"rollout_us": out[0], "graph_iteration_us": out[1]}

    def last_kernel_ms(self):
        out = (C.c_float * 4)()
        self._ck(self.lib.mppi_last_kernel_ms(self._h, out))
        return {"rollout": out[0], "reduce": out[1], "finalize": out[2], "event_pair_overhead": out[3]}
```

### include/mppi_hip.h

```cpp
#ifndef MPPI_HIP_H
#define MPPI_HIP_H

#include <stdint.h>

#ifdef __cplusplus
extern "C" {
#endif

#define MPPI_ABI_VERSION 6

typedef enum {
    MPPI_OK = 0,
    MPPI_ERR_BAD_ARG = -1,
    MPPI_ERR_SHAPE = -2,
    MPPI_ERR_NO_DEVICE = -3,
    MPPI_ERR_HIP = -4,
    MPPI_ERR_PATH_END = -5,
    MPPI_ERR_UNSUPPORTED = -6,
    MPPI_ERR_STATE = -7,
    MPPI_ERR_COMM = -8
} mppi_status;

typedef enum {
    MPPI_MODEL_DIFFDRIVE = 0,
    MPPI_MODEL_RACECAR = 1,
    MPPI_MODEL_DIFFDRIVE_MLP = 2
} mppi_model;
typedef enum { MPPI_PREC_F32 = 0, MPPI_PREC_F64 = 1 } mppi_precision;
typedef enum { MPPI_WAYPOINT_SEQUENTIAL = 0, MPPI_WAYPOINT_FROZEN = 1, MPPI_WAYPOINT_PER_ROLLOUT = 2 } mppi_waypoint_mode;
typedef enum { MPPI_BETA_INV_EXPLORATION = 0, MPPI_BETA_INV_LAMBDA = 1, MPPI_BETA_LAMBDA = 2 } mppi_beta_mode;
typedef enum {
    MPPI_FILTER_DIFFDRIVE = 0, MPPI_FILTER_RACECAR = 1, MPPI_FILTER_NONE = 2, MPPI_FILTER_TORCH = 3
} mppi_filter_mode;
typedef enum { MPPI_OBSTACLE_NONE = 0, MPPI_OBSTACLE_CIRCLE = 1, MPPI_OBSTACLE_OUTLINE = 2 } mppi_obstacle_model;

typedef struct {
    int32_t struct_size;
    int32_t device;
    int32_t model;
    int32_t precision;
    int32_t K;
    int32_t T;
    int32_t K_global;
    int32_t k_offset;
    double delta_t;
    double u_max[2];
    double wheel_base;
    double param_exploration, param_lambda, param_alpha;
    double sigma[4];
    double stage_cost_weight[4];
    double terminal_cost_weight[4];
    int32_t beta_mode;
    int32_t accumulate_stage_cost;
    int32_t waypoint_mode;
    int32_t search_window;
    int32_t wrap_yaw_stage;
    int32_t wrap_yaw_terminal;
    int32_t clamp_rollout;
    int32_t clamp_u_after_update;
    int32_t filter_mode;
    int32_t filter_window;
    int32_t obstacle_model;
    int32_t raise_at_path_end;
    double safety_margin;
    double vehicle_w, vehicle_l;
    double collision_penalty;
    uint64_t seed;
    int32_t n_agents;
    int32_t noise_stream;
} mppi_config;

typedef struct {
    double rho;
    double eta;
    double ess;
    int32_t idx_start;
    int32_t idx_after;
    int32_t path_end;
    int32_t rounds;
    int64_t iteration;
    int32_t n_collided;
    int32_t reserved;
    double iter_us;
    double kernel_us;
} mppi_stats;

typedef struct mppi_handle mppi_handle;

int mppi_abi_version(void);
const char *mppi_last_error(const mppi_handle *h);
int mppi_device_count(void);

int mppi_create(const mppi_config *cfg, mppi_handle **out);
int mppi_destroy(mppi_handle *h);

int mppi_set_ref_path(mppi_handle *h, const double *path, int32_t n, int32_t ncols);
int mppi_set_obstacles(mppi_handle *h, const double *xyr, int32_t m);
int mppi_set_agent_ref_path(mppi_handle *h, int32_t agent, const double *path, int32_t n, int32_t ncols);
int mppi_set_agent_obstacles(mppi_handle *h, int32_t agent, const double *xyr, int32_t m);
int mppi_get_agent_status(mppi_handle *h, int32_t *idx_out, int32_t *path_end_out);
int mppi_set_mlp(mppi_handle *h, int32_t hidden, int32_t n_hidden, const float *w_in, const float *b_in,
                 const float *const *w_hidden, const float *const *b_hidden, const float *w_out, const float *b_out);
int mppi_set_mlp_scaled(mppi_handle *h, int32_t hidden, int32_t n_hidden, const float *w_in, const float *b_in,
                        const float *const *w_hidden, const float *const *b_hidden, const float *w_out, const float *b_out,
                        const double *in_mean, const double *in_scale, const double *out_mean, const double *out_scale);
int mppi_set_agent_mlp(mppi_handle *h, int32_t agent, int32_t hidden, int32_t n_hidden, const float *w_in, const float *b_in,
                       const float *const *w_hidden, const float *const *b_hidden, const float *w_out, const float *b_out);
int mppi_set_agent_mlp_scaled(mppi_handle *h, int32_t agent, int32_t hidden, int32_t n_hidden, const float *w_in,
                              const float *b_in, const float *const *w_hidden, const float *const *b_hidden, const float *w_out,
                              const float *b_out, const double *in_mean, const double *in_scale, const double *out_mean,
                              const double *out_scale);
int mppi_set_u_prev(mppi_handle *h, const double *u);
int mppi_get_u_prev(mppi_handle *h, double *u);
int mppi_set_waypoint_idx(mppi_handle *h, int32_t idx);
int mppi_get_waypoint_idx(mppi_handle *h, int32_t *idx);

int mppi_step(mppi_handle *h, const double *x0, const float *eps, double *u_out, double *u0_out,
              mppi_stats *stats, void *stream);

int mppi_step_device_x0(mppi_handle *h, const double *x0_device, const float *eps, double *u_out, double *u0_out,
                        mppi_stats *stats, void *stream);

int mppi_partial_len(const mppi_handle *h, int32_t *n_doubles);
int mppi_step_begin(mppi_handle *h, const double *x0, const float *eps, double *partial, void *stream);
int mppi_step_end(mppi_handle *h, const double *partials, int32_t nranks, double *u_out, double *u0_out,
                  mppi_stats *stats, void *stream);
int mppi_step_end_async(mppi_handle *h, const double *partials, int32_t nranks, void *stream);
int mppi_sync_result(mppi_handle *h, double *u_out, double *u0_out, mppi_stats *stats, void *stream);

int mppi_comm_handle_bytes(void);
int mppi_comm_export(mppi_handle *h, int32_t nranks, void *handle_out);
int mppi_comm_buffer(mppi_handle *h, void **device_ptr);
int mppi_comm_connect(mppi_handle *h, int32_t rank, int32_t nranks, const void *handles ,
                      void *const *local_ptrs );
int mppi_comm_probe(mppi_handle *h, void *stream);
int mppi_comm_close(mppi_handle *h);

int mppi_comm_unique_id_bytes(void);
int mppi_comm_unique_id(void *id_out);
int mppi_comm_init(mppi_handle *h, const void *unique_id, int32_t rank, int32_t nranks);

int mppi_get_costs(mppi_handle *h, double *S);
int mppi_get_weights(mppi_handle *h, double *w);
int mppi_sample_epsilon(mppi_handle *h, int64_t iteration, float *eps_out, void *stream);
int mppi_set_noise_ring(mppi_handle *h, const float *eps_ring, int32_t n_slots);
int mppi_set_iteration(mppi_handle *h, int64_t iteration);

int mppi_rollout_viz(mppi_handle *h, float *optimal_traj, float *sampled_traj, void *stream);

int mppi_set_state(mppi_handle *h, const double *x);
int mppi_get_state(mppi_handle *h, double *x);
int mppi_run_closed_loop(mppi_handle *h, int32_t n_iters, double *u0_trace ,
                         mppi_stats *stats, void *stream);

int mppi_eval_state_transition(mppi_handle *h, const double *x, const double *v, int32_t n, double *x_next);
int mppi_eval_clamp(mppi_handle *h, const double *v, int32_t n, double *out);
int mppi_eval_is_collided(mppi_handle *h, const double *x, int32_t n, double *out);
int mppi_eval_nearest_waypoint(mppi_handle *h, const double *x, int32_t n, int32_t *prev_idx, int32_t update_prev_idx,
                               int32_t *idx_out);
int mppi_eval_cost(mppi_handle *h, int32_t terminal, const double *x, int32_t n, int32_t *prev_idx, int32_t update_prev_idx,
                   double *cost, int32_t *idx_out);
int mppi_eval_moving_average(mppi_handle *h, const double *xx, double *out);
int mppi_eval_weights(mppi_handle *h, const double *S, int32_t n, double *w);

int mppi_last_kernel_ms(mppi_handle *h, float *out4);
int mppi_enable_timing(mppi_handle *h, int32_t on);
int mppi_set_rollout_repeats(mppi_handle *h, int32_t n);
int mppi_get_counters(mppi_handle *h, int64_t *out3);

int mppi_get_host_timing(const mppi_handle *h, double *out2);

int mppi_time_rollout_launch(mppi_handle *h, int32_t n_slots, int32_t extra, void *stream, double *us_out2);

int mppi_get_rollout_layout(const mppi_handle *h, int32_t *layout);
int mppi_get_rollout_kernel(const mppi_handle *h, char *buf, int32_t n);

typedef enum {
    MPPI_CB_DYN_UNICYCLE = 0,
    MPPI_CB_DYN_SKID_STEER = 1
} mppi_cb_dynamics;
typedef enum {
    MPPI_CB_OBS_INVERSE = 0,
    MPPI_CB_OBS_EXPONENTIAL = 1
} mppi_cb_obstacle_cost;
typedef struct {
    int32_t struct_size, device;
    int32_t dynamics;
    int32_t obstacle_kind;
    int32_t K, T;
    int32_t n_obs;
    int32_t sample_null_action;
    double dt, lambda_;
    double noise_sigma[16];
    double u_min[4], u_max[4], u_init[4];
    double goal[5], q_diag[5], r_diag[4];
    double obstacles[64];
    double safety_distance, obstacle_weight;
    double skid_params[5];
    uint64_t seed;
} mppi_cb_config;
typedef struct mppi_cb_handle mppi_cb_handle;
const char *mppi_cb_last_error(const mppi_cb_handle *h);
int mppi_cb_create(const mppi_cb_config *cfg, mppi_cb_handle **out);
int mppi_cb_destroy(mppi_cb_handle *h);
int mppi_cb_set_nominal(mppi_cb_handle *h, const double *U);
int mppi_cb_get_nominal(mppi_cb_handle *h, double *U);
int mppi_cb_command(mppi_cb_handle *h, const double *state, const float *eps, int32_t shift_nominal_trajectory,
                    double *action_out, void *stream);
int mppi_cb_get_costs(mppi_cb_handle *h, double *cost_total, double *omega);
int mppi_cb_eval(mppi_cb_handle *h, int32_t what, const double *states, const double *actions, int32_t t, int32_t n,
                 double *out);
int mppi_cb_nominal_trajectory(mppi_cb_handle *h, const double *state, double *traj);

#ifdef __cplusplus
}
#endif
#endif
```

Baseline: 21.97 billion trajectory-steps/s.

## Size merge/finalize group count to the number of partial records

Adds a group-count template parameter (tiers 1/2/4/8) to the merge and finalize kernels, picked at plan time from how many partial records are being combined. With few records, each group spans more vector columns and there are fewer cross-group sums, which is meant to cut idle lanes and register use in the tail kernels. It also adds a switch to force the old 8-group tier, an API to report which tail kernels were chosen, and a build hook for a tier test harness. The cost is more template instantiations and a sched_barrier after tile loads.

Result: slower. 21.03 billion trajectory-steps/s (-4.3%).

```diff
diff --git a/dnn-mppi-mpc_amd/_capi.py b/dnn-mppi-mpc_amd/_capi.py
--- a/dnn-mppi-mpc_amd/_capi.py
+++ b/dnn-mppi-mpc_amd/_capi.py
@@ -110,6 +110,7 @@
     "mppi_get_rollout_layout": (C.c_int, [_H, C.POINTER(C.c_int32)]),
     "mppi_get_host_timing": (C.c_int, [_H, C.POINTER(C.c_double)]),
     "mppi_get_rollout_kernel": (C.c_int, [_H, C.c_char_p, C.c_int32]),
+    "mppi_get_tail_kernels": (C.c_int, [_H, C.c_char_p, C.c_char_p, C.c_int32]),
     "mppi_time_rollout_launch": (C.c_int, [_H, C.c_int32, C.c_int32, C.c_void_p, C.POINTER(C.c_double)]),
     "mppi_step_device_x0": (C.c_int, [_H, C.c_void_p, C.c_void_p, _D, _D, C.POINTER(MppiStats), C.c_void_p]),
     "mppi_eval_state_transition": (C.c_int, [_H, _D, _D, C.c_int32, _D]),
diff --git a/dnn-mppi-mpc_amd/build.py b/dnn-mppi-mpc_amd/build.py
--- a/dnn-mppi-mpc_amd/build.py
+++ b/dnn-mppi-mpc_amd/build.py
@@ -33,18 +33,30 @@
 PRIMS_SRC = os.path.join(os.path.dirname(PKG), "tests", "device", "prims_harness.hip")
 
 
-def prims_library() -> str:
-    srcs = [PRIMS_SRC] + [os.path.join(CSRC, f) for f in os.listdir(CSRC) if f.endswith(".h")]
-    if not os.path.exists(PRIMS_LIB) or any(os.path.getmtime(s) > os.path.getmtime(PRIMS_LIB) for s in srcs):
-        res = subprocess.run(["make", "-C", CSRC, "prims"], stdout=subprocess.PIPE, stderr=subprocess.STDOUT, text=True)
+TIERS_LIB = os.path.join(PKG, "lib", "libmppi_merge_tiers.so")
+TIERS_SRC = os.path.join(os.path.dirname(PKG), "tests", "device", "merge_tiers_harness.hip")
+
+
+def _harness_library(lib: str, src: str, target: str) -> str:
+    srcs = [src] + [os.path.join(CSRC, f) for f in os.listdir(CSRC) if f.endswith(".h")]
+    if not os.path.exists(lib) or any(os.path.getmtime(s) > os.path.getmtime(lib) for s in srcs):
+        res = subprocess.run(["make", "-C", CSRC, target], stdout=subprocess.PIPE, stderr=subprocess.STDOUT, text=True)
         if res.returncode != 0:
             print(res.stdout)
-            raise RuntimeError("building libmppi_prims.so failed (hipcc, gfx950)")
-    return PRIMS_LIB
+            raise RuntimeError(f"building {os.path.basename(lib)} failed (hipcc, gfx950)")
+    return lib
+
+
+def prims_library() -> str:
+    return _harness_library(PRIMS_LIB, PRIMS_SRC, "prims")
+
+
+def tiers_library() -> str:
+    return _harness_library(TIERS_LIB, TIERS_SRC, "tiers")
 
 
 def build(force: bool = False, verbose: bool = False) -> str:
-    if force or lib_is_stale() or not os.path.exists(PRIMS_LIB):
+    if force or lib_is_stale() or not os.path.exists(PRIMS_LIB) or not os.path.exists(TIERS_LIB):
         cmd = ["make", "-j4", "-C", CSRC] + (["-B"] if force else [])
         res = subprocess.run(cmd, stdout=subprocess.PIPE, stderr=subprocess.STDOUT, text=True)
         if verbose or res.returncode != 0:
diff --git a/dnn-mppi-mpc_amd/csrc/mppi_capi.hip b/dnn-mppi-mpc_amd/csrc/mppi_capi.hip
--- a/dnn-mppi-mpc_amd/csrc/mppi_capi.hip
+++ b/dnn-mppi-mpc_amd/csrc/mppi_capi.hip
@@ -53,6 +53,7 @@
     sw.mlp.form = form && !strcmp(form, "4x64") ? 0 : form && !strcmp(form, "8x64") ? 1 : -1;
     if (const char *e = getenv("MPPI_EXCHANGE_TIMEOUT_MS")) sw.exchange_timeout_ms = atoll(e);
     sw.lb_timeout_ticks = std::max(0, num("MPPI_LB_TIMEOUT_TICKS", (int)LB_TIMEOUT_TICKS));
+    sw.merge_tier8 = set("MPPI_MERGE_TIER8");
     return sw;
 }
 
@@ -88,6 +89,7 @@
     long long seq = 0;
     bool idx_valid = true;
     int layout = 0;
+    const char *merge_kernel = "", *finalize_kernel = "";
     const char *rollout_kernel = "";
     MlpParams mlp = {}, mlp_shared = {};
     bool shared_set = false;
@@ -948,12 +950,12 @@
     const void *recs = h->d_partials, *heads = h->d_heads;
     const MergeTree tree = merge_tree(sp.front.records, rank_record == nullptr);
     if (tree.group) {
-        sp.merge[sp.n_merges++] = plan_merge<R>(recs, heads, sp.front.records, tree.group, h->cfg.T, h->d_partials2, h->d_heads2);
+        sp.merge[sp.n_merges++] = plan_merge<R>(recs, heads, sp.front.records, tree.group, h->cfg.T, h->d_partials2, h->d_heads2, h->sw);
         recs = h->d_partials2;
         heads = h->d_heads2;
     }
     if (rank_record) {
-        sp.merge[sp.n_merges++] = plan_merge<R>(recs, heads, tree.n_out, tree.n_out, h->cfg.T, rank_record, nullptr);
+        sp.merge[sp.n_merges++] = plan_merge<R>(recs, heads, tree.n_out, tree.n_out, h->cfg.T, rank_record, nullptr, h->sw);
         return sp;
     }
     F->partials = recs;
@@ -962,7 +964,7 @@
     F->hyp = sp.front.lookback;
     F->hyp_blocks = sp.front.records;
     wire_exchange(h, *F);
-    sp.fin = plan_finalize<R>(*F, false, sp.front.lookback);
+    sp.fin = plan_finalize<R>(*F, false, sp.front.lookback, h->sw);
     return sp;
 }
 
@@ -982,12 +984,14 @@
     if (tm) hipEventRecord(next_event(h), s);
     if (sp.reduce) launch_reduce<R>(P, h->d_partials, sp.front.records, s);
     for (int i = 0; i < sp.n_merges; ++i) launch_merge<R>(sp.merge[i], h->cfg.T, sp.beta, s);
+    h->merge_kernel = sp.n_merges ? sp.merge[sp.n_merges - 1].k.name : "";
     if (tm) hipEventRecord(next_event(h), s);
 }
 
 static void launch_back(mppi_handle *h, const KernelLaunch &fin, const FinalizeParams &F, hipStream_t s, bool tm) {
     if (tm) hipEventRecord(next_event(h), s);
     ++h->n_finalize_launches;
+    h->finalize_kernel = fin.name;
     launch_finalize(fin, F, s);
     if (tm) hipEventRecord(next_event(h), s);
     if (tm) hipEventRecord(next_event(h), s);
@@ -1242,7 +1246,7 @@
     HIPCHECK(h, hipSetDevice(h->cfg.device));
     hipStream_t s = (hipStream_t)stream;
     const FinalizeParams F = make_finalize(h, 0, partials, nranks);
-    with_real(h, [&](auto r) { launch_back(h, plan_finalize<decltype(r)>(F, true, false), F, s, h->slot_timed); });
+    with_real(h, [&](auto r) { launch_back(h, plan_finalize<decltype(r)>(F, true, false, h->sw), F, s, h->slot_timed); });
     if ((rc = fetch_result(h, h->res_bytes, s))) return rc;
     h->begun = false;
     h->dev_loop_primed = false;
@@ -1258,7 +1262,7 @@
     if (!h->begun) FAIL(h, MPPI_ERR_STATE, "mppi_step_end_async without mppi_step_begin");
     HIPCHECK(h, hipSetDevice(h->cfg.device));
     const FinalizeParams F = make_finalize(h, 1, partials, nranks);
-    with_real(h, [&](auto r) { launch_back(h, plan_finalize<decltype(r)>(F, true, false), F, (hipStream_t)stream, h->slot_timed); });
+    with_real(h, [&](auto r) { launch_back(h, plan_finalize<decltype(r)>(F, true, false, h->sw), F, (hipStream_t)stream, h->slot_timed); });
     HIPCHECK(h, hipGetLastError());
     h->begun = false;
     h->idx_valid = false;
@@ -1454,7 +1458,7 @@
                                       h->rccl_comm, s));
     FinalizeParams F = make_finalize(h, plant, h->d_rccl_gath, h->rccl_nranks);
     F.u0_trace = u0_trace_dev;
-    launch_back(h, plan_finalize<R>(F, true, false), F, s, tm);
+    launch_back(h, plan_finalize<R>(F, true, false, h->sw), F, s, tm);
     return MPPI_OK;
 }
 
@@ -1967,6 +1971,13 @@
     return MPPI_OK;
 }
 
+extern "C" int mppi_get_tail_kernels(const mppi_handle *h, char *merge_buf, char *finalize_buf, int32_t n) {
+    if (!h || !merge_buf || !finalize_buf || n < 1) return MPPI_ERR_BAD_ARG;
+    snprintf(merge_buf, (size_t)n, "%s", h->merge_kernel);
+    snprintf(finalize_buf, (size_t)n, "%s", h->finalize_kernel);
+    return MPPI_OK;
+}
+
 extern "C" int mppi_enable_timing(mppi_handle *h, int32_t on) {
     if (!h) return MPPI_ERR_BAD_ARG;
     if (on && !h->timing) h->ev_used = 0;
diff --git a/dnn-mppi-mpc_amd/csrc/mppi_kernels.h b/dnn-mppi-mpc_amd/csrc/mppi_kernels.h
--- a/dnn-mppi-mpc_amd/csrc/mppi_kernels.h
+++ b/dnn-mppi-mpc_amd/csrc/mppi_kernels.h
@@ -76,6 +76,7 @@
     t.windows = (t.n_out + MERGE_MAX_RECORDS - 1) / MERGE_MAX_RECORDS;
     return t;
 }
+constexpr int merge_tier(int n, bool force8 = false) { return force8 || n > 128 ? 8 : n > 64 ? 4 : n > 32 ? 2 : 1; }
 
 struct alignas(32) AgentScene {
     const void *ref, *obs;
@@ -197,6 +198,7 @@
     struct Mlp { bool f32 = false; int terms = 3, form = -1; } mlp;
     long long exchange_timeout_ms = 0;
     int lb_timeout_ticks = (int)LB_TIMEOUT_TICKS;
+    bool merge_tier8 = false;
 };
 
 struct KernelLaunch {
@@ -258,9 +260,10 @@
 int fused_max_records(int K, int T, int layout);
 template <typename R> RolloutPlan plan_rollout(const KParams<R> &P, bool fused, const Switches &sw);
 template <typename R> void launch_rollout(const RolloutPlan &plan, const KParams<R> &P, void *partials, hipStream_t s);
-template <typename R> MergeStep plan_merge(const void *recs, const void *heads, int n, int group, int T, void *out, void *out_heads);
+template <typename R>
+MergeStep plan_merge(const void *recs, const void *heads, int n, int group, int T, void *out, void *out_heads, const Switches &sw);
 template <typename R> void launch_merge(const MergeStep &m, int T, double beta, hipStream_t s);
-template <typename R> KernelLaunch plan_finalize(const FinalizeParams &F, bool abi_recs, bool lookback);
+template <typename R> KernelLaunch plan_finalize(const FinalizeParams &F, bool abi_recs, bool lookback, const Switches &sw);
 void launch_finalize(const KernelLaunch &k, const FinalizeParams &F, hipStream_t s);
 void launch_exchange_probe(const FinalizeParams &F, int *ok_out, hipStream_t s);
 enum { EVAL_TRANSITION = 0, EVAL_COST_STAGE = 1, EVAL_COST_TERMINAL = 2, EVAL_COLLIDED = 3, EVAL_CLAMP = 4 };
diff --git a/dnn-mppi-mpc_amd/csrc/mppi_kernels.hip b/dnn-mppi-mpc_amd/csrc/mppi_kernels.hip
--- a/dnn-mppi-mpc_amd/csrc/mppi_kernels.hip
+++ b/dnn-mppi-mpc_amd/csrc/mppi_kernels.hip
@@ -1,6 +1,8 @@
 #include <hip/hip_runtime.h>
 #include <limits.h>
 #include <math.h>
+
+#include <type_traits>
 
 #include "mppi_device.h"
 
@@ -1308,7 +1310,7 @@
     if (k < K) w[k] = exp(-beta * ((double)S[k] - rho)) / eta;
 }
 
-template <typename A, bool ABI_OUT>
+template <typename A, bool ABI_OUT, int GA = 8>
 __global__ __launch_bounds__(MERGE_THREADS) void k_merge(const A *__restrict__ recs, const A *__restrict__ heads, int n,
                                                          int group, int T, A beta, void *__restrict__ out,
                                                          A *__restrict__ out_heads) {
@@ -1317,7 +1319,7 @@
     A *sh_w = L.w;
     const int b0 = blockIdx.x * group, nb = min(group, n - b0);
     const A *mine = recs + (size_t)b0 * record_len(T, (int)sizeof(A));
-    MergeRegs<A, MERGE_THREADS, 1> mr;
+    MergeRegs<A, MERGE_THREADS, 1, GA> mr;
     merge_load_heads<A, MERGE_THREADS, 1>(heads + 4 * (size_t)b0, mr);
     merge_load_tile<A, MERGE_THREADS, 1>(mine, T, 0, mr);
     A rho, eta, eta2, n_hit = 0;
@@ -1387,7 +1389,7 @@
     if (tid == 0) *ok_out = ok ? 1 : 0;
 }
 
-template <typename A, int MODE, int NT, int NWIN, bool PLAIN = false, bool HYPK = false>
+template <typename A, int MODE, int NT, int NWIN, bool PLAIN = false, bool HYPK = false, int GA = NT / 32>
 __device__ __forceinline__ void finalize_body(const void *partials_pre, const void *heads_pre, const DevState *st_pre,
                                               const void *u_pre, int T_pre, const FinalizeParams &F, char *smem,
                                               int agent) {
@@ -1417,7 +1419,7 @@
     const A u_old = tid < 2 * T_pre ? u_in[tid] : A(0);
     unsigned long long peer_ptr = 0;
     if (XCHG) peer_ptr = load_peer_ptrs(F);
-    MergeRegs<A, NT, NWIN> mr;
+    MergeRegs<A, NT, NWIN, GA> mr;
     constexpr int HW = HYP_MAX_BLOCKS / 256;
     uint4 hwords[HW];
 #pragma unroll
@@ -1677,7 +1679,7 @@
     STAMP(21);
 }
 
-template <typename A, int MODE, int NWIN, bool MULTI, bool PLAIN = false, bool HYPK = false>
+template <typename A, int MODE, int NWIN, bool MULTI, bool PLAIN = false, bool HYPK = false, int GA = 8>
 __global__ __launch_bounds__(MERGE_THREADS) void k_finalize(const void *partials_pre, const void *heads_pre,
                                                             const DevState *st_pre, const void *u_pre, int T_pre,
                                                             const FinalizeParams F) {
@@ -1690,12 +1692,11 @@
         Fa.n_ref = sc.n_ref;
         Fa.count_hits = F.count_hits && sc.n_obs > 0;
         const size_t rec = (size_t)a * F.slots * record_len(T_pre, (int)sizeof(A));
-        finalize_body<A, MODE, MERGE_THREADS, NWIN>(reinterpret_cast<const A *>(partials_pre) + rec,
-                                                    reinterpret_cast<const A *>(heads_pre) + (size_t)a * F.slots * 4,
-                                                    st_pre + a, reinterpret_cast<const A *>(u_pre) + (size_t)a * 2 * T_pre,
-                                                    T_pre, Fa, smem, a);
+        finalize_body<A, MODE, MERGE_THREADS, NWIN, false, false, GA>(
+            reinterpret_cast<const A *>(partials_pre) + rec, reinterpret_cast<const A *>(heads_pre) + (size_t)a * F.slots * 4,
+            st_pre + a, reinterpret_cast<const A *>(u_pre) + (size_t)a * 2 * T_pre, T_pre, Fa, smem, a);
     } else {
-        finalize_body<A, MODE, MERGE_THREADS, NWIN, PLAIN, HYPK>(partials_pre, heads_pre, st_pre, u_pre, T_pre, F, smem, 0);
+        finalize_body<A, MODE, MERGE_THREADS, NWIN, PLAIN, HYPK, GA>(partials_pre, heads_pre, st_pre, u_pre, T_pre, F, smem, 0);
     }
 }
 
@@ -2037,13 +2038,23 @@
 
 static size_t merge_lds(int T, int W, size_t elem) { return elem * merge_lds_elems(T, W, elem); }
 
-template <typename R, bool ABI_OUT> static KernelLaunch merge_entry() {
-    static KernelEntry e("k_merge<%s, %s>", type_name<R>(), KernelEntry::of(ABI_OUT));
-    return plan_entry(reinterpret_cast<const void *>(k_merge<R, ABI_OUT>), e, MERGE_THREADS);
-}
-template <typename R> MergeStep plan_merge(const void *recs, const void *heads, int n, int group, int T, void *out, void *out_heads) {
+template <typename R, bool ABI_OUT, int GA> static KernelLaunch merge_entry() {
+    static KernelEntry e("k_merge<%s, %s, %d>", type_name<R>(), KernelEntry::of(ABI_OUT), GA);
+    return plan_entry(reinterpret_cast<const void *>(k_merge<R, ABI_OUT, GA>), e, MERGE_THREADS);
+}
+template <typename Entry> static KernelLaunch at_tier(int ga, Entry entry) {
+    return ga == 1   ? entry(std::integral_constant<int, 1>{})
+           : ga == 2 ? entry(std::integral_constant<int, 2>{})
+           : ga == 4 ? entry(std::integral_constant<int, 4>{})
+                     : entry(std::integral_constant<int, 8>{});
+}
+template <typename R>
+MergeStep plan_merge(const void *recs, const void *heads, int n, int group, int T, void *out, void *out_heads, const Switches &sw) {
     MergeStep m;
-    m.k = out_heads ? merge_entry<R, false>() : merge_entry<R, true>();
+    m.k = at_tier(merge_tier(group, sw.merge_tier8), [&](auto tier) {
+        constexpr int GA = decltype(tier)::value;
+        return out_heads ? merge_entry<R, false, GA>() : merge_entry<R, true, GA>();
+    });
     m.k.grid = dim3((n + group - 1) / group);
     m.k.lds = merge_lds(T, 0, sizeof(R));
     m.recs = recs, m.heads = heads, m.n = n, m.group = group, m.out = out, m.out_heads = out_heads;
@@ -2056,22 +2067,29 @@
     launch_plan(m.k, args, s);
 }
 
-template <typename R, int MODE, int NWIN, bool MULTI, bool PLAIN = false, bool HYPK = false> static KernelLaunch finalize_entry() {
-    static KernelEntry e("k_finalize<%s, %d, %d, %s, %s, %s>", type_name<R>(), MODE, NWIN, KernelEntry::of(MULTI), KernelEntry::of(PLAIN),
-                         KernelEntry::of(HYPK));
-    return plan_entry(reinterpret_cast<const void *>(k_finalize<R, MODE, NWIN, MULTI, PLAIN, HYPK>), e, MERGE_THREADS);
-}
-template <typename R> KernelLaunch plan_finalize(const FinalizeParams &F, bool abi_recs, bool lookback) {
+template <typename R, int MODE, int NWIN, bool MULTI, bool PLAIN = false, bool HYPK = false, int GA = 8> static KernelLaunch finalize_entry() {
+    static KernelEntry e("k_finalize<%s, %d, %d, %s, %s, %s, %d>", type_name<R>(), MODE, NWIN, KernelEntry::of(MULTI),
+                         KernelEntry::of(PLAIN), KernelEntry::of(HYPK), GA);
+    return plan_entry(reinterpret_cast<const void *>(k_finalize<R, MODE, NWIN, MULTI, PLAIN, HYPK, GA>), e, MERGE_THREADS);
+}
+template <typename R> KernelLaunch plan_finalize(const FinalizeParams &F, bool abi_recs, bool lookback, const Switches &sw) {
     const bool two = merge_tree(F.n_part, true).windows > 1;
     const bool multi = !abi_recs && F.x_nranks <= 1 && F.n_agents > 1;
     const bool plain = F.sequential && F.plant && !F.use_args && !F.raise_at_path_end && !F.clamp_u && F.model == MODEL_DIFF &&
                        !F.u0_trace && F.filter_mode == FILTER_DIFF;
+    const auto one_window = [&](auto tier) {
+        constexpr int GA = decltype(tier)::value;
+        return F.x_nranks > 1 ? finalize_entry<R, 2, 1, false, false, false, GA>()
+               : multi        ? finalize_entry<R, 0, 1, true, false, false, GA>()
+               : lookback     ? (plain ? finalize_entry<R, 0, 1, false, true, true, GA>() : finalize_entry<R, 0, 1, false, false, true, GA>())
+                              : (plain ? finalize_entry<R, 0, 1, false, true, false, GA>() : finalize_entry<R, 0, 1, false, false, false, GA>());
+    };
     KernelLaunch k = abi_recs         ? finalize_entry<R, 1, 1, false>()
-                     : F.x_nranks > 1 ? (two ? finalize_entry<R, 2, 2, false>() : finalize_entry<R, 2, 1, false>())
-                     : multi          ? (two ? finalize_entry<R, 0, 2, true>() : finalize_entry<R, 0, 1, true>())
-                     : two            ? (lookback ? finalize_entry<R, 0, 2, false, false, true>() : finalize_entry<R, 0, 2, false>())
-                     : lookback       ? (plain ? finalize_entry<R, 0, 1, false, true, true>() : finalize_entry<R, 0, 1, false, false, true>())
-                                      : (plain ? finalize_entry<R, 0, 1, false, true, false>() : finalize_entry<R, 0, 1, false>());
+                     : !two           ? at_tier(merge_tier(F.n_part, sw.merge_tier8), one_window)
+                     : F.x_nranks > 1 ? finalize_entry<R, 2, 2, false>()
+                     : multi          ? finalize_entry<R, 0, 2, true>()
+                     : lookback       ? finalize_entry<R, 0, 2, false, false, true>()
+                                      : finalize_entry<R, 0, 2, false>();
     k.grid = dim3(1, multi ? F.n_agents : 1);
     k.lds = merge_lds(F.T, F.filter_window, sizeof(R)) + (F.x_nranks > 1 ? sizeof(double) * XCHG_LDS_RANKS * xchg_rec_len(F.T) : 0) +
             (lookback ? (size_t)HYP_MAX_BLOCKS + 16 : 0);
@@ -2144,9 +2162,9 @@
     template RolloutPlan plan_rollout<R>(const KParams<R> &, bool, const Switches &);                     \
     template void launch_rollout<R>(const RolloutPlan &, const KParams<R> &, void *, hipStream_t);        \
     template void launch_reduce<R>(const KParams<R> &, void *, int, hipStream_t);                         \
-    template MergeStep plan_merge<R>(const void *, const void *, int, int, int, void *, void *);             \
+    template MergeStep plan_merge<R>(const void *, const void *, int, int, int, void *, void *, const Switches &); \
     template void launch_merge<R>(const MergeStep &, int, double, hipStream_t);                           \
-    template KernelLaunch plan_finalize<R>(const FinalizeParams &, bool, bool);                           \
+    template KernelLaunch plan_finalize<R>(const FinalizeParams &, bool, bool, const Switches &);         \
     template void launch_weights<R>(const KParams<R> &, double, double, double *, hipStream_t);           \
     template void launch_eval_index<R>(const KParams<R> &, const R *, int, int, int, int, int *, int *, hipStream_t); \
     template void launch_eval<R>(const KParams<R> &, int, const R *, const R *, const int *, int, R *, hipStream_t);   \
diff --git a/dnn-mppi-mpc_amd/csrc/mppi_merge.h b/dnn-mppi-mpc_amd/csrc/mppi_merge.h
--- a/dnn-mppi-mpc_amd/csrc/mppi_merge.h
+++ b/dnn-mppi-mpc_amd/csrc/mppi_merge.h
@@ -12,8 +12,12 @@
 
 namespace mppi {
 
-template <int NT> struct MergeShape {
-    static constexpr int GROUPS = NT / 32, MAXJ = MERGE_MAX_RECORDS / GROUPS, WAVES = NT / 64;
+template <int NT, int GA = NT / 32> struct MergeShape {
+    static_assert(GA == NT / 32 || (NT == 256 && (GA == 1 || GA == 2 || GA == 4)), "tiers: 256 threads, 1 / 2 / 4 / 8 groups");
+    static constexpr int GROUPS = GA, MAXJ = MERGE_MAX_RECORDS / (NT / 32), WAVES = NT / 64;
+    static constexpr int CW = NT / GA;
+    static constexpr int NH = GA >= 8 ? 4 : (GA + 1) / 2;
+    static constexpr int GPW = CW < 64 ? 64 / CW : 1;
 };
 
 template <typename A> struct alignas(16) VecT { A v[16 / sizeof(A)]; };
@@ -95,17 +99,20 @@
     }
 };
 
-template <typename A, int NT = MERGE_THREADS, int NWIN = 1> struct MergeRegs {
-    VecT<A> w[NWIN][MergeShape<NT>::MAXJ];
-    A hr[4 * NWIN], he[4 * NWIN], he2[4 * NWIN];
-    A hc[4 * NWIN];
-};
-
-template <typename A, int NT, int NWIN>
-__device__ __forceinline__ void merge_load_heads(const A *__restrict__ heads, MergeRegs<A, NT, NWIN> &m) {
+template <typename A, int NT = MERGE_THREADS, int NWIN = 1, int GA = NT / 32> struct MergeRegs {
+    static_assert(GA == NT / 32 || NWIN == 1, "tiers below NT / 32 groups: one window");
+    static constexpr int NH = MergeShape<NT, GA>::NH;
+    VecT<A> w[NWIN][MergeShape<NT, GA>::MAXJ];
+    A hr[NH * NWIN], he[NH * NWIN], he2[NH * NWIN];
+    A hc[NH * NWIN];
+};
+
+template <typename A, int NT, int NWIN, int GA>
+__device__ __forceinline__ void merge_load_heads(const A *__restrict__ heads, MergeRegs<A, NT, NWIN, GA> &m) {
+    constexpr int NH = MergeShape<NT, GA>::NH;
     const int lane = threadIdx.x & 63;
 #pragma unroll
-    for (int i = 0; i < 4 * NWIN; ++i) {
+    for (int i = 0; i < NH * NWIN; ++i) {
         const int b = lane + 64 * i;
         const size_t r = (size_t)b;
         const VecT4<A> hd = *reinterpret_cast<const VecT4<A> *>(heads + 4 * r);
@@ -116,44 +123,46 @@
     }
 }
 
-template <typename A, int NT, int NWIN>
-__device__ __forceinline__ void merge_load_tile(const A *__restrict__ recs, int T, int vt, MergeRegs<A, NT, NWIN> &m) {
-    constexpr int VW = 16 / sizeof(A), MAXJ = MergeShape<NT>::MAXJ;
-    const int tid = threadIdx.x, vc = tid & 31, grp = tid >> 5;
+template <typename A, int NT, int NWIN, int GA>
+__device__ __forceinline__ void merge_load_tile(const A *__restrict__ recs, int T, int vt, MergeRegs<A, NT, NWIN, GA> &m) {
+    constexpr int VW = 16 / sizeof(A), MAXJ = MergeShape<NT, GA>::MAXJ, CW = MergeShape<NT, GA>::CW;
+    const int tid = threadIdx.x, vc = tid & (CW - 1), grp = (int)((unsigned)tid / CW);
     const unsigned rbytes = (unsigned)record_len(T, (int)sizeof(A)) * (unsigned)sizeof(A);
     const int nvc = (2 * T + VW - 1) / VW;
     const char *base = reinterpret_cast<const char *>(recs);
-    const unsigned col = (unsigned)(4 + min(vt * 32 + vc, nvc - 1) * VW) * (unsigned)sizeof(A);
+    const unsigned col = (unsigned)(4 + min(vt * CW + vc, nvc - 1) * VW) * (unsigned)sizeof(A);
     const unsigned off0 = (unsigned)(grp * MAXJ) * rbytes + col;
 #pragma unroll
     for (int win = 0; win < NWIN; ++win)
 #pragma unroll
         for (int j = 0; j < MAXJ; ++j)
             m.w[win][j] = *reinterpret_cast<const VecT<A> *>(base + (off0 + (unsigned)(win * MERGE_MAX_RECORDS + j) * rbytes));
-}
-
-template <typename A, int NT, int NWIN, typename Store>
+    if constexpr (GA != NT / 32) __builtin_amdgcn_sched_barrier(0);
+}
+
+template <typename A, int NT, int NWIN, int GA, typename Store>
 __device__ __forceinline__ void merge_combine(const A *__restrict__ recs, int n, int T, A beta,
-                                              MergeRegs<A, NT, NWIN> &m, A *sh_s, A *sh_part, A &rho, A &eta, A &eta2,
+                                              MergeRegs<A, NT, NWIN, GA> &m, A *sh_s, A *sh_part, A &rho, A &eta, A &eta2,
                                               Store store, A *n_hit = nullptr) {
-    constexpr int VW = 16 / sizeof(A), MAXJ = MergeShape<NT>::MAXJ, GROUPS = MergeShape<NT>::GROUPS;
+    using Shape = MergeShape<NT, GA>;
+    constexpr int VW = 16 / sizeof(A), MAXJ = Shape::MAXJ, GROUPS = Shape::GROUPS, CW = Shape::CW, NH = Shape::NH, GPW = Shape::GPW;
     using V = VecT<A>;
     const int tid = threadIdx.x, lane = tid & 63, wid = tid >> 6;
-    const int vc = tid & 31, grp = tid >> 5;
+    const int vc = tid & (CW - 1), grp = (int)((unsigned)tid / CW);
     const int nvc = (2 * T + VW - 1) / VW;
     A lr = A(INFINITY);
 #pragma unroll
-    for (int i = 0; i < 4 * NWIN; ++i) {
+    for (int i = 0; i < NH * NWIN; ++i) {
         if (lane + 64 * i >= n) m.hr[i] = A(INFINITY);
         lr = fmin(lr, m.hr[i]);
     }
     rho = wv::reduce<wv::OpMin>(lr);
     STAMP(25);
-    A sc[4 * NWIN];
+    A sc[NH * NWIN];
     eta = 0;
     eta2 = 0;
 #pragma unroll
-    for (int i = 0; i < 4 * NWIN; ++i) {
+    for (int i = 0; i < NH * NWIN; ++i) {
         sc[i] = lane + 64 * i < n ? fast_exp(-beta * (m.hr[i] - rho)) : A(0);
         eta += sc[i] * m.he[i];
         eta2 += sc[i] * sc[i] * m.he2[i];
@@ -163,22 +172,26 @@
     if (n_hit && *n_hit >= A(0)) {
         A cnt = 0;
 #pragma unroll
-        for (int i = 0; i < 4 * NWIN; ++i) cnt += lane + 64 * i < n ? m.hc[i] : A(0);
+        for (int i = 0; i < NH * NWIN; ++i) cnt += lane + 64 * i < n ? m.hc[i] : A(0);
         *n_hit = wv::reduce<wv::OpAdd>(cnt);
     }
-    const int r0 = wid * 2 * MAXJ, slot = r0 >> 6;
+    const int r0 = (int)((unsigned)(wid * 64) / CW) * MAXJ, slot = r0 >> 6;
     A *my_s = sh_s + wid * 64;
 #pragma unroll
-    for (int win = 0; win < NWIN; ++win)
-        my_s[win * NT + lane] = slot == 0 ? sc[4 * win] : slot == 1 ? sc[4 * win + 1] : slot == 2 ? sc[4 * win + 2] : sc[4 * win + 3];
+    for (int win = 0; win < NWIN; ++win) {
+        if constexpr (NH == 4) my_s[win * NT + lane] = slot == 0 ? sc[4 * win] : slot == 1 ? sc[4 * win + 1] : slot == 2 ? sc[4 * win + 2] : sc[4 * win + 3];
+        else if constexpr (NH == 2) my_s[win * NT + lane] = slot == 0 ? sc[2 * win] : sc[2 * win + 1];
+        else my_s[win * NT + lane] = sc[win];
+    }
     __builtin_amdgcn_fence(__ATOMIC_RELEASE, "wavefront");
     __builtin_amdgcn_wave_barrier();
     __builtin_amdgcn_fence(__ATOMIC_ACQUIRE, "wavefront");
     STAMP(26);
-    const A *sj_base = my_s + (r0 & 63) + (grp & 1) * MAXJ;
+    const A *sj_base = my_s + (r0 & 63) + (grp & (GPW - 1)) * MAXJ;
     const A inv_eta = fast_div(A(1), eta);
-    const int n_tiles = (nvc + 31) / 32;
-    for (int vt = 0; vt < n_tiles; ++vt) {
+    const int n_tiles = (nvc + CW - 1) / CW;
+    constexpr bool FIRST_ROUND_RUNS = GA != NT / 32;
+    for (int vt = 0; vt < n_tiles || (FIRST_ROUND_RUNS && vt == 0); ++vt) {
         V acc;
 #pragma unroll
         for (int q = 0; q < VW; ++q) acc.v[q] = 0;
@@ -191,15 +204,15 @@
                 for (int q = 0; q < VW; ++q) acc.v[q] += sj * m.w[win][j].v[q];
             }
         if (vt > 0) __syncthreads();
-        *reinterpret_cast<V *>(sh_part + (grp * 32 + vc) * VW) = acc;
+        *reinterpret_cast<V *>(sh_part + (grp * CW + vc) * VW) = acc;
         __syncthreads();
         if (__builtin_expect(vt + 1 < n_tiles, 0)) merge_load_tile<A, NT, NWIN>(recs, T, vt + 1, m);
-        for (int e = tid; e < 32 * VW; e += NT) {
-            const int i = vt * 32 * VW + e;
+        for (int e = tid; e < CW * VW; e += NT) {
+            const int i = vt * CW * VW + e;
             if (i < 2 * T) {
                 A t = 0;
 #pragma unroll
-                for (int g = 0; g < GROUPS; ++g) t += sh_part[g * 32 * VW + e];
+                for (int g = 0; g < GROUPS; ++g) t += sh_part[g * CW * VW + e];
                 store(i, t * inv_eta);
             }
         }
diff --git a/dnn-mppi-mpc_amd/engine.py b/dnn-mppi-mpc_amd/engine.py
--- a/dnn-mppi-mpc_amd/engine.py
+++ b/dnn-mppi-mpc_amd/engine.py
@@ -370,6 +370,13 @@
         self._ck(self.lib.mppi_get_rollout_kernel(self._h, buf, 192))
         return buf.value.decode()
 
+    def tail_kernels(self):
+        if not hasattr(self.lib, "mppi_get_tail_kernels"):
+            return {"merge": "", "finalize": ""}
+        m, f = C.create_string_buffer(192), C.create_string_buffer(192)
+        self._ck(self.lib.mppi_get_tail_kernels(self._h, m, f, 192))
+        return {"merge": m.value.decode(), "finalize": f.value.decode()}
+
     def host_timing(self):
         out = (C.c_double * 2)()
         self._ck(self.lib.mppi_get_host_timing(self._h, out))
diff --git a/include/mppi_hip.h b/include/mppi_hip.h
--- a/include/mppi_hip.h
+++ b/include/mppi_hip.h
@@ -174,6 +174,7 @@
 
 int mppi_get_rollout_layout(const mppi_handle *h, int32_t *layout);
 int mppi_get_rollout_kernel(const mppi_handle *h, char *buf, int32_t n);
+int mppi_get_tail_kernels(const mppi_handle *h, char *merge_buf, char *finalize_buf, int32_t n);
 
 typedef enum {
     MPPI_CB_DYN_UNICYCLE = 0,
```
